# SeanNaren/deepspeech.pytorch

Measured on AMD Instinct MI355X. Metric: audio-seconds/sec (train step), higher is better.
Workload: dtype bf16

## Files before the change

### deepspeech/pytorch_amd/_lib.py

```python
import ctypes as C
import os

HERE = os.path.dirname(os.path.abspath(__file__))
LIB_PATH = os.path.join(HERE, "libds2hip.so")

F32, BF16 = 0, 1
CELL_GRU, CELL_LSTM, CELL_RNN_TANH = 0, 1, 2

_vp, _i, _l, _f, _ll = C.c_void_p, C.c_int, C.c_long, C.c_float, C.c_longlong

SIGNATURES = {
    "ds2_version": (_i, []),
    "ds2_error_string": (C.c_char_p, [_i]),
    "ds2_gemm_nt": (_i, [_i, _vp, _vp, _vp, _vp, _i, _i, _i, _l, _l, _l, _i, _i, _l, _l, _l, _l, _i, _vp]),
    "ds2_gemm_nt_coresident": (_i, [_i, _vp, _vp, _vp, _vp, _i, _i, _i, _l, _l, _l, _i, _i, _l, _l, _l, _l, _i, _vp]),
    "ds2_gemm_nt_rows2": (_i, [_i, _vp, _vp, _i, _vp, _vp, _i, _i, _i, _l, _l, _l, _i, _i, _i, _vp]),
    "ds2_gemm8_nt": (_i, [_vp, _vp, _vp, _vp, _i, _i, _i, _l, _l, _l, _i, _vp]),
    "ds2_gemm8_tn_grouped": (_i, [_i, _vp, _vp, _vp, _vp, _vp, _vp, _vp, _vp, _vp, _vp, _vp, _i, _vp]),
    "ds2_gemm8_nt_rows": (_i, [_vp, _vp, _vp, _vp, _i, _i, _i, _l, _l, _l, _i, _vp, _i, _vp]),
    "ds2_gemm8_tn_grouped_rows": (_i, [_i, _vp, _vp, _vp, _vp, _vp, _vp, _vp, _vp, _vp, _vp, _vp, _i, _vp, _i, _vp]),
    "ds2_gemm8_wgrad_dx_rows": (_i, [_i, _vp, _vp, _vp, _vp, _vp, _vp, _vp, _vp, _vp, _vp, _vp, _i, _vp, _vp, _vp, _i, _i, _i, _l, _l, _l, _vp, _i, _vp]),
    "ds2_zero_pad_rows": (_i, [_i, _vp, _l, _i, _vp, _i, _i, _vp]),
    "ds2_gemm8_wgrad_dx": (_i, [_i, _vp, _vp, _vp, _vp, _vp, _vp, _vp, _vp, _vp, _vp, _vp, _i, _vp, _vp, _vp, _i, _i, _i, _l, _l, _l, _vp]),
    "ds2_norm_partials": (_i, [_l]),
    "ds2_bn_fwd": (_i, [_i, _i, _i, _vp, _vp, _l, _i, _l, _l, _i, _i, _i, _vp, _vp, _vp, _vp, _vp, _vp, _f, _f, _vp, _vp,
                        _vp, _vp, _vp, _vp]),
    "ds2_bn_bwd": (_i, [_i, _i, _vp, _vp, _vp, _l, _i, _l, _l, _l, _i, _i, _i, _vp, _vp, _vp, _vp, _vp, _vp, _vp, _vp, _vp]),
    "ds2_colsum": (_i, [_i, _vp, _l, _i, _l, _vp, _f, _vp, _vp]),
    "ds2_conv_rows": (_i, [_i, _vp, _vp]),
    "ds2_conv1_fwd": (_i, [_i, _vp, _vp, _vp, _vp, _vp, _i, _i, _i, _i, _vp]),
    "ds2_conv1_wgrad_ws_floats": (_l, [_i, _i, _i]),
    "ds2_conv1_wgrad": (_i, [_i, _vp, _vp, _vp, _i, _i, _i, _i, _vp, _vp]),
    "ds2_conv2_fwd_ws_bytes": (_l, [_i, _i, _i, _i]),
    "ds2_conv2_fwd": (_i, [_i, _vp, _vp, _vp, _vp, _vp, _i, _i, _i, _vp, _vp]),
    "ds2_conv2_dgrad": (_i, [_i, _vp, _vp, _vp, _vp, _i, _i, _i, _vp]),
    "ds2_conv2_wgrad_ws_floats": (_l, [_i, _i]),
    "ds2_conv2_wgrad": (_i, [_i, _vp, _vp, _vp, _i, _i, _i, _vp, _vp]),
    "ds2_rnn_gates": (_i, [_i]),
    "ds2_rnn_saved_planes": (_i, [_i]),
    "ds2_rnn_state_bytes": (_l, [_i, _i, _i]),
    "ds2_rnn_fwd": (_i, [_i, _i, _i, _i, _i, _i, _vp, _vp, _vp, _vp, _vp, _vp, _vp, _l, _vp, _vp, _vp, _vp, _vp]),
    "ds2_rnn_bwd": (_i, [_i, _i, _i, _i, _i, _i, _vp, _vp, _vp, _vp, _l, _vp, _vp, _vp, _vp, _vp, _vp, _vp, _vp, _vp]),
    "ds2_rnn_persist_plan": (_i, [_i, _i, _i, _i, _i, _i, C.c_uint, C.POINTER(_l)]),
    "ds2_rnn_persist_supported": (_i, [_i, _i, _i, _i, _i, C.c_uint]),
    "ds2_rnn_persist_shape_covered": (_i, [_i, _i, _i, _i, _i]),
    "ds2_rnn_persist_kind": (_i, [_i, _i, _i, _i, _i, C.c_uint]),
    "ds2_rnn_persist_ws_bytes": (_l, [_i, _i, _i, _i, _i, C.c_uint]),
    "ds2_rnn_persist_fwd": (_i, [_i, _i, _i, _i, _i, _i, _vp, _vp, _vp, _vp, _vp, _vp, _vp, _l, _vp, _vp, _vp, _vp, _vp, _vp, _vp]),
    "ds2_rnn_persist_bwd": (_i, [_i, _i, _i, _i, _i, _i, _vp, _vp, _vp, _vp, _l, _vp, _vp, _vp, _vp, _i, _vp, _vp, _vp, _vp]),
    "ds2_add2": (_i, [_i, _vp, _vp, _vp, _l, _vp]),
    "ds2_sum_slices": (_i, [_vp, _vp, _l, _i, _vp]),
    "ds2_transpose": (_i, [_i, _vp, _vp, _l, _i, _l, _l, _vp]),
    "ds2_split3_bf16": (_i, [_vp, _l, _l, _i, _i, _i, _vp, _l, _vp]),
    "ds2_cast_transpose_bf16": (_i, [_vp, _l, _i, _i, _i, _i, _i, _vp, _l, _vp, _l, _vp]),
    "ds2_small_weight_layouts": (_i, [_i, _vp, _vp, _vp, _i, _i, _vp, _vp, _vp, _vp, _vp, _vp, _vp]),
    "ds2_scale_by": (_i, [_vp, _vp, _l, _vp]),
    "ds2_copy_words": (_i, [_vp, _vp, _l, _vp]),
    "ds2_lookahead_fwd": (_i, [_i, _vp, _vp, _vp, _vp, _i, _i, _i, _i, _vp]),
    "ds2_lookahead_ws_floats": (_l, [_i, _i, _i, _i]),
    "ds2_lookahead_bwd": (_i, [_i, _vp, _vp, _vp, _vp, _vp, _vp, _i, _i, _i, _i, _vp, _vp]),
    "ds2_rnn_bias_grads": (_i, [_i, _i, _i, _i, _vp, _vp, _vp, _vp]),
    "ds2_softmax_rows": (_i, [_vp, _vp, _l, _i, _l, _l, _vp]),
    "ds2_opt_max_tensors": (_i, []),
    "ds2_clip_ws_floats": (_l, [_i, _vp]),
    "ds2_clip_coef": (_i, [_i, _vp, _vp, _f, _vp, _vp, _vp]),
    "ds2_opt_multi": (_i, [_i, _i, _vp, _vp, _vp, _vp, _vp, _vp, _i, _vp, _vp]),
    "ds2_opt_matrix": (_i, [_i, _vp, _vp, _vp, _vp, _i, _i, _i, _i, _i, _vp, _l, _vp, _l, _vp, _i, _vp, _vp]),
    "ds2_opt_matrices": (_i, [_i, _i] + [_vp] * 13 + [_vp, _i, _vp, _vp]),
    "ds2_spect_frames": (_i, [_i]),
    "ds2_spect_ws_bytes": (_l, [_i, _i]),
    "ds2_spectrogram": (_i, [_vp, _l, _vp, _i, _i, _vp, _i, _i, _vp, _vp, _vp]),
    "ds2_spectrogram_aug": (_i, [_vp, _l, _vp, _i, _i, _vp, _i, _i, _vp, _vp, _vp, _i, _vp, _i, _vp, _i, _vp, _vp]),
    "ds2_spec_augment_coef": (_i, [_vp, _i, _i, _i, _vp, _vp, _i, _vp, _vp]),
    "ds2_spec_augment": (_i, [_vp, _vp, _i, _i, _i, _vp, _vp, _vp, _i, _vp, _i, _vp]),
    "ds2_greedy_decode": (_i, [_vp, _l, _l, _i, _i, _i, _vp, _i, _vp, _vp, _vp, _vp]),
    "ds2_beam_ws_bytes": (_l, [_i, _i, _i]),
    "ds2_beam_decode": (_i, [_vp, _l, _l, _i, _i, _i, _vp, _i, _i, _i, _f, _vp, _vp, _vp, _vp, _vp, _vp]),
    "ds2_beam_decode_lm": (_i, [_vp, _l, _l, _i, _i, _i, _vp, _i, _i, _i, _f, _i, _vp, _l, _vp, _l, _i, _i, _f, _f, _i,
                                _vp, _vp, _vp, _vp, _vp, _vp, _vp]),
    "ds2_beam_grid_ws_bytes": (_l, [_i, _i, _i, _i]),
    "ds2_beam_decode_lm_grid": (_i, [_vp, _l, _l, _i, _i, _i, _vp, _i, _i, _i, _f, _i, _vp, _l, _vp, _l, _i, _i, _i, _i, _vp, _vp,
                                     _vp, _vp, _vp, _vp, _vp, _vp, _vp]),
    "ds2_error_counts": (_i, [_vp, _l, _vp, _i, _vp, _vp, _i, _i, _vp, _vp, _vp, _vp, _vp]),
    "ds2_ctc_ws_floats": (_l, [_i, _i, _i, _i]),
    "ds2_ctc_loss_grad": (_i, [_vp, _l, _vp, _vp, _vp, _vp, _i, _i, _i, _i, _i, _f, _vp, _vp, _vp, _l, _vp, _i, _vp]),
}



class PersistOpts(C.Structure):
    _fields_ = [("variant", C.c_uint), ("spin_limit", C.c_uint), ("startup_ms", C.c_uint)]


_lib = None


class Ds2HipError(RuntimeError):
    pass


def load():
    global _lib
    if _lib is not None:
        return _lib
    if not os.path.exists(LIB_PATH):
        raise Ds2HipError(
            "libds2hip.so not found at %s -- build it with `python -m deepspeech.pytorch_amd.build` "
            "(hipcc --offload-arch=gfx950).  There is no fallback path." % LIB_PATH)
    lib = C.CDLL(LIB_PATH)
    for name, (res, args) in SIGNATURES.items():
        fn = getattr(lib, name)
        fn.restype = res
        fn.argtypes = args
    _lib = lib
    return lib


def error_string(code):
    return load().ds2_error_string(int(code)).decode()


def call(name, *args):
    rc = getattr(load(), name)(*args)
    if rc != 0:
        raise Ds2HipError("%s failed with code %d: %s" % (name, rc, error_string(rc)))


def query(name, *args):
    return getattr(load(), name)(*args)
```

### deepspeech/pytorch_amd/csrc/ds2_norm.hip

```cpp
#include "ds2_common.h"

namespace {

constexpr int NORM_RY = 8;
constexpr int NORM_CX = 32;

struct RowMap {
  int F, Tp;
  __device__ __forceinline__ void nt(long row, int& n, int& t) const {
    t = (int)(row % Tp);
    n = (int)(row / ((long)F * Tp));
  }
};

__device__ __forceinline__ float bn_affine(float x, float sc, float sh) { return __builtin_fmaf(x, sc, sh); }
__device__ __forceinline__ bool hardtanh_open(float y) { return y > 0.f && y < 20.f; }
__device__ __forceinline__ float bn_dx(float g, float xh, float sc, float k1, float k2) { return sc * __builtin_fmaf(-xh, k2, g - k1); }

struct RedMap {
  int cpb, rpx, chunk, rsub;
  bool ok;
  __device__ __forceinline__ RedMap(int chunks) {
    cpb = chunks < NORM_CX ? chunks : NORM_CX;
    rpx = NORM_CX / cpb;
    const int tx = threadIdx.x;
    rsub = tx / cpb;
    chunk = blockIdx.x * cpb + tx % cpb;
    ok = rsub < rpx && chunk < chunks;
  }
  __device__ __forceinline__ long first_row() const { return ((long)blockIdx.y * NORM_RY + threadIdx.y) * rpx + rsub; }
  __device__ __forceinline__ long row_step() const { return (long)gridDim.y * NORM_RY * rpx; }
};
template <int V>
__device__ __forceinline__ void red_block(float (*red)[NORM_CX * V + 1], const RedMap& m, const float (&v)[V], float (&out)[V]) {
  __syncthreads();
#pragma unroll
  for (int i = 0; i < V; ++i) red[threadIdx.y][threadIdx.x * V + i] = v[i];
  __syncthreads();
  if (threadIdx.y == 0 && m.rsub == 0) {
#pragma unroll
    for (int i = 0; i < V; ++i) {
      float a = 0.f;
      for (int k = 0; k < m.rpx; ++k)
#pragma unroll
        for (int y = 0; y < NORM_RY; ++y) a += red[y][(threadIdx.x + k * m.cpb) * V + i];
      out[i] = a;
    }
  }
}

template <typename T, bool SQ>
__global__ void __launch_bounds__(NORM_RY* NORM_CX) k_colstats(const T* __restrict__ X, long R, int C, long ld,
                                                                float* __restrict__ psum, float* __restrict__ psq) {
  constexpr int V = Vec16<T>::N;
  __shared__ float red[NORM_RY][NORM_CX * V + 1];
  const RedMap m(C / V);
  float s[V], q[V];
#pragma unroll
  for (int i = 0; i < V; ++i) s[i] = q[i] = 0.f;
  if (m.ok) {
    for (long r = m.first_row(); r < R; r += m.row_step()) {
      float v[V];
      Vec16<T>::load(X + r * ld + (long)m.chunk * V, v);
#pragma unroll
      for (int i = 0; i < V; ++i) {
        s[i] += v[i];
        if (SQ) q[i] += v[i] * v[i];
      }
    }
  }
  float o[V];
  red_block<V>(red, m, s, o);
  if (threadIdx.y == 0 && m.rsub == 0 && m.ok) {
#pragma unroll
    for (int i = 0; i < V; ++i) psum[(long)blockIdx.y * C + (long)m.chunk * V + i] = o[i];
  }
  if (SQ) {
    red_block<V>(red, m, q, o);
    if (threadIdx.y == 0 && m.rsub == 0 && m.ok) {
#pragma unroll
      for (int i = 0; i < V; ++i) psq[(long)blockIdx.y * C + (long)m.chunk * V + i] = o[i];
    }
  }
}

constexpr int FIN_COLS = 32, FIN_SLICES = 8;
template <int NA>
__device__ __forceinline__ void finalize_sums(const float* const (&arr)[NA], int P, int C, int c, int py, double (&tot)[NA]) {
  __shared__ double sh[NA][FIN_SLICES][FIN_COLS];
  double acc[NA];
#pragma unroll
  for (int a = 0; a < NA; ++a) acc[a] = 0.0;
  if (c < C) {
#pragma unroll 8
    for (int p = py; p < P; p += FIN_SLICES) {
#pragma unroll
      for (int a = 0; a < NA; ++a) acc[a] += (double)arr[a][(long)p * C + c];
    }
  }
#pragma unroll
  for (int a = 0; a < NA; ++a) sh[a][py][threadIdx.x & (FIN_COLS - 1)] = acc[a];
  __syncthreads();
#pragma unroll
  for (int a = 0; a < NA; ++a) {
    double t = 0.0;
    if (py == 0) {
#pragma unroll
      for (int q = 0; q < FIN_SLICES; ++q) t += sh[a][q][threadIdx.x & (FIN_COLS - 1)];
    }
    tot[a] = t;
  }
}

__global__ void __launch_bounds__(256) k_colsum_finalize(const float* __restrict__ psum, int P, int C, float* __restrict__ out,
                                                          float scale) {
  const int c = blockIdx.x * FIN_COLS + (threadIdx.x & (FIN_COLS - 1)), py = threadIdx.x / FIN_COLS;
  const float* const arr[1] = {psum};
  double tot[1];
  finalize_sums<1>(arr, P, C, c, py, tot);
  if (py == 0 && c < C) out[c] = (float)(tot[0] * (double)scale);
}

__global__ void k_bn_finalize(const float* __restrict__ psum, const float* __restrict__ psq, int P, int C, double count,
                              const float* __restrict__ gamma, const float* __restrict__ beta, float eps,
                              float momentum, float* __restrict__ running_mean, float* __restrict__ running_var,
                              long long* __restrict__ num_batches_tracked, float* __restrict__ mean_out,
                              float* __restrict__ rstd_out, float* __restrict__ scale_out, float* __restrict__ shift_out) {
  const int c = blockIdx.x * FIN_COLS + (threadIdx.x & (FIN_COLS - 1)), py = threadIdx.x / FIN_COLS;
  if (blockIdx.x == 0 && threadIdx.x == 0 && num_batches_tracked) *num_batches_tracked += 1;
  const float* const arr[2] = {psum, psq};
  double tot[2];
  finalize_sums<2>(arr, P, C, c, py, tot);
  if (py != 0 || c >= C) return;
  const double s = tot[0], q = tot[1];
  double mean = s / count;
  double var = q / count - mean * mean;
  if (var < 0.0) var = 0.0;
  double rstd = 1.0 / sqrt(var + (double)eps);
  mean_out[c] = (float)mean;
  rstd_out[c] = (float)rstd;
  float sc = (float)((double)gamma[c] * rstd);
  scale_out[c] = sc;
  shift_out[c] = (float)((double)beta[c] - mean * (double)gamma[c] * rstd);
  if (running_mean) {
    double unb = count > 1.0 ? var * (count / (count - 1.0)) : var;
    running_mean[c] = (float)((1.0 - (double)momentum) * (double)running_mean[c] + (double)momentum * mean);
    running_var[c] = (float)((1.0 - (double)momentum) * (double)running_var[c] + (double)momentum * unb);
  }
}

__global__ void k_bn_eval_coeffs(int C, const float* __restrict__ gamma, const float* __restrict__ beta,
                                 const float* __restrict__ running_mean, const float* __restrict__ running_var, float eps,
                                 float* __restrict__ scale_out, float* __restrict__ shift_out) {
  int c = blockIdx.x * blockDim.x + threadIdx.x;
  if (c >= C) return;
  double rstd = 1.0 / sqrt((double)running_var[c] + (double)eps);
  scale_out[c] = (float)((double)gamma[c] * rstd);
  shift_out[c] = (float)((double)beta[c] - (double)running_mean[c] * (double)gamma[c] * rstd);
}

template <typename T, bool CONV, bool SEQ_OUT, bool CENTRED = false>
__global__ void __launch_bounds__(256) k_bn_apply(const T* __restrict__ X, T* __restrict__ Y, long R, int C, long ldx,
                                                   long ldy, const float* __restrict__ scale,
                                                   const float* __restrict__ shift, const float* __restrict__ mean,
                                                   const float* __restrict__ beta, RowMap rm,
                                                   const int* __restrict__ lens, int N) {
  constexpr int V = Vec16<T>::N;
  const int chunks = C / V;
  const long total = R * chunks;
  for (long e = (long)blockIdx.x * blockDim.x + threadIdx.x; e < total; e += (long)gridDim.x * blockDim.x) {
    long r = e / chunks;
    int c0 = (int)(e % chunks) * V;
    float v[V];
    bool live = true;
    int n = 0, t = 0;
    if (CONV) {
      rm.nt(r, n, t);
      live = t < lens[n];
    }
    if (live) {
      Vec16<T>::load(X + r * ldx + c0, v);
#pragma unroll
      for (int i = 0; i < V; ++i) {
        float y = CENTRED ? __builtin_fmaf(v[i] - mean[c0 + i], scale[c0 + i], beta[c0 + i]) : bn_affine(v[i], scale[c0 + i], shift[c0 + i]);
        if (CONV) y = fminf(fmaxf(y, 0.f), 20.f);
        v[i] = y;
      }
    } else {
#pragma unroll
      for (int i = 0; i < V; ++i) v[i] = 0.f;
    }
    if (SEQ_OUT) {
      int f = (int)((r / rm.Tp) % rm.F);
      Vec16<T>::store(Y + ((long)t * N + n) * ldy + (long)f * C + c0, v);
    } else {
      Vec16<T>::store(Y + r * ldy + c0, v);
    }
  }
}

template <typename T, bool CONV, bool SEQ_IN>
__device__ __forceinline__ bool load_gated(const T* __restrict__ G, const T* __restrict__ X, long r, int c0, int C,
                                           long ldg, long ldx, const float* __restrict__ scale,
                                           const float* __restrict__ shift, const float* __restrict__ mean,
                                           const float* __restrict__ rstd, const RowMap& rm, const int* __restrict__ lens,
                                           int N, float (&g)[Vec16<T>::N], float (&xh)[Vec16<T>::N]) {
  constexpr int V = Vec16<T>::N;
  int n = 0, t = 0, f = 0;
  if (CONV) {
    const unsigned ur = (unsigned)r, q = ur / (unsigned)rm.Tp;
    t = (int)(ur - q * (unsigned)rm.Tp);
    n = (int)(q / (unsigned)rm.F);
    f = (int)(q - (unsigned)n * (unsigned)rm.F);
  }
  const int len = CONV ? lens[n] : 0;
  float x[V];
  Vec16<T>::load(X + r * ldx + c0, x);
  if (SEQ_IN) {
    Vec16<T>::load(G + ((long)t * N + n) * ldg + (long)f * C + c0, g);
  } else {
    Vec16<T>::load(G + r * ldg + c0, g);
  }
  if (CONV && t >= len) return false;
#pragma unroll
  for (int i = 0; i < V; ++i) {
    if (CONV) {
      if (!hardtanh_open(bn_affine(x[i], scale[c0 + i], shift[c0 + i]))) g[i] = 0.f;
    }
    xh[i] = (x[i] - mean[c0 + i]) * rstd[c0 + i];
  }
  return true;
}

template <typename T, bool CONV, bool SEQ_IN>
__global__ void __launch_bounds__(NORM_RY* NORM_CX)
    k_bn_bwd_reduce(const T* __restrict__ G, const T* __restrict__ X, long R, int C, long ldg, long ldx,
                    const float* __restrict__ scale, const float* __restrict__ shift, const float* __restrict__ mean,
                    const float* __restrict__ rstd, RowMap rm, const int* __restrict__ lens, int N,
                    float* __restrict__ psum_g, float* __restrict__ psum_gx) {
  constexpr int V = Vec16<T>::N;
  __shared__ float red[NORM_RY][NORM_CX * V + 1];
  const RedMap m(C / V);
  float s[V], q[V];
#pragma unroll
  for (int i = 0; i < V; ++i) s[i] = q[i] = 0.f;
  if (m.ok) {
    for (long r = m.first_row(); r < R; r += m.row_step()) {
      float g[V], xh[V];
      if (load_gated<T, CONV, SEQ_IN>(G, X, r, m.chunk * V, C, ldg, ldx, scale, shift, mean, rstd, rm, lens, N, g, xh)) {
#pragma unroll
        for (int i = 0; i < V; ++i) {
          s[i] += g[i];
          q[i] += g[i] * xh[i];
        }
      }
    }
  }
  float o[V];
  red_block<V>(red, m, s, o);
  if (threadIdx.y == 0 && m.rsub == 0 && m.ok) {
#pragma unroll
    for (int i = 0; i < V; ++i) psum_g[(long)blockIdx.y * C + (long)m.chunk * V + i] = o[i];
  }
  red_block<V>(red, m, q, o);
  if (threadIdx.y == 0 && m.rsub == 0 && m.ok) {
#pragma unroll
    for (int i = 0; i < V; ++i) psum_gx[(long)blockIdx.y * C + (long)m.chunk * V + i] = o[i];
  }
}

__global__ void k_bn_bwd_finalize(const float* __restrict__ psum_g, const float* __restrict__ psum_gx, int P, int C,
                                  double count, float* __restrict__ dgamma, float* __restrict__ dbeta,
                                  float* __restrict__ c1, float* __restrict__ c2) {
  const int c = blockIdx.x * FIN_COLS + (threadIdx.x & (FIN_COLS - 1)), py = threadIdx.x / FIN_COLS;
  const float* const arr[2] = {psum_g, psum_gx};
  double tot[2];
  finalize_sums<2>(arr, P, C, c, py, tot);
  if (py != 0 || c >= C) return;
  const double s = tot[0], q = tot[1];
  dbeta[c] = (float)s;
  dgamma[c] = (float)q;
  c1[c] = (float)(s / count);
  c2[c] = (float)(q / count);
}

template <typename T, bool CONV, bool SEQ_IN>
__global__ void __launch_bounds__(256)
    k_bn_bwd_apply(const T* __restrict__ G, const T* __restrict__ X, T* __restrict__ DX, long R, int C, long ldg, long ldx,
                   long lddx, const float* __restrict__ scale, const float* __restrict__ shift,
                   const float* __restrict__ mean, const float* __restrict__ rstd, const float* __restrict__ c1,
                   const float* __restrict__ c2, RowMap rm, const int* __restrict__ lens, int N) {
  constexpr int V = Vec16<T>::N;
  const int chunks = C / V;
  const long total = R * chunks;
  for (long e = (long)blockIdx.x * blockDim.x + threadIdx.x; e < total; e += (long)gridDim.x * blockDim.x) {
    long r = e / chunks;
    int c0 = (int)(e % chunks) * V;
    float g[V], xh[V], o[V];
    if (load_gated<T, CONV, SEQ_IN>(G, X, r, c0, C, ldg, ldx, scale, shift, mean, rstd, rm, lens, N, g, xh)) {
#pragma unroll
      for (int i = 0; i < V; ++i) o[i] = bn_dx(g[i], xh[i], scale[c0 + i], c1[c0 + i], c2[c0 + i]);
    } else {
#pragma unroll
      for (int i = 0; i < V; ++i) o[i] = 0.f;
    }
    Vec16<T>::store(DX + r * lddx + c0, o);
  }
}

template <typename T, bool CONV, bool SEQ_IN>
__global__ void __launch_bounds__(NORM_RY* NORM_CX)
    k_bn_bwd_apply_cols(const T* __restrict__ G, const T* __restrict__ X, T* __restrict__ DX, long R, int C, long ldg, long ldx,
                        long lddx, const float* __restrict__ scale, const float* __restrict__ shift,
                        const float* __restrict__ mean, const float* __restrict__ rstd, const float* __restrict__ c1,
                        const float* __restrict__ c2, RowMap rm, const int* __restrict__ lens, int N) {
  constexpr int V = Vec16<T>::N;
  const RedMap m(C / V);
  if (!m.ok) return;
  const int c0 = m.chunk * V;
  float sc[V], sh[V], mu[V], rs[V], k1[V], k2[V];
#pragma unroll
  for (int i = 0; i < V; ++i) {
    sc[i] = scale[c0 + i];
    sh[i] = CONV ? shift[c0 + i] : 0.f;
    mu[i] = mean[c0 + i];
    rs[i] = rstd[c0 + i];
    k1[i] = c1[c0 + i];
    k2[i] = c2[c0 + i];
  }
  const long step = m.row_step();
  auto addr = [&](long r, int& t, int& len, const T*& gp) {
    int n = 0, f = 0;
    t = 0;
    if (CONV) {
      const unsigned ur = (unsigned)r, q = ur / (unsigned)rm.Tp;
      t = (int)(ur - q * (unsigned)rm.Tp);
      n = (int)(q / (unsigned)rm.F);
      f = (int)(q - (unsigned)n * (unsigned)rm.F);
    }
    len = CONV ? lens[n] : 0;
    gp = SEQ_IN ? G + ((long)t * N + n) * ldg + (long)f * C + c0 : G + r * ldg + c0;
  };
  auto finish = [&](long r, int t, int len, float (&x)[V], float (&g)[V]) {
    float o[V];
    if (CONV && t >= len) {
#pragma unroll
      for (int i = 0; i < V; ++i) o[i] = 0.f;
    } else {
#pragma unroll
      for (int i = 0; i < V; ++i) {
        float gi = g[i];
        if (CONV) {
          if (!hardtanh_open(bn_affine(x[i], sc[i], sh[i]))) gi = 0.f;
        }
        const float xh = (x[i] - mu[i]) * rs[i];
        o[i] = bn_dx(gi, xh, sc[i], k1[i], k2[i]);
      }
    }
    Vec16<T>::store(DX + r * lddx + c0, o);
  };
  long r = m.first_row();
  for (; r + step < R; r += 2 * step) {
    int t0, t1, l0, l1;
    const T *g0p, *g1p;
    addr(r, t0, l0, g0p);
    addr(r + step, t1, l1, g1p);
    float x0[V], x1[V], g0[V], g1[V];
    Vec16<T>::load(X + r * ldx + c0, x0);
    Vec16<T>::load(X + (r + step) * ldx + c0, x1);
    Vec16<T>::load(g0p, g0);
    Vec16<T>::load(g1p, g1);
    finish(r, t0, l0, x0, g0);
    finish(r + step, t1, l1, x1, g1);
  }
  if (r < R) {
    int t0, l0;
    const T* g0p;
    addr(r, t0, l0, g0p);
    float x0[V], g0[V];
    Vec16<T>::load(X + r * ldx + c0, x0);
    Vec16<T>::load(g0p, g0);
    finish(r, t0, l0, x0, g0);
  }
}

inline int norm_grid_y(long R, int col_blocks = 1) {
  long gy = (R + NORM_RY - 1) / NORM_RY;
  long cap = 1024 / (col_blocks < 1 ? 1 : col_blocks);
  if (cap < 256) cap = 256;
  if (gy > cap) gy = cap;
  if (gy < 1) gy = 1;
  return (int)gy;
}

template <typename T>
int colstats_impl(const void* X, long R, int C, long ld, float* psum, float* psq, int* P_out, hipStream_t st) {
  constexpr int V = Vec16<T>::N;
  DS2_REQUIRE(C % V == 0 && ld % V == 0, DS2_ERR_ALIGN);
  dim3 blk(NORM_CX, NORM_RY);
  dim3 grd(ds2_cdiv(C / V, NORM_CX), norm_grid_y(R, ds2_cdiv(C / V, NORM_CX)));
  if (psq)
    hipLaunchKernelGGL((k_colstats<T, true>), grd, blk, 0, st, (const T*)X, R, C, ld, psum, psq);
  else
    hipLaunchKernelGGL((k_colstats<T, false>), grd, blk, 0, st, (const T*)X, R, C, ld, psum, psq);
  *P_out = grd.y;
  DS2_CHECK_LAUNCH();
  return 0;
}

inline int apply_grid(long total) {
  long g = (total + 255) / 256;
  if (g > 256 * 8) g = 256 * 8;
  if (g < 1) g = 1;
  return (int)g;
}

}

extern "C" {

int ds2_norm_partials(long R) { return norm_grid_y(R); }

int ds2_colsum(int dtype, const void* X, long R, int C, long ld, float* out, float scale, float* ws, ds2_stream_t st_) {
  hipStream_t st = (hipStream_t)st_;
  int P = 0, rc;
  if (dtype == DS2_F32)
    rc = colstats_impl<float>(X, R, C, ld, ws, nullptr, &P, st);
  else
    rc = colstats_impl<bf16_t>(X, R, C, ld, ws, nullptr, &P, st);
  if (rc) return rc;
  hipLaunchKernelGGL(k_colsum_finalize, dim3(ds2_cdiv(C, FIN_COLS)), dim3(256), 0, st, ws, P, C, out, scale);
  DS2_CHECK_LAUNCH();
  return 0;
}

int ds2_bn_fwd(int dtype, int mode, int training, const void* X, void* Y, long R, int C, long ldx, long ldy, int F, int Tp,
               int N, const int* lens, const float* gamma, const float* beta, float* running_mean, float* running_var,
               long long* num_batches_tracked, float eps, float momentum, float* save_mean, float* save_rstd,
               float* save_scale, float* save_shift, float* ws, ds2_stream_t st_) {
  hipStream_t st = (hipStream_t)st_;
  DS2_REQUIRE(dtype == DS2_F32 || dtype == DS2_BF16, DS2_ERR_DTYPE);
  DS2_REQUIRE(mode >= 0 && mode <= 2, DS2_ERR_ARG);
  DS2_REQUIRE(mode == 0 || R < (1L << 31), DS2_ERR_ARG);
  int rc, P = 0;
  if (training) {
    float* psum = ws;
    float* psq = ws + (long)norm_grid_y(R) * C;
    rc = dtype == DS2_F32 ? colstats_impl<float>(X, R, C, ldx, psum, psq, &P, st)
                          : colstats_impl<bf16_t>(X, R, C, ldx, psum, psq, &P, st);
    if (rc) return rc;
    hipLaunchKernelGGL(k_bn_finalize, dim3(ds2_cdiv(C, FIN_COLS)), dim3(256), 0, st, psum, psq, P, C, (double)R, gamma, beta,
                       eps, momentum, running_mean, running_var, num_batches_tracked, save_mean, save_rstd, save_scale,
                       save_shift);
  } else {
    hipLaunchKernelGGL(k_bn_eval_coeffs, dim3(ds2_cdiv(C, 128)), dim3(128), 0, st, C, gamma, beta, running_mean,
                       running_var, eps, save_scale, save_shift);
  }
  DS2_CHECK_LAUNCH();
  RowMap rm{F, Tp};
  const int V = dtype == DS2_F32 ? 4 : 8;
  DS2_REQUIRE(C % V == 0 && ldx % V == 0 && ldy % V == 0, DS2_ERR_ALIGN);
  dim3 g(apply_grid(R * (C / V))), b(256);
#define LAUNCH_APPLY(TT)                                                                                              \
  if (mode == 0 && training && R == 1)                                                                                \
    hipLaunchKernelGGL((k_bn_apply<TT, false, false, true>), g, b, 0, st, (const TT*)X, (TT*)Y, R, C, ldx, ldy,        \
                       save_scale, save_shift, save_mean, beta, rm, lens, N);                                         \
  else if (mode == 0)                                                                                                 \
    hipLaunchKernelGGL((k_bn_apply<TT, false, false>), g, b, 0, st, (const TT*)X, (TT*)Y, R, C, ldx, ldy, save_scale,  \
                       save_shift, save_mean, beta, rm, lens, N);                                                     \
  else if (mode == 1)                                                                                                 \
    hipLaunchKernelGGL((k_bn_apply<TT, true, false>), g, b, 0, st, (const TT*)X, (TT*)Y, R, C, ldx, ldy, save_scale,   \
                       save_shift, save_mean, beta, rm, lens, N);                                                     \
  else                                                                                                                \
    hipLaunchKernelGGL((k_bn_apply<TT, true, true>), g, b, 0, st, (const TT*)X, (TT*)Y, R, C, ldx, ldy, save_scale,    \
                       save_shift, save_mean, beta, rm, lens, N);
  if (dtype == DS2_F32) {
    LAUNCH_APPLY(float)
  } else {
    LAUNCH_APPLY(bf16_t)
  }
#undef LAUNCH_APPLY
  DS2_CHECK_LAUNCH();
  return 0;
}

int ds2_bn_bwd(int dtype, int mode, const void* G, const void* X, void* DX, long R, int C, long ldg, long ldx, long lddx,
               int F, int Tp, int N, const int* lens, const float* save_mean, const float* save_rstd,
               const float* save_scale, const float* save_shift, float* dgamma, float* dbeta, float* ws, ds2_stream_t st_) {
  hipStream_t st = (hipStream_t)st_;
  DS2_REQUIRE(dtype == DS2_F32 || dtype == DS2_BF16, DS2_ERR_DTYPE);
  DS2_REQUIRE(mode >= 0 && mode <= 2, DS2_ERR_ARG);
  DS2_REQUIRE(mode == 0 || R < (1L << 31), DS2_ERR_ARG);
  const int V = dtype == DS2_F32 ? 4 : 8;
  DS2_REQUIRE(C % V == 0 && ldx % V == 0 && ldg % V == 0 && lddx % V == 0, DS2_ERR_ALIGN);
  RowMap rm{F, Tp};
  const int P = norm_grid_y(R, ds2_cdiv(C / V, NORM_CX));
  float* ps = ws;
  float* pq = ws + (long)P * C;
  float* c1 = pq + (long)P * C;
  float* c2 = c1 + C;
  dim3 blk(NORM_CX, NORM_RY), grd(ds2_cdiv(C / V, NORM_CX), P);
#define LAUNCH_RED(TT, CV, SI)                                                                                          \
  hipLaunchKernelGGL((k_bn_bwd_reduce<TT, CV, SI>), grd, blk, 0, st, (const TT*)G, (const TT*)X, R, C, ldg, ldx,          \
                     save_scale, save_shift, save_mean, save_rstd, rm, lens, N, ps, pq)
  const int acb = ds2_cdiv(C / V, NORM_CX), arpx = NORM_CX / (C / V < NORM_CX ? C / V : NORM_CX);
  long agy = ds2_cdiv(R, (long)NORM_RY * arpx * 2);
  if (agy > 2048 / acb) agy = 2048 / acb;
  if (agy < 1) agy = 1;
  const dim3 agrd(acb, (unsigned)agy);
#ifdef DS2_BN_APPLY_GRIDSTRIDE
#define LAUNCH_APP(TT, CV, SI)                                                                                          \
  hipLaunchKernelGGL((k_bn_bwd_apply<TT, CV, SI>), dim3(apply_grid(R*(C / V))), dim3(256), 0, st, (const TT*)G,           \
                     (const TT*)X, (TT*)DX, R, C, ldg, ldx, lddx, save_scale, save_shift, save_mean, save_rstd, c1, c2, \
                     rm, lens, N)
#else
#define LAUNCH_APP(TT, CV, SI)                                                                                          \
  hipLaunchKernelGGL((k_bn_bwd_apply_cols<TT, CV, SI>), agrd, blk, 0, st, (const TT*)G, (const TT*)X, (TT*)DX, R, C, ldg, \
                     ldx, lddx, save_scale, save_shift, save_mean, save_rstd, c1, c2, rm, lens, N)
#endif
#define BOTH(WHICH)                                        \
  if (dtype == DS2_F32) {                                  \
    if (mode == 0) WHICH(float, false, false);             \
    else if (mode == 1) WHICH(float, true, false);         \
    else WHICH(float, true, true);                         \
  } else {                                                 \
    if (mode == 0) WHICH(bf16_t, false, false);            \
    else if (mode == 1) WHICH(bf16_t, true, false);        \
    else WHICH(bf16_t, true, true);                        \
  }
  BOTH(LAUNCH_RED)
  DS2_CHECK_LAUNCH();
  hipLaunchKernelGGL(k_bn_bwd_finalize, dim3(ds2_cdiv(C, FIN_COLS)), dim3(256), 0, st, ps, pq, P, C, (double)R, dgamma, dbeta,
                     c1, c2);
  DS2_CHECK_LAUNCH();
  BOTH(LAUNCH_APP)
  DS2_CHECK_LAUNCH();
#undef BOTH
#undef LAUNCH_RED
#undef LAUNCH_APP
  return 0;
}

}
```

### deepspeech/pytorch_amd/model.py

```python
import math
from typing import List

import numpy as np
import torch
import torch.nn as nn

from . import ops
from ._lib import Ds2HipError

try:
    import pytorch_lightning as pl
    _Base = pl.LightningModule
except Exception:
    pl = None

    class _Base(nn.Module):

        def save_hyperparameters(self, *a, **k):
            import inspect
            frame = inspect.currentframe().f_back
            try:
                names = [n for n in inspect.signature(type(self).__init__).parameters if n != "self"]
                self._hparams = {n: frame.f_locals[n] for n in names if n in frame.f_locals}
            finally:
                del frame

        @property
        def hparams(self):
            return getattr(self, "_hparams", {})

        def log(self, *a, **k):
            pass

        @property
        def device(self):
            return next(self.parameters()).device

        @classmethod
        def load_from_checkpoint(cls, checkpoint_path, map_location=None, strict=True, **overrides):
            ckpt = torch.load(checkpoint_path, map_location=map_location or "cpu", weights_only=False)
            hp = dict(ckpt.get("hyper_parameters", {}))
            hp.update(overrides)
            model = cls(**hp)
            model.load_state_dict(ckpt["state_dict"], strict=strict)
            return model

try:
    from omegaconf import OmegaConf

    def _cfg_type_name(cfg):
        t = OmegaConf.get_type(cfg)
        return getattr(t, "__name__", str(t))
except Exception:
    def _cfg_type_name(cfg):
        return type(cfg).__name__

from .configs import AdamConfig, BiDirectionalConfig, SGDConfig, SpectConfig, UniDirectionalConfig, rnn_kind

import os

WGRAD_WITH_DX = os.environ.get("DS2_WGRAD_WITH_DX", "1") not in ("", "0")

COMPOSITE_NODE = {"": None, "0": False}.get(os.environ.get("DS2_COMPOSITE_NODE", ""), True)
PER_LAYER_NODES_FOR_DDP = [False]


PAD_HIDDEN = os.environ.get("DS2_PAD_HIDDEN", "1") != "0"


def _padded_hidden(H, kind, precision, bidirectional=None):
    base = (int(H) + 15) // 16 * 16
    if not PAD_HIDDEN or base < 200 or kind not in ("gru", "lstm", "rnn"):
        return base
    try:
        from ._lib import query
        dt_ = ops.dt(torch.bfloat16 if str(precision) in ("16", "bf16", "16-mixed", "bf16-mixed") else torch.float32)
        cell = ops.CELLS[kind]
        dirs = (2, 1) if bidirectional is None else ((2,) if bidirectional else (1,))
        for w in range(base, int(base * 1.5) + 1, 16):
            if any(query("ds2_rnn_persist_shape_covered", dt_, cell, D_, 1, w) for D_ in dirs):
                return w
    except Exception:
        pass
    return base


def _data_parallel_active():
    if PER_LAYER_NODES_FOR_DDP[0]:
        return True
    try:
        import torch.distributed as _dist
        return _dist.is_available() and _dist.is_initialized() and _dist.get_world_size() > 1
    except Exception:
        return False


FP32_WGRAD_TN = os.environ.get("DS2_FP32_WGRAD_TN", "1") != "0"

ROW_LISTS = os.environ.get("DS2_ROW_LISTS", "1") != "0"
ROW_LIST_MIN_PADDING = 0.97

N_FREQ_CONV2 = 41
RNN_INPUT = 32 * N_FREQ_CONV2
RNN_INPUT_LD = 1344


def _round64(n):
    return (n + 63) // 64 * 64


class SequenceWise(nn.Module):
    def __init__(self, module):
        super().__init__()
        self.module = module


class MaskConv(nn.Module):
    def __init__(self, seq_module):
        super().__init__()
        self.seq_module = seq_module


class _RNNParams(nn.Module):

    def __init__(self, kind, input_size, hidden_size, bidirectional):
        super().__init__()
        g = ops.GATES[kind]
        for suf in [""] + (["_reverse"] if bidirectional else []):
            self.register_parameter("weight_ih_l0" + suf, nn.Parameter(torch.empty(g * hidden_size, input_size)))
            self.register_parameter("weight_hh_l0" + suf, nn.Parameter(torch.empty(g * hidden_size, hidden_size)))
            self.register_parameter("bias_ih_l0" + suf, nn.Parameter(torch.empty(g * hidden_size)))
            self.register_parameter("bias_hh_l0" + suf, nn.Parameter(torch.empty(g * hidden_size)))
        stdv = 1.0 / math.sqrt(hidden_size) if hidden_size > 0 else 0
        for w in self.parameters():
            nn.init.uniform_(w, -stdv, stdv)


class BatchRNN(nn.Module):
    def __init__(self, input_size, hidden_size, kind, bidirectional=False, batch_norm=True):
        super().__init__()
        self.input_size, self.hidden_size, self.bidirectional, self.kind = input_size, hidden_size, bidirectional, kind
        self.batch_norm = SequenceWise(nn.BatchNorm1d(input_size)) if batch_norm else None
        self.rnn = _RNNParams(kind, input_size, hidden_size, bidirectional)
        self.num_directions = 2 if bidirectional else 1


class Lookahead(nn.Module):
    def __init__(self, n_features, context):
        super().__init__()
        assert context > 0
        self.context, self.n_features = context, n_features
        self.conv = nn.Conv1d(n_features, n_features, kernel_size=context, stride=1, groups=n_features, padding=0, bias=False)


class _WeightCache:

    def __init__(self):
        self._store = {}
        self.epoch = 0

    def get(self, key, params, builder):
        ver = (self.epoch,) + tuple((p._version, p.data_ptr()) for p in params)
        hit = self._store.get(key)
        if hit is not None and hit[0] == ver:
            return hit[1]
        with torch.no_grad():
            val = builder()
        self._store[key] = (ver, val)
        return val

    def _ver(self, params):
        return (self.epoch,) + tuple((p._version, p.data_ptr()) for p in params)

    def valid(self, key, params):
        hit = self._store.get(key)
        return hit is not None and hit[0] == self._ver(params)

    def put(self, key, params, val, epoch=None):
        ver = self._ver(params)
        if epoch is not None:
            ver = (epoch,) + ver[1:]
        self._store[key] = (ver, val)

    def clear(self):
        self._store.clear()


def _wgrad_splitk(M, N, K):
    tiles = ((M + 127) // 128) * ((N + 127) // 128)
    if tiles >= 128:
        return 1
    return max(1, min(8, 768 // max(tiles, 1), K // (64 * 32)))


def _pad_gate_rows(w, G, H, Hp):
    if Hp == H:
        return w
    out = w.new_zeros((G, Hp) + tuple(w.shape[1:]))
    out[:, :H] = w.reshape((G, H) + tuple(w.shape[1:]))
    return out.reshape((G * Hp,) + tuple(w.shape[1:]))


def _pad_cols(w, Cp):
    if w.shape[-1] == Cp:
        return w
    out = w.new_zeros(tuple(w.shape[:-1]) + (Cp,))
    out[..., :w.shape[-1]] = w
    return out


def _unpad_gate_rows(g, G, H, Hp):
    if Hp == H:
        return g
    return g.reshape((G, Hp) + tuple(g.shape[1:]))[:, :H].reshape((G * H,) + tuple(g.shape[1:])).contiguous()


def _bn_seq_fwd(bn, w, b, X, Xh, R, Ct, Cp, training):
    if Ct == Cp:
        return ops.bn_fwd(X, 0, training, w.detach(), b.detach(), bn.running_mean, bn.running_var, bn.num_batches_tracked, R, Ct,
                          X.stride(0), Xh, Xh.stride(0), eps=bn.eps, momentum=bn.momentum)
    g, be = w.new_ones(Cp), w.new_zeros(Cp)
    rm, rv = w.new_zeros(Cp), w.new_ones(Cp)
    g[:Ct], be[:Ct], rm[:Ct], rv[:Ct] = w.detach(), b.detach(), bn.running_mean, bn.running_var
    sv = ops.bn_fwd(X, 0, training, g, be, rm, rv, bn.num_batches_tracked, R, Cp, X.stride(0), Xh, Xh.stride(0), eps=bn.eps,
                    momentum=bn.momentum)
    if training:
        bn.running_mean.copy_(rm[:Ct])
        bn.running_var.copy_(rv[:Ct])
    return sv


def _bn_seq_bwd(G, X, DX, sv, R, Ct, Cp):
    dg, db = ops.bn_bwd(G, X, DX, 0, sv, R, Cp, G.stride(0), X.stride(0), DX.stride(0))
    return (dg, db) if Ct == Cp else (dg[:Ct].contiguous(), db[:Ct].contiguous())


def _perm_cols_to_internal(w):
    g, rin = w.shape
    out = w.new_zeros((g, _round64(rin)))
    out[:, :rin] = w.reshape(g, 32, rin // 32).permute(0, 2, 1).reshape(g, rin)
    return out


def _perm_cols_to_reference(w, rin=RNN_INPUT):
    g = w.shape[0]
    return w[:, :rin].reshape(g, rin // 32, 32).permute(0, 2, 1).reshape(g, rin)


class _ConvStackFn(torch.autograd.Function):

    @staticmethod
    def forward(ctx, x, w1, b1, g1, be1, w2, b2, g2, be2, mod, lens_dev, Tp, dtype, training):
        N, T = x.shape[0], x.shape[3]
        c = mod._cache
        bn1, bn2 = mod.conv.seq_module[1], mod.conv.seq_module[4]
        w1k = c.get("w1k", [w1], lambda: w1.detach().reshape(32, 451).t().contiguous())
        w2t = c.get(("w2t", dtype), [w2], lambda: w2.detach().permute(2, 3, 0, 1).contiguous().to(dtype))
        x = x.contiguous().float()
        F0, F1, F2, rin, rld = mod._F0, mod._F1, mod._F2, mod._rnn_in, mod._rnn_ld
        if x.shape[2] != F0:
            raise ValueError("this model was built for %d frequency bins (SpectConfig: sample_rate * window_size / 2 + 1), got input "
                             "with %d" % (F0, x.shape[2]))
        y1 = ops.conv1_fwd(x, w1k, b1.detach(), lens_dev, Tp, dtype)
        R1 = N * F1 * Tp
        a1 = torch.empty_like(y1)
        sv1 = ops.bn_fwd(y1, 1, training, g1.detach(), be1.detach(), bn1.running_mean, bn1.running_var,
                         bn1.num_batches_tracked, R1, 32, 32, a1, 32, F=F1, Tp=Tp, N=N, lens=lens_dev, eps=bn1.eps,
                         momentum=bn1.momentum)
        y2 = ops.conv2_fwd(a1, w2t, b2.detach(), lens_dev, F0)
        R2 = N * F2 * Tp
        x0 = torch.empty((Tp * N, rld), dtype=dtype, device=x.device)
        if rld > rin:
            x0[:, rin:].zero_()
        sv2 = ops.bn_fwd(y2, 2, training, g2.detach(), be2.detach(), bn2.running_mean, bn2.running_var,
                         bn2.num_batches_tracked, R2, 32, 32, x0, rld, F=F2, Tp=Tp, N=N, lens=lens_dev, eps=bn2.eps,
                         momentum=bn2.momentum)
        ctx.mod, ctx.dims, ctx.sv = mod, (N, T, Tp, dtype), (sv1, sv2)
        ctx.save_for_backward(x, y1, a1, y2, lens_dev, w2)
        return x0

    @staticmethod
    def backward(ctx, dx0):
        x, y1, a1, y2, lens_dev, w2 = ctx.saved_tensors
        N, T, Tp, dtype = ctx.dims
        sv1, sv2 = ctx.sv
        c = ctx.mod._cache
        dx0 = dx0.contiguous().to(dtype)
        F0, F1, F2, rld = ctx.mod._F0, ctx.mod._F1, ctx.mod._F2, ctx.mod._rnn_ld
        R1, R2 = N * F1 * Tp, N * F2 * Tp
        dy2 = torch.empty_like(y2)
        dg2, dbe2 = ops.bn_bwd(dx0, y2, dy2, 2, sv2, R2, 32, rld, 32, 32, F=F2, Tp=Tp, N=N, lens=lens_dev)
        w2d = c.get(("w2d", dtype), [w2], lambda: [
            w2.detach()[:, :, q::2, :].flip(2, 3).permute(2, 3, 1, 0).contiguous().to(dtype) for q in (0, 1)])
        da1 = ops.conv2_dgrad(dy2, w2d[0], w2d[1], F0)
        dy1 = torch.empty_like(y1)
        dg1, dbe1 = ops.bn_bwd(da1, y1, dy1, 1, sv1, R1, 32, 32, 32, 32, F=F1, Tp=Tp, N=N, lens=lens_dev)
        db1 = ops.colsum(dy1.view(R1, 32))
        dw1k = ops.conv1_wgrad(x, dy1, Tp)
        dw1 = dw1k.t().reshape(32, 1, 41, 11).contiguous()
        db2 = ops.colsum(dy2.view(R2, 32))
        dw2 = ops.conv2_wgrad(dy2, a1, F0).view(21, 11, 32, 32).permute(2, 3, 0, 1).contiguous()
        return (None, dw1, db1, dg1, dbe1, dw2, db2, dg2, dbe2, None, None, None, None, None)


def _layer_param_count(layer):
    return (2 if layer.batch_norm is not None else 0) + 4 * layer.num_directions


_ROWS_STAGING, _CTC_STAGING = ops.PinnedRing(), ops.PinnedRing()


def _frame_rows(output_lengths, Tp, N, dev):
    ol = output_lengths.numpy().astype(np.int32)
    n_valid = int(np.minimum(ol, Tp).sum())
    if not ROW_LISTS or n_valid >= ROW_LIST_MIN_PADDING * Tp * N or n_valid == 0:
        return output_lengths.to(dev, torch.int32, non_blocking=True), None
    rows = np.flatnonzero(np.arange(Tp, dtype=np.int32)[:, None] < ol[None, :]).astype(np.int32)
    both = _ROWS_STAGING.stage(dev, [ol, rows])
    return both[:N], both[N:]


def _rnn_layer_forward(mod, li, X, lens_dev, N, Tp, dtype, training, h0, c0, lparams, rows=None):
    c = mod._cache
    R = Tp * N
    layer = mod.rnns[li]
    kind, Ht, D = layer.kind, layer.hidden_size, layer.num_directions
    H = mod._Hp
    G = ops.GATES[kind]
    first = li == 0
    I = mod._rnn_ld if first else H
    has_bn = layer.batch_norm is not None
    bn_w, bn_b = (lparams[0], lparams[1]) if has_bn else (None, None)
    wts = lparams[2 if has_bn else 0:]
    wih = [wts[4 * d + 0] for d in range(D)]
    whh = [wts[4 * d + 1] for d in range(D)]
    bih = [wts[4 * d + 2] for d in range(D)]
    bhh = [wts[4 * d + 3] for d in range(D)]

    def build_ih():
        w = torch.cat([_pad_gate_rows(p.detach(), G, Ht, H) for p in wih], 0)
        w = _perm_cols_to_internal(w) if first else _pad_cols(w, H)
        out = ops.empty_padded(w.shape[0], w.shape[1], dtype, w.device)
        out.copy_(w)
        return out
    Wih = c.get(("wih", li, dtype), wih, build_ih)
    Whh = c.get(("whh", li, dtype), whh, lambda: torch.stack(
        [_pad_gate_rows(_pad_cols(p.detach(), H), G, Ht, H) for p in whh], 0).to(dtype).contiguous())
    if H == Ht:
        Bih, Bhh = mod._bias_views(li)
    else:
        Bih = c.get(("bih", li), bih, lambda: torch.cat([_pad_gate_rows(p.detach(), G, Ht, H) for p in bih], 0))
        Bhh = c.get(("bhh", li), bhh, lambda: torch.stack([_pad_gate_rows(p.detach(), G, Ht, H) for p in bhh], 0))
    sv, Xh = None, X
    if has_bn:
        bn = layer.batch_norm.module
        Xh = ops.empty_padded(R, I, X.dtype, X.device)
        sv = _bn_seq_fwd(bn, bn_w, bn_b, X, Xh, R, layer.input_size, I, training)
    if ops.split3_ok(dtype, R, D * G * H, I):
        Wih3 = c.get(("wih3", li), wih, lambda: ops.split3(Wih, 1))
        GI = ops.gemm_nt(ops.split3(Xh, 0), Wih3, bias=Bih, out_dtype=torch.float32, rows=rows)
    else:
        GI = ops.gemm_nt(Xh, Wih, bias=Bih, rows=rows)
    if H != Ht:
        h0 = _pad_cols(h0, H) if h0 is not None else None
        c0 = _pad_cols(c0, H) if c0 is not None else None
    hext, Sv, hn, cn = ops.rnn_fwd(kind, GI, Whh, Bhh, lens_dev, D, N, H, Tp, h0=h0, c0=c0)
    if H != Ht:
        hn = hn[..., :Ht].contiguous()
        cn = cn[..., :Ht].contiguous() if cn is not None else None
    del GI
    if D == 2:
        out = ops.add2(hext[0, 1:Tp + 1].reshape(R, H), hext[1, 1:Tp + 1].reshape(R, H))
    else:
        out = hext[0, 1:Tp + 1].reshape(R, H)
    return out, hn, cn, [X, Xh if has_bn else None, hext, Sv], (kind, H, D, G, I, has_bn, sv, Ht, layer.input_size)


def _rnn_layer_backward(mod, li, meta, saved, lparams, dout, lens_dev, N, Tp, dtype, main, side, rows=None, state=None):
    kind, H, D, G, I, has_bn, sv, Ht, It = meta
    if state is not None:
        h0, c0, want = state
        h0p = _pad_cols(h0, H) if (h0 is not None and H != Ht) else h0
        c0p = _pad_cols(c0, H) if (c0 is not None and H != Ht) else c0
        state = (h0p, c0p, bool(want))
    dX, grads, rg = _rnn_layer_backward_impl(mod, li, meta, saved, lparams, dout, lens_dev, N, Tp, dtype, main, side, rows, state)
    if state is None:
        return dX, grads, None
    main.wait_stream(side)
    GH, po = G * H, (2 if has_bn else 0)
    if h0p is not None:
        n4 = (N + 3) // 4 * 4
        ar = torch.arange(N, device=lens_dev.device)
        for d in range(D):
            t_first = torch.zeros_like(ar) if d == 0 else (lens_dev.long().clamp(1, Tp) - 1)
            src = rg.dGH[d].reshape(Tp * N, GH) if (kind == "gru" and rg.dGH is not None) else rg.dGI[:, d * GH:(d + 1) * GH]
            g_first = src.index_select(0, t_first * N + ar).float()
            A = torch.zeros((GH, n4), dtype=torch.float32, device=g_first.device)
            A[:, :N] = g_first.t()
            B = torch.zeros((H, n4), dtype=torch.float32, device=g_first.device)
            B[:, :N] = h0p[d].t()
            corr = ops.gemm_nt(A, B, out_dtype=torch.float32)
            grads[po + 4 * d + 1] = grads[po + 4 * d + 1] + _unpad_gate_rows(corr, G, Ht, H)[:, :Ht]
    dstate = None
    if want:
        dstate = (rg.dh0[..., :Ht].contiguous(), rg.dc0[..., :Ht].contiguous() if rg.dc0 is not None else None)
    return dX, grads, dstate


def _rnn_transposed_weights(mod, li, meta, lparams, dtype):
    kind, H, D, G, I, has_bn, sv, Ht, It = meta
    po = 2 if has_bn else 0
    wih = [lparams[po + 4 * d + 0] for d in range(D)]
    whh = [lparams[po + 4 * d + 1] for d in range(D)]
    WhhT = mod._cache.get(("whhT", li, dtype), whh, lambda: torch.stack(
        [_pad_gate_rows(_pad_cols(p.detach(), H), G, Ht, H).t() for p in whh], 0).to(dtype).contiguous())

    def build_ihT():
        w = torch.cat([_pad_gate_rows(p.detach(), G, Ht, H) for p in wih], 0)
        w = _perm_cols_to_internal(w) if li == 0 else _pad_cols(w, H)
        return w.t().to(dtype).contiguous()
    return WhhT, mod._cache.get(("wihT", li, dtype), wih, build_ihT)


def _wgrad_path(dtype, kind, R, D, GH, H, Xh, rg=None):
    if ops.wgrad_tn_ok(dtype, R, D * GH, Xh.shape[1], lda=D * GH, ldb=Xh.stride(0)) and \
            ops.wgrad_tn_ok(dtype, R, GH, H, lda=D * GH, ldb=H):
        return "tn"
    if rg is None:
        return None
    if ops.split3_ok(dtype, GH, H, R, leaf=True) and FP32_WGRAD_TN and Xh.shape[1] % 8 == 0 and \
            ops.wgrad_tn_ok(torch.bfloat16, 3 * R, D * GH, Xh.shape[1]) and ops.wgrad_tn_ok(torch.bfloat16, 3 * R, GH, H) and \
            (kind != "gru" or rg.dQ is not None or rg.dGH is not None):
        return "tn_split"
    return "nt"


def _rnn_layer_backward_impl(mod, li, meta, saved, lparams, dout, lens_dev, N, Tp, dtype, main, side, rows=None, state=None):
    kind, H, D, G, I, has_bn, sv, Ht, It = meta
    X, Xh, hext, Sv = saved
    if Xh is None:
        Xh = X
    R, GH = Tp * N, G * H
    grads = [None] * len(lparams)
    WhhT, WihT = _rnn_transposed_weights(mod, li, meta, lparams, dtype)
    path = _wgrad_path(dtype, kind, R, D, GH, H, Xh)
    n_probs = 1 + D * (2 if (kind == "gru" and (2 * H) % 256 != 0) else 1)
    fuse_dx = path == "tn" and WGRAD_WITH_DX and n_probs < 6 and WihT.dim() == 2 and WihT.data_ptr() % 16 == 0 and \
        ops.gemm8_nt_shape_ok(dtype, R, WihT.shape[0], D * GH, D * GH, WihT.stride(0))
    if state is None:
        rg = ops.rnn_bwd(kind, dout, WhhT, hext, Sv, lens_dev, D, N, H, Tp, pad_rows_unread=bool(fuse_dx and rows is not None))
    else:
        rg = ops.rnn_bwd(kind, dout, WhhT, hext, Sv, lens_dev, D, N, H, Tp, h0=state[0], c0=state[1], want_dstate=state[2])
    dGI = rg.dGI
    layer = (mod, li, meta, lparams, grads, Xh, hext, rg, N, Tp)
    if fuse_dx:
        dXh = _wgrad_tn(*layer, rows=rows, dx=(dGI, WihT), zero_pad=(lens_dev, Tp, N))
    else:
        if path == "tn":
            _wgrad_tn(*layer, rows=rows)
        if ops.split3_ok(dtype, R, H, GH):
            po = 2 if has_bn else 0
            WihT3 = mod._cache.get(("wihT3", li), [lparams[po + 4 * d] for d in range(D)], lambda: ops.split3(WihT, 1))
            dXh = ops.gemm_nt(ops.split3(dGI, 0), WihT3, out_dtype=torch.float32, rows=rows, zero_pad=(lens_dev, Tp, N))
        else:
            dXh = ops.gemm_nt(dGI, WihT, rows=rows, zero_pad=(lens_dev, Tp, N))
    if has_bn:
        dX = torch.empty_like(dXh)
        grads[0], grads[1] = _bn_seq_bwd(dXh, X, dX, sv, R, It, I)
    else:
        dX = dXh
    if path == "tn":
        return dX, grads, rg
    ready = torch.cuda.Event()
    ready.record(main)
    with torch.cuda.stream(side):
        side.wait_event(ready)
        for t in rg.tensors() + [Xh, hext]:
            t.record_stream(side)
        if _wgrad_path(dtype, kind, R, D, GH, H, Xh, rg) == "tn_split":
            _wgrad_tn(*layer, split=True)
        else:
            _wgrad_nt(*layer)
    return dX, grads, rg


def _h_prev(hext, d, Tp, R, H):
    return (hext[d, 0:Tp] if d == 0 else hext[d, 2:Tp + 2]).reshape(R, H)


def _wgrad_problems(kind, rg, Xh, hext, Tp, operand, two_block, dWih, dWhh):
    D, GH, H = dWhh.shape
    R = rg.dGI.shape[0]
    A, B = operand(rg.dGI, 0), operand(Xh, 1)
    lda = A.stride(0)
    probs = [dict(At=A, Bt=B, M=D * GH, N=Xh.shape[1], lda=lda, ldb=B.stride(0), out=dWih)]
    for d in range(D):
        Hp = operand(_h_prev(hext, d, Tp, R, H), 1)
        hh = dict(Bt=Hp, N=H, ldb=Hp.stride(0))
        if kind == "gru" and rg.dQ is not None:
            Q = operand(rg.dQ[d].reshape(R, H), 0)
            if two_block:
                probs.append(dict(hh, At=A[:, d * GH:], At2=Q, lda2=Q.stride(0), m_split=2 * H, M=GH, lda=lda, out=dWhh[d]))
            else:
                probs.append(dict(hh, At=A[:, d * GH:], M=2 * H, lda=lda, out=dWhh[d, :2 * H]))
                probs.append(dict(hh, At=Q, M=H, lda=Q.stride(0), out=dWhh[d, 2 * H:]))
        elif kind == "gru":
            Gd = operand(rg.dGH[d].reshape(R, GH), 0)
            probs.append(dict(hh, At=Gd, M=GH, lda=Gd.stride(0), out=dWhh[d]))
        else:
            probs.append(dict(hh, At=A[:, d * GH:], M=GH, lda=lda, out=dWhh[d]))
    return probs


def _rnn_bias_grads(kind, rg, D, N, H):
    R, GH = rg.dGI.shape[0], rg.dGI.shape[1] // D
    if rg.bacc is not None:
        dBih, dBhh_all = ops.rnn_bias_grads(kind, rg.bacc, D, N, H)
        return dBih, dBhh_all, [dBhh_all[d] for d in range(D)]
    dBih = ops.colsum(rg.dGI)
    if kind == "gru":
        return dBih, None, [ops.colsum(rg.dGH[d].reshape(R, GH)) for d in range(D)]
    return dBih, None, [dBih[d * GH:(d + 1) * GH] for d in range(D)]


def _deliver_layer_grads(mod, li, meta, lparams, grads, per_dir, own):
    kind, H, D, G, I, has_bn, sv, Ht, It = meta
    po = 2 if has_bn else 0
    for d in range(D):
        grads[po + 4 * d:po + 4 * d + 4] = per_dir[d]
    sync = getattr(mod, "_grad_sync", None)
    if sync is not None and H == Ht:
        sync.layer_ready(own, lparams[po:po + 4 * D])
    _unpad_layer_grads(grads, po, D, G, Ht, H, It, li == 0)


def _wgrad_tn(mod, li, meta, lparams, grads, Xh, hext, rg, N, Tp, split=False, rows=None, dx=None, zero_pad=None):
    kind, H, D, G = meta[:4]
    GH, dev = G * H, rg.dGI.device
    K = (3 if split else 1) * Tp * N
    dWih = torch.empty((D * GH, Xh.shape[1]), dtype=torch.float32, device=dev)
    dWhh = torch.empty((D, GH, H), dtype=torch.float32, device=dev)
    probs = _wgrad_problems(kind, rg, Xh, hext, Tp, ops.split3_rows if split else (lambda t, mode: t),
                            not split and (2 * H) % 256 == 0, dWih, dWhh)
    dXh = None
    if dx is not None:
        assert ops.gemm8_nt_ok(dx[0], dx[1], K, dx[1].shape[0], D * GH, D * GH, dx[1].stride(0))
        _, dXh = ops.gemm8_tn_grouped(probs, K, dx=dx, rows=rows, zero_pad=zero_pad)
    else:
        ops.gemm8_tn_grouped(probs, K, rows=rows)
    if li == 0:
        dWih = torch.cat([_perm_cols_to_reference(dWih[d * GH:(d + 1) * GH], mod._rnn_in) for d in range(D)], 0)
    dBih, dBhh_all, dBhh_l = _rnn_bias_grads(kind, rg, D, N, H)
    per_dir = [(dWih[d * GH:(d + 1) * GH], dWhh[d], dBih[d * GH:(d + 1) * GH], dBhh_l[d]) for d in range(D)]
    own = [dWih, dWhh, dBih] + ([dBhh_all] if dBhh_all is not None else dBhh_l if kind == "gru" else [])
    _deliver_layer_grads(mod, li, meta, lparams, grads, per_dir, own)
    return dXh


def _wgrad_nt(mod, li, meta, lparams, grads, Xh, hext, rg, N, Tp):
    kind, H, D, G = meta[:4]
    R, GH, dGI, cores = Tp * N, G * H, rg.dGI, li > 0
    s3 = ops.split3_ok(dGI.dtype, GH, H, R, leaf=True)
    dGI_T = ops.transpose(dGI)
    Xh_T = ops.transpose(Xh)
    ldT = dGI_T.shape[1]
    dGI_T3 = ops.split3(dGI_T, 0) if s3 else None
    if s3:
        dWih = ops.gemm_nt(dGI_T3, ops.split3(Xh_T, 1), out_dtype=torch.float32, coresident=cores)
    else:
        dWih = ops.gemm_nt(dGI_T, Xh_T, out_dtype=torch.float32, splitk=_wgrad_splitk(dGI_T.shape[0], Xh_T.shape[0], ldT),
                           coresident=cores)
    del Xh_T
    if li == 0:
        dWih = torch.cat([_perm_cols_to_reference(dWih[d * GH:(d + 1) * GH], mod._rnn_in) for d in range(D)], 0)
    bsum = None
    if rg.bacc is not None:
        bsum = [ops.colsum(rg.bacc[d]) for d in range(D)]
        dBih = torch.cat([b[:GH] for b in bsum], 0)
    else:
        dBih = ops.colsum(dGI)
    per_dir = []
    for d in range(D):
        Hp_T = ops.transpose(_h_prev(hext, d, Tp, R, H))
        if kind == "gru" and rg.dQ is not None:
            dQ_T = ops.transpose(rg.dQ[d].reshape(R, H))
            if s3:
                A3 = torch.empty((GH, 3 * ldT), dtype=torch.bfloat16, device=dGI.device)
                A3[:2 * H].copy_(dGI_T3[d * GH:d * GH + 2 * H])
                ops.split3(dQ_T, 0, out=A3[2 * H:])
                dWhh = ops.gemm_nt(A3, ops.split3(Hp_T, 1), out_dtype=torch.float32, coresident=cores)
            else:
                dWhh = ops.gemm_nt_rows2(dGI_T[d * GH:d * GH + 2 * H], dQ_T, 2 * H, Hp_T, GH, H, ldT, ldT, ldT,
                                         splitk=_wgrad_splitk(GH, H, ldT), coresident=cores)
            dBhh = torch.cat([bsum[d][:2 * H], bsum[d][3 * H:4 * H]], 0) if bsum is not None else \
                torch.cat([dBih[d * GH:d * GH + 2 * H], ops.colsum(rg.dQ[d].reshape(R, H))], 0)
        else:
            if kind == "gru":
                dGH_T = ops.transpose(rg.dGH[d].reshape(R, GH))
                dBhh = ops.colsum(rg.dGH[d].reshape(R, GH))
            else:
                dGH_T = dGI_T[d * GH:(d + 1) * GH]
                dBhh = dBih[d * GH:(d + 1) * GH]
            if s3:
                A3 = ops.split3(dGH_T, 0) if kind == "gru" else dGI_T3[d * GH:(d + 1) * GH]
                dWhh = ops.gemm_nt(A3, ops.split3(Hp_T, 1), out_dtype=torch.float32, coresident=cores)
            else:
                dWhh = ops.gemm_nt(dGH_T, Hp_T, out_dtype=torch.float32, M=GH, N=H, K=ldT, lda=ldT, ldb=ldT,
                                   splitk=_wgrad_splitk(GH, H, ldT), coresident=cores)
        per_dir.append((dWih[d * GH:(d + 1) * GH].contiguous(), dWhh, dBih[d * GH:(d + 1) * GH].contiguous(), dBhh.contiguous()))
    own = [dWih, dBih] + [p[1] for p in per_dir] + ([p[3] for p in per_dir] if kind == "gru" else [])
    _deliver_layer_grads(mod, li, meta, lparams, grads, per_dir, own)


class _RnnLayerFn(torch.autograd.Function):

    @staticmethod
    def forward(ctx, X, mod, lens_dev, N, Tp, dtype, training, li, h0, c0, *lparams):
        ctx.rows = mod._frame_rows
        out, hn, cn, saved, meta = _rnn_layer_forward(mod, li, X, lens_dev, N, Tp, dtype, training, h0, c0, lparams, rows=ctx.rows)
        ctx.mod, ctx.dims, ctx.meta, ctx.li = mod, (N, Tp, dtype), meta, li
        ctx.had_state = h0 is not None or c0 is not None
        ctx.h0, ctx.c0 = h0, c0
        ctx.none_mask = [t is None for t in saved]
        ctx.save_for_backward(lens_dev, *[t for t in saved if t is not None], *lparams)
        ctx.n_saved = sum(1 for t in saved if t is not None)
        outs = (out, hn) + ((cn,) if cn is not None else ())
        ctx.mark_non_differentiable(*outs[1:])
        ctx.set_materialize_grads(False)
        return outs

    @staticmethod
    def backward(ctx, dout, *unused):
        N, Tp, dtype = ctx.dims
        mod = ctx.mod
        st = ctx.saved_tensors
        it = iter(st[1:1 + ctx.n_saved])
        saved = [None if is_none else next(it) for is_none in ctx.none_mask]
        lparams = st[1 + ctx.n_saved:]
        main = torch.cuda.current_stream()
        side = mod._wgrad_stream(dout.device)
        state = None
        if ctx.had_state:
            want = bool(ctx.needs_input_grad[8] or (len(ctx.needs_input_grad) > 9 and ctx.needs_input_grad[9]))
            state = (ctx.h0, ctx.c0, want)
        dX, grads, dstate = _rnn_layer_backward(mod, ctx.li, ctx.meta, saved, lparams, dout.contiguous().to(dtype), st[0], N, Tp, dtype,
                                                main, side, rows=ctx.rows, state=state)
        main.wait_stream(side)
        for g in grads:
            if g is not None:
                g.record_stream(main)
        sync = getattr(mod, "_grad_sync", None)
        if sync is not None:
            grads = sync.defer_early(lparams, grads)
        dh0 = dstate[0] if (dstate is not None and ctx.needs_input_grad[8]) else None
        dc0 = dstate[1] if (dstate is not None and ctx.c0 is not None and ctx.needs_input_grad[9]) else None
        return (dX, None, None, None, None, None, None, None, dh0, dc0, *grads)


class _RnnStackFn(torch.autograd.Function):

    @staticmethod
    def forward(ctx, X, mod, lens_dev, N, Tp, dtype, training, n_layers, *rest):
        L = n_layers
        hs0, cs0, params = rest[:L], rest[L:2 * L], rest[2 * L:]
        ctx.rows = mod._frame_rows
        saved, meta, outs_h, outs_c, pos = [], [], [], [], 0
        for li in range(L):
            n = _layer_param_count(mod.rnns[li])
            out, hn, cn, sv4, mt = _rnn_layer_forward(mod, li, X, lens_dev, N, Tp, dtype, training, hs0[li], cs0[li], params[pos:pos + n],
                                                      rows=ctx.rows)
            pos += n
            saved += sv4
            meta.append(mt)
            outs_h.append(hn)
            if cn is not None:
                outs_c.append(cn)
            X = out
        ctx.mod, ctx.dims, ctx.meta = mod, (N, Tp, dtype, L), meta
        ctx.had_state = any(h is not None for h in hs0)
        ctx.n_params = len(params)
        ctx.save_for_backward(lens_dev, *saved, *params)
        ctx.mark_non_differentiable(*outs_h, *outs_c)
        return (X, *outs_h, *outs_c)

    @staticmethod
    def backward(ctx, dout, *unused):
        N, Tp, dtype, L = ctx.dims
        if ctx.had_state:
            raise Ds2HipError("backward through a forward that was given initial hidden states (hs) is not supported")
        mod = ctx.mod
        st = ctx.saved_tensors
        lens_dev, saved, params = st[0], st[1:1 + 4 * L], st[1 + 4 * L:]
        main = torch.cuda.current_stream()
        side = mod._wgrad_stream(dout.device)
        offs, pos = [], 0
        for li in range(L):
            offs.append(pos)
            pos += _layer_param_count(mod.rnns[li])
        grads = [None] * len(params)
        dout = dout.contiguous().to(dtype)
        for li in reversed(range(L)):
            n = _layer_param_count(mod.rnns[li])
            dout, lg, _ = _rnn_layer_backward(mod, li, ctx.meta[li], list(saved[4 * li:4 * li + 4]), params[offs[li]:offs[li] + n],
                                              dout, lens_dev, N, Tp, dtype, main, side, rows=ctx.rows)
            grads[offs[li]:offs[li] + n] = lg
        if getattr(ctx, "defer_join", False):
            ctx.pending = (main, side, grads, mod)
        else:
            _join_side(main, side, grads, mod)
        return (dout, None, None, None, None, None, None, None, *([None] * (2 * L)), *grads)


def _unpad_layer_grads(grads, po, D, G, Ht, H, It, first):
    if H == Ht:
        return
    for d in range(D):
        dWih, dWhh, dBih, dBhh = grads[po + 4 * d:po + 4 * d + 4]
        dWih = _unpad_gate_rows(dWih, G, Ht, H)
        grads[po + 4 * d] = dWih if first else dWih[:, :It].contiguous()
        grads[po + 4 * d + 1] = _unpad_gate_rows(dWhh, G, Ht, H)[:, :Ht].contiguous()
        grads[po + 4 * d + 2] = _unpad_gate_rows(dBih, G, Ht, H)
        grads[po + 4 * d + 3] = _unpad_gate_rows(dBhh, G, Ht, H)


def _join_side(main, side, grads, mod=None):
    main.wait_stream(side)
    sync = getattr(mod, "_grad_sync", None)
    if sync is not None:
        sync.wait_early()
    for g in grads:
        if g is not None:
            g.record_stream(main)


class _SubCtx:

    def save_for_backward(self, *t):
        self.saved_tensors = t

    def mark_non_differentiable(self, *a):
        pass


class _FrontFn(torch.autograd.Function):

    @staticmethod
    def forward(ctx, x, mod, lens_dev, N, Tp, dtype, training, n_layers, *rest):
        conv_params, rnn_rest = rest[:8], rest[8:]
        c1, c2 = _SubCtx(), _SubCtx()
        X0 = _ConvStackFn.forward(c1, x, *conv_params, mod, lens_dev, Tp, dtype, training)
        if mod._prep_done is not None:
            torch.cuda.current_stream().wait_event(mod._prep_done)
            mod._prep_done = None
        outs = _RnnStackFn.forward(c2, X0, mod, lens_dev, N, Tp, dtype, training, n_layers, *rnn_rest)
        ctx.c1, ctx.c2, ctx.L = c1, c2, n_layers
        ctx.mark_non_differentiable(*outs[1:])
        ctx.set_materialize_grads(False)
        return outs

    @staticmethod
    def backward(ctx, dout, *unused):
        c1, c2, L = ctx.c1, ctx.c2, ctx.L
        if c1 is None:
            raise RuntimeError("DeepSpeech (gfx950): trying to backward through the conv + RNN stack a second time -- its saved "
                               "activations were freed by the first backward; run the forward again (retain_graph is not supported)")
        c2.defer_join = True
        r = _RnnStackFn.backward(c2, dout)
        rnn_grads = r[8 + 2 * L:]
        cg = _ConvStackFn.backward(c1, r[0])
        _join_side(*c2.pending)
        ctx.c1 = ctx.c2 = None
        return (None,) * 8 + tuple(cg[1:9]) + (None,) * (2 * L) + tuple(rnn_grads)


class _LookaheadFn(torch.autograd.Function):

    @staticmethod
    def forward(ctx, X, w, N, Tp):
        Ht, ctxlen = w.shape[0], w.shape[2]
        H = X.shape[1]
        wf = w.detach().reshape(Ht, ctxlen)
        if H != Ht:
            wf = torch.cat([wf, wf.new_zeros((H - Ht, ctxlen))], 0)
        wf = wf.contiguous()
        y, pre = ops.lookahead_fwd(X, wf, Tp, N, H)
        ctx.dims = (N, Tp, H, ctxlen, Ht)
        ctx.save_for_backward(X, wf, pre)
        return y

    @staticmethod
    def backward(ctx, dy):
        X, wf, pre = ctx.saved_tensors
        N, Tp, H, ctxlen, Ht = ctx.dims
        dx, dw = ops.lookahead_bwd(X, wf, pre, dy.contiguous().to(X.dtype), Tp, N, H)
        return dx, dw[:Ht].reshape(Ht, 1, ctxlen).contiguous(), None, None


class _HeadFn(torch.autograd.Function):

    @staticmethod
    def forward(ctx, X, bn_w, bn_b, wfc, mod, N, Tp, dtype, training):
        bn = mod.fc[0].module[0]
        Ht, Cc = wfc.shape[1], wfc.shape[0]
        H, Cp = mod._Hp, mod._Cp
        R = Tp * N
        c = mod._cache
        Xh = torch.empty_like(X)
        sv = _bn_seq_fwd(bn, bn_w, bn_b, X, Xh, R, Ht, H, training)
        Wp = c.get(("wfc", dtype), [wfc], lambda: _pad_cols(torch.cat(
            [wfc.detach(), torch.zeros(Cp - Cc, Ht, device=wfc.device)], 0), H).to(dtype).contiguous())
        logits = ops.gemm_nt(Xh, Wp, out_dtype=torch.float32)
        ctx.mod, ctx.dims, ctx.sv = mod, (N, Tp, dtype, H, Cc, Ht, Cp), sv
        ctx.save_for_backward(X, Xh, wfc)
        return logits

    @staticmethod
    def backward(ctx, dlogits):
        X, Xh, wfc = ctx.saved_tensors
        N, Tp, dtype, H, Cc, Ht, Cp = ctx.dims
        R = Tp * N
        c = ctx.mod._cache
        dl = dlogits.contiguous().to(dtype)
        WpT = c.get(("wfcT", dtype), [wfc], lambda: _pad_cols(torch.cat(
            [wfc.detach(), torch.zeros(Cp - Cc, Ht, device=wfc.device)], 0), H).t().to(dtype).contiguous())
        dXh = ops.gemm_nt(dl, WpT)
        dl_T, Xh_T = ops.transpose(dl), ops.transpose(Xh)
        dW = ops.gemm_nt_kslices(dl_T, Xh_T, max(1, min(32, R // 2048)))
        dX = torch.empty_like(dXh)
        dg, db = _bn_seq_bwd(dXh, X, dX, ctx.sv, R, Ht, H)
        return dX, dg, db, dW[:Cc, :Ht].contiguous(), None, None, None, None, None


class _CtcFn(torch.autograd.Function):

    @staticmethod
    def forward(ctx, logits, targets, out_lens_dev, target_sizes, N, Tp, Cc, blank):
        dev = logits.device
        tsz = target_sizes.to(torch.int64).cpu()
        offs = torch.zeros(N, dtype=torch.int64)
        if N > 1:
            offs[1:] = torch.cumsum(tsz, 0)[:-1]
        max_tl = int(tsz.max().item()) if N > 0 else 0
        tg = targets.cpu() if targets.is_cuda else targets
        parts = [offs.to(torch.int32).numpy(), tsz.to(torch.int32).numpy(), tg.reshape(-1).to(torch.int32).numpy()]
        meta = _CTC_STAGING.stage(dev, parts)
        loss, nll, dl = ops.ctc_loss_grad(logits, meta[2 * N:], meta[:N], out_lens_dev, meta[N:2 * N], Tp, N, Cc, blank, max_tl)
        ctx.save_for_backward(dl)
        ctx.consumed = False
        return loss.reshape(())

    @staticmethod
    def backward(ctx, g):
        (dl,) = ctx.saved_tensors
        if ctx.consumed:
            raise RuntimeError("DeepSpeech (gfx950): backward through the CTC loss a second time -- its gradient buffer was scaled in "
                               "place by the first backward; run the forward again (retain_graph is not supported)")
        ctx.consumed = True
        return ops.scale_by_(dl, g.detach().float()), None, None, None, None, None, None, None


class InferenceBatchSoftmax(nn.Module):
    def forward(self, input_):
        if self.training:
            return input_
        if not input_.is_cuda:
            raise Ds2HipError("InferenceBatchSoftmax (gfx950) needs a HIP tensor; there is no CPU fallback")
        x = input_.float().contiguous()
        return ops.softmax_rows(x.view(-1, x.shape[-1]), x.shape[-1]).view(x.shape)


class CTCLossHip(nn.Module):

    def __init__(self, blank=0):
        super().__init__()
        self.blank, self.reduction, self.zero_infinity = blank, "sum", True

    def forward(self, log_probs, targets, input_lengths, target_lengths):
        Tp, N, Cc = log_probs.shape
        if not log_probs.is_cuda:
            raise Ds2HipError("CTCLossHip needs a HIP tensor; there is no CPU fallback")
        x = torch.zeros((Tp * N, (Cc + 31) // 32 * 32), dtype=torch.float32, device=log_probs.device)
        x[:, :Cc] = log_probs.reshape(Tp * N, Cc).float()
        loss = _CtcFn.apply(x, targets, input_lengths.to(log_probs.device, torch.int32), target_lengths, N, Tp, Cc, self.blank)
        return loss


def _reference_metrics(decoder):
    try:
        from deepspeech_pytorch.validation import CharErrorRate, WordErrorRate
    except Exception:
        from .decoder import CharErrorRate, WordErrorRate
    return (WordErrorRate(decoder=decoder, target_decoder=decoder), CharErrorRate(decoder=decoder, target_decoder=decoder))


class DeepSpeech(_Base):
    def __init__(self, labels: List, model_cfg, precision, optim_cfg, spect_cfg):
        super().__init__()
        self.save_hyperparameters()
        self.model_cfg = model_cfg
        self.precision = precision
        self.optim_cfg = optim_cfg
        self.spect_cfg = spect_cfg
        self.bidirectional = _cfg_type_name(model_cfg) == "BiDirectionalConfig"
        self.labels = labels
        num_classes = len(self.labels)
        kind = rnn_kind(model_cfg.rnn_type)
        H, L = int(model_cfg.hidden_size), int(model_cfg.hidden_layers)
        if num_classes > 8192:
            raise ValueError("the CTC gradient kernel holds one row of per-class sums per wave in LDS: at most 8192 classes, got %d" % num_classes)
        self._Hp = _padded_hidden(H, kind, precision, self.bidirectional)
        self._Cp = (num_classes + 31) // 32 * 32

        self.conv = MaskConv(nn.Sequential(
            nn.Conv2d(1, 32, kernel_size=(41, 11), stride=(2, 2), padding=(20, 5)),
            nn.BatchNorm2d(32),
            nn.Hardtanh(0, 20, inplace=True),
            nn.Conv2d(32, 32, kernel_size=(21, 11), stride=(2, 1), padding=(10, 5)),
            nn.BatchNorm2d(32),
            nn.Hardtanh(0, 20, inplace=True)
        ))
        rnn_input_size = int(math.floor((self.spect_cfg.sample_rate * self.spect_cfg.window_size) / 2) + 1)
        rnn_input_size = int(math.floor(rnn_input_size + 2 * 20 - 41) / 2 + 1)
        rnn_input_size = int(math.floor(rnn_input_size + 2 * 10 - 21) / 2 + 1)
        rnn_input_size *= 32
        self._F0 = int(math.floor((self.spect_cfg.sample_rate * self.spect_cfg.window_size) / 2) + 1)
        self._F1, self._F2 = ops.conv_rows(self._F0)
        self._rnn_in, self._rnn_ld = 32 * self._F2, _round64(32 * self._F2)
        if rnn_input_size != self._rnn_in or self._F2 < 1:
            raise ValueError("unsupported spectrogram geometry: %d frequency bins" % self._F0)
        self.rnns = nn.Sequential(
            BatchRNN(rnn_input_size, H, kind, bidirectional=self.bidirectional, batch_norm=False),
            *(BatchRNN(H, H, kind, bidirectional=self.bidirectional) for _ in range(L - 1))
        )
        self.lookahead = nn.Sequential(
            Lookahead(H, context=model_cfg.lookahead_context),
            nn.Hardtanh(0, 20, inplace=True)
        ) if not self.bidirectional else None
        fully_connected = nn.Sequential(nn.BatchNorm1d(H), nn.Linear(H, num_classes, bias=False))
        self.fc = nn.Sequential(SequenceWise(fully_connected))
        self.blank_index = self.labels.index('_')
        from .decoder import GreedyDecoder
        self.inference_softmax = InferenceBatchSoftmax()
        self.criterion = CTCLossHip(blank=self.blank_index)
        self.evaluation_decoder = GreedyDecoder(self.labels, blank_index=self.blank_index)
        self.wer, self.cer = _reference_metrics(self.evaluation_decoder)
        self._cache = _WeightCache()
        self._flat_bias = {}
        self._side_streams = {}
        self._prep_done = None
        self._frame_rows = None
        self._weights_dirty = False
        self._kind = kind

    def _prep_rnn_weights(self, dtype, need_backward):
        c = self._cache
        if self._Hp != self.rnns[0].hidden_size:
            return
        for li, layer in enumerate(self.rnns):
            p, D, first = layer.rnn, layer.num_directions, li == 0
            sufs = [""] + (["_reverse"] if D == 2 else [])
            wih = [getattr(p, "weight_ih_l0" + s_) for s_ in sufs]
            whh = [getattr(p, "weight_hh_l0" + s_) for s_ in sufs]
            bih = [getattr(p, "bias_ih_l0" + s_) for s_ in sufs]
            bhh = [getattr(p, "bias_hh_l0" + s_) for s_ in sufs]

            if dtype == torch.bfloat16:
                keys = [("wih", li, dtype), ("whh", li, dtype)]
                if need_backward:
                    keys += [("wihT", li, dtype), ("whhT", li, dtype)]
                if not all(c.valid(k, wih if k[0].startswith("wih") else whh) for k in keys):
                    GH, H = whh[0].shape
                    I = wih[0].shape[1]
                    Io = self._rnn_ld if first else I
                    perm = (32, self._F2) if first else None
                    dev = wih[0].device
                    Wih = ops.empty_padded(D * GH, Io, dtype, dev)
                    Whh = torch.empty((D, GH, H), dtype=dtype, device=dev)
                    WihT = torch.empty((Io, D * GH), dtype=dtype, device=dev) if need_backward else None
                    WhhT = torch.empty((D, H, GH), dtype=dtype, device=dev) if need_backward else None
                    with torch.no_grad():
                        for d in range(D):
                            ops.cast_transpose_bf16(wih[d].detach(), Wih[d * GH:], Wih.stride(0),
                                                    WihT[:, d * GH:] if need_backward else None, D * GH, perm=perm, cout=Io)
                            ops.cast_transpose_bf16(whh[d].detach(), Whh[d], H, WhhT[d] if need_backward else None, GH)
                    c.put(("wih", li, dtype), wih, Wih)
                    c.put(("whh", li, dtype), whh, Whh)
                    if need_backward:
                        c.put(("wihT", li, dtype), wih, WihT)
                        c.put(("whhT", li, dtype), whh, WhhT)

            def cat_ih(wih=wih, first=first):
                w = torch.cat([q.detach() for q in wih], 0)
                return _perm_cols_to_internal(w) if first else w
            def padded_ih():
                w = cat_ih()
                out = ops.empty_padded(w.shape[0], w.shape[1], dtype, w.device)
                out.copy_(w)
                return out
            c.get(("wih", li, dtype), wih, padded_ih)
            c.get(("whh", li, dtype), whh, lambda whh=whh: torch.stack([q.detach() for q in whh], 0).to(dtype).contiguous())
            self._bias_views(li)
            if need_backward:
                c.get(("whhT", li, dtype), list(whh),
                      lambda whh=whh: torch.stack([q.detach().t() for q in whh], 0).to(dtype).contiguous())
                c.get(("wihT", li, dtype), list(wih), lambda: cat_ih().t().to(dtype).contiguous())

    def _bias_views(self, li):
        layer = self.rnns[li]
        p, D = layer.rnn, layer.num_directions
        sufs = [""] + (["_reverse"] if D == 2 else [])
        out = []
        for name in ("bias_ih_l0", "bias_hh_l0"):
            ps = [getattr(p, name + s_) for s_ in sufs]
            n = ps[0].numel()
            key = (li, name)
            flat = self._flat_bias.get(key)
            ok = flat is not None and all(q.data_ptr() == flat.data_ptr() + 4 * n * i and q.is_contiguous() for i, q in enumerate(ps))
            if not ok:
                with torch.no_grad():
                    flat = torch.cat([q.detach().reshape(-1) for q in ps]).contiguous()
                    for i, q in enumerate(ps):
                        q.data = flat[i * n:(i + 1) * n]
                self._flat_bias[key] = flat
            out.append(flat)
        return out[0], out[1].view(D, -1)

    def _prep_small_weights(self, dtype):
        c = self._cache
        sm, fcw = self.conv.seq_module, self.fc[0].module[1].weight
        w1, w2 = sm[0].weight, sm[3].weight
        keys = (("w1k", [w1]), (("w2t", dtype), [w2]), (("w2d", dtype), [w2]), (("wfc", dtype), [fcw]), (("wfcT", dtype), [fcw]))
        if all(c.valid(k, ps) for k, ps in keys[:3]) and (c.valid(*keys[3]) or fcw.shape[0] > 32 or self._Hp != fcw.shape[1]):
            return
        plain_head = fcw.shape[0] <= 32 and self._Hp == fcw.shape[1]
        with torch.no_grad():
            vals = ops.small_weight_layouts(w1.detach().contiguous(), w2.detach().contiguous(),
                                            fcw.detach().contiguous() if plain_head else fcw.detach()[:min(32, fcw.shape[0])].contiguous(), dtype)
        for (k, ps), v in zip(keys, vals):
            if plain_head or k[0] not in ("wfc", "wfcT"):
                c.put(k, ps, v)

    def _wgrad_stream(self, device):
        key = device.index if device.index is not None else torch.cuda.current_device()
        st = self._side_streams.get(key)
        if st is None:
            st = self._side_streams[key] = torch.cuda.Stream(device=device)
        return st

    def compute_dtype(self):
        if torch.is_autocast_enabled():
            return torch.bfloat16
        if str(self.precision) in ("16", "bf16", "16-mixed", "bf16-mixed"):
            return torch.bfloat16
        return torch.float32

    def _logits(self, x, lengths, hs=None):
        if not x.is_cuda:
            raise Ds2HipError("DeepSpeech (gfx950) needs its input on a HIP device; there is no CPU fallback")
        dtype = self.compute_dtype()
        if self.training:
            self._cache.epoch += 1
            self._weights_dirty = True
        elif self._weights_dirty:
            self._cache.epoch += 1
            self._weights_dirty = False
        lengths = lengths.cpu().int()
        output_lengths = self.get_seq_lens(lengths)
        N, T = x.shape[0], x.shape[3]
        Tp = (T + 2 * 5 - 10 - 1) // 2 + 1
        dev = x.device
        lens_dev, self._frame_rows = _frame_rows(output_lengths, Tp, N, dev)
        training = self.training
        sm = self.conv.seq_module
        with torch.autocast("cuda", enabled=False):
            self._prep_small_weights(dtype)
            if self._Hp == self.rnns[0].hidden_size:
                for li in range(len(self.rnns)):
                    self._bias_views(li)
            main, side = torch.cuda.current_stream(), self._wgrad_stream(dev)
            side.wait_stream(main)
            ready = getattr(self, "_layouts_ready", None)
            if ready is not None:
                side.wait_event(ready)
                self._layouts_ready = None
            with torch.cuda.stream(side):
                self._prep_rnn_weights(dtype, training and torch.is_grad_enabled())
            prep_done = torch.cuda.Event()
            prep_done.record(side)
            self._prep_done = prep_done
            L = len(self.rnns)
            if hs is None:
                hs = [None] * L
            h0s, c0s, params = [], [], []
            for i, layer in enumerate(self.rnns):
                h0 = c0 = None
                if hs[i] is not None:
                    if self._kind == "lstm":
                        h0, c0 = hs[i][0].float().contiguous(), hs[i][1].float().contiguous()
                    else:
                        h0 = hs[i].float().contiguous()
                h0s.append(h0)
                c0s.append(c0)
                if layer.batch_norm is not None:
                    bn = layer.batch_norm.module
                    params += [bn.weight, bn.bias]
                p = layer.rnn
                for suf in [""] + (["_reverse"] if self.bidirectional else []):
                    params += [getattr(p, "weight_ih_l0" + suf), getattr(p, "weight_hh_l0" + suf),
                               getattr(p, "bias_ih_l0" + suf), getattr(p, "bias_hh_l0" + suf)]
            Hh = self._Hp
            GH = ops.GATES[self._kind] * Hh
            Dd = 2 if self.bidirectional else 1
            fast_bwd = (ops.wgrad_tn_ok(dtype, Tp * N, Dd * GH, Hh, lda=Dd * GH, ldb=ops.pad_ld(Hh, dtype)) and
                        ops.wgrad_tn_ok(dtype, Tp * N, GH, Hh, lda=Dd * GH, ldb=Hh))
            composite = COMPOSITE_NODE if COMPOSITE_NODE is not None else (not fast_bwd and not _data_parallel_active())
            if any(h is not None for h in h0s) and torch.is_grad_enabled():
                composite = False
            if composite:
                res = _FrontFn.apply(x, self, lens_dev, N, Tp, dtype, training, L, sm[0].weight, sm[0].bias, sm[1].weight, sm[1].bias,
                                     sm[3].weight, sm[3].bias, sm[4].weight, sm[4].bias, *h0s, *c0s, *params)
                X = res[0]
                hn_l = list(res[1:1 + L])
                cn_l = list(res[1 + L:1 + 2 * L]) if self._kind == "lstm" else []
            else:
                X = _ConvStackFn.apply(x, sm[0].weight, sm[0].bias, sm[1].weight, sm[1].bias, sm[3].weight, sm[3].bias, sm[4].weight,
                                       sm[4].bias, self, lens_dev, Tp, dtype, training)
                if self._prep_done is not None:
                    torch.cuda.current_stream().wait_event(self._prep_done)
                    self._prep_done = None
                hn_l, cn_l, pos = [], [], 0
                for i, layer in enumerate(self.rnns):
                    n = _layer_param_count(layer)
                    outs = _RnnLayerFn.apply(X, self, lens_dev, N, Tp, dtype, training, i, h0s[i], c0s[i], *params[pos:pos + n])
                    pos += n
                    X = outs[0]
                    hn_l.append(outs[1])
                    if len(outs) > 2:
                        cn_l.append(outs[2])
            if self._kind == "lstm":
                new_hs = [(hn_l[i], cn_l[i]) for i in range(L)]
            else:
                new_hs = list(hn_l)
            if not self.bidirectional:
                X = _LookaheadFn.apply(X, self.lookahead[0].conv.weight, N, Tp)
            fcm = self.fc[0].module
            logits = _HeadFn.apply(X, fcm[0].weight, fcm[0].bias, fcm[1].weight, self, N, Tp, dtype, training)
        return logits, output_lengths, new_hs, lens_dev, N, Tp

    def forward(self, x, lengths, hs=None):
        logits, output_lengths, new_hs, _, N, Tp = self._logits(x, lengths, hs)
        Cc = len(self.labels)
        if self.training:
            out = logits.view(Tp, N, self._Cp)[:, :, :Cc].transpose(0, 1)
        else:
            out = ops.softmax_rows(logits, Cc).view(Tp, N, Cc).transpose(0, 1)
        return out, output_lengths, new_hs

    def training_step(self, batch, batch_idx):
        inputs, targets, input_percentages, target_sizes = batch
        if inputs.is_cuda:
            ops.poll_persistent_error(inputs.device)
        input_sizes = input_percentages.mul_(int(inputs.size(3))).int()
        logits, output_sizes, _, lens_dev, N, Tp = self._logits(inputs, input_sizes)
        return _CtcFn.apply(logits, targets, lens_dev, target_sizes, N, Tp, len(self.labels), self.blank_index)

    def validation_step(self, batch, batch_idx):
        inputs, targets, input_percentages, target_sizes = batch
        input_sizes = input_percentages.mul_(int(inputs.size(3))).int()
        inputs = inputs.to(self.device)
        with torch.autocast("cuda", dtype=torch.bfloat16, enabled=str(self.precision) in ("16", "bf16", "16-mixed", "bf16-mixed")):
            out, output_sizes, hs = self(inputs, input_sizes)
        decoded_output, _ = self.evaluation_decoder.decode(out, output_sizes)
        self.wer(preds=out, preds_sizes=output_sizes, targets=targets, target_sizes=target_sizes)
        self.cer(preds=out, preds_sizes=output_sizes, targets=targets, target_sizes=target_sizes)
        self.log('wer', self.wer.compute(), prog_bar=True, on_epoch=True)
        self.log('cer', self.cer.compute(), prog_bar=True, on_epoch=True)

    def attach_evaluation(self, decoder, wer=None, cer=None):
        self.evaluation_decoder = decoder
        if wer is not None:
            self.wer = wer
        if cer is not None:
            self.cer = cer

    def configure_optimizers(self):
        from .optim import FusedAdamW, FusedSGD
        name = _cfg_type_name(self.optim_cfg)
        on_gpu = all(p.is_cuda for p in self.parameters())
        if name == "SGDConfig":
            kw = dict(params=self.parameters(), lr=self.optim_cfg.learning_rate, momentum=self.optim_cfg.momentum, nesterov=True,
                      weight_decay=self.optim_cfg.weight_decay)
            optimizer = FusedSGD(model=self, **kw) if on_gpu else torch.optim.SGD(**kw)
        elif name == "AdamConfig":
            kw = dict(params=self.parameters(), lr=self.optim_cfg.learning_rate, betas=tuple(self.optim_cfg.betas),
                      eps=self.optim_cfg.eps, weight_decay=self.optim_cfg.weight_decay)
            optimizer = FusedAdamW(model=self, **kw) if on_gpu else torch.optim.AdamW(**kw)
        else:
            raise ValueError("Optimizer has not been specified correctly.")
        scheduler = torch.optim.lr_scheduler.ExponentialLR(optimizer=optimizer, gamma=self.optim_cfg.learning_anneal)
        return [optimizer], [scheduler]

    def get_seq_lens(self, input_length):
        seq_len = input_length
        for m in self.conv.modules():
            if type(m) == nn.modules.conv.Conv2d:
                seq_len = ((seq_len + 2 * m.padding[1] - m.dilation[1] * (m.kernel_size[1] - 1) - 1) // m.stride[1] + 1)
        return seq_len.int()
```

### deepspeech/pytorch_amd/ops.py

```python
import ctypes as C

import numpy as np
import torch

from . import _lib
from ._lib import F32, BF16, call, query

CELLS = {"gru": _lib.CELL_GRU, "lstm": _lib.CELL_LSTM, "rnn": _lib.CELL_RNN_TANH}
GATES = {"gru": 3, "lstm": 4, "rnn": 1}
SAVED_PLANES = {"gru": 4, "lstm": 5, "rnn": 0}


def dt(t):
    d = t if isinstance(t, torch.dtype) else t.dtype
    if d == torch.float32:
        return F32
    if d == torch.bfloat16:
        return BF16
    raise TypeError("ds2hip supports float32 and bfloat16 activations, got %s" % d)


def vecw(dtype):
    return 4 if dtype == torch.float32 else 8


def P(t):
    if t is None:
        return C.c_void_p(0)
    if not t.is_cuda:
        raise _lib.Ds2HipError("ds2hip ops need CUDA(HIP) tensors; got a %s tensor -- there is no CPU fallback" % t.device)
    return C.c_void_p(t.data_ptr())


def PF(t):
    if t is not None and t.dtype != torch.float32:
        raise _lib.Ds2HipError("ds2hip kernels keep parameters, BatchNorm statistics and carried states in float32 (bf16 is an "
                               "activation/operand type selected by `precision`/autocast); got %s" % t.dtype)
    return P(t)


def S():
    return C.c_void_p(torch.cuda.current_stream().cuda_stream)


def rup(x, m):
    return (x + m - 1) // m * m


SWEEP_EVENTS = None


class _sweep_timer:
    def __init__(self, tag, launches):
        self.tag, self.launches = tag, launches

    def __enter__(self):
        if SWEEP_EVENTS is not None:
            self.e0 = torch.cuda.Event(enable_timing=True)
            self.e1 = torch.cuda.Event(enable_timing=True)
            self.e0.record()
        return self

    def __exit__(self, *exc):
        if SWEEP_EVENTS is not None:
            self.e1.record()
            SWEEP_EVENTS.append((self.tag, self.launches, self.e0, self.e1))
        return False


def pad_ld(n, dtype=torch.bfloat16):
    esz = 2 if dtype == torch.bfloat16 else 4
    return n + 64 if (n * esz) % 1024 == 0 else n


def empty_padded(rows, cols, dtype, device):
    ld = pad_ld(cols, dtype)
    return torch.empty((rows, ld), dtype=dtype, device=device)[:, :cols] if ld != cols else torch.empty((rows, cols), dtype=dtype, device=device)


GEMM8_ENABLED = True


def gemm8_nt_shape_ok(dtype, M, N, K, lda, ldb):
    return (GEMM8_ENABLED and dtype == torch.bfloat16 and K % 64 == 0 and lda % 8 == 0 and ldb % 8 == 0 and
            M >= 1024 and N >= 256 and rup(M, 256) // 256 * (rup(N, 256) // 256) >= 160 and M * lda < (1 << 31) and N * ldb < (1 << 31))


def gemm8_nt_ok(A, B, M, N, K, lda, ldb):
    return (A.dtype == B.dtype and gemm8_nt_shape_ok(A.dtype, M, N, K, lda, ldb) and
            A.data_ptr() % 16 == 0 and B.data_ptr() % 16 == 0)


def wgrad_tn_ok(dtype, R, M, N, lda=None, ldb=None):
    lda = M if lda is None else lda
    ldb = N if ldb is None else ldb
    return (GEMM8_ENABLED and dtype == torch.bfloat16 and R >= 512 and M % 8 == 0 and N % 8 == 0 and M >= 256 and N >= 256 and
            R * lda < (1 << 31) and R * ldb < (1 << 31))


def zero_pad_rows(X, lens, Tp, N):
    call("ds2_zero_pad_rows", dt(X), P(X), X.stride(0), X.shape[1], P(lens), Tp, N, S())
    return X


def gemm_nt(A, B, bias=None, out_dtype=None, M=None, N=None, K=None, lda=None, ldb=None, out=None, ldc=None, splitk=1,
            batch=1, sA=0, sB=0, sC=0, sBias=0, coresident=False, rows=None, zero_pad=None):
    M = A.shape[-2] if M is None else M
    N = B.shape[-2] if N is None else N
    K = A.shape[-1] if K is None else K
    lda = A.stride(-2) if lda is None else lda
    ldb = B.stride(-2) if ldb is None else ldb
    out_dtype = out_dtype or A.dtype
    if out is None and splitk == 1 and batch == 1 and not coresident and gemm8_nt_ok(A, B, M, N, K, lda, ldb):
        res = gemm8_nt(A, B, bias=bias, out_dtype=out_dtype, M=M, N=N, K=K, lda=lda, ldb=ldb, rows=rows)
        if rows is not None and zero_pad is not None:
            zero_pad_rows(res, *zero_pad)
        return res
    ks = fp32_ksplit(A.dtype, M, N, K) if (out is None and splitk == 1 and batch == 1 and not coresident and bias is None and
                                            out_dtype == torch.float32 and A.dtype == torch.float32) else 1
    if ks > 1:
        Ks = K // ks
        ws = torch.empty((ks, M, N), dtype=torch.float32, device=A.device)
        call("ds2_gemm_nt", dt(A), P(A), P(B), P(ws), None, M, N, Ks, lda, ldb, N, 1, ks, Ks, Ks, M * N, 0, 1, S())
        out = torch.empty((M, N), dtype=torch.float32, device=A.device)
        call("ds2_sum_slices", P(ws), P(out), M * N, ks, S())
        if rows is not None and zero_pad is not None:
            zero_pad_rows(out, *zero_pad)
        return out
    if out is None:
        shape = (batch, M, N) if batch > 1 else (M, N)
        out = torch.empty(shape, dtype=out_dtype, device=A.device)
        ldc = N
        sC = M * N
    out_f32 = 1 if out.dtype == torch.float32 else 0
    call("ds2_gemm_nt_coresident" if coresident else "ds2_gemm_nt", dt(A), P(A), P(B), P(out), PF(bias), M, N, K, lda, ldb, ldc,
         out_f32, batch, sA, sB, sC, sBias, splitk, S())
    if rows is not None and zero_pad is not None and batch == 1:
        zero_pad_rows(out, *zero_pad)
    return out


def gemm_nt_kslices(A, B, slices):
    M, K = A.shape[-2], A.shape[-1]
    N = B.shape[-2]
    lda, ldb = A.stride(-2), B.stride(-2)
    nkt = K // 64
    for s_ in range(slices, max(1, slices // 2), -1):
        if nkt % s_ == 0 and K % 64 == 0:
            slices = s_
            break
    Ks = (K // max(slices, 1)) // 64 * 64
    if slices <= 1 or Ks == 0 or (M * N) % 4 != 0:
        return gemm_nt(A, B, out_dtype=torch.float32)
    rest = K - slices * Ks
    ws = torch.empty((slices + (1 if rest else 0), M, N), dtype=torch.float32, device=A.device)
    call("ds2_gemm_nt", dt(A), P(A), P(B), P(ws), None, M, N, Ks, lda, ldb, N, 1, slices, Ks, Ks, M * N, 0, 1, S())
    if rest:
        call("ds2_gemm_nt", dt(A), P(A[:, slices * Ks:]), P(B[:, slices * Ks:]), P(ws[slices]), None, M, N, rest, lda, ldb, N, 1, 1,
             0, 0, 0, 0, 1, S())
    out = torch.empty((M, N), dtype=torch.float32, device=A.device)
    call("ds2_sum_slices", P(ws), P(out), M * N, ws.shape[0], S())
    return out


FP32_KSPLIT = __import__("os").environ.get("DS2_FP32_KSPLIT", "1") != "0"


def fp32_ksplit(dtype, M, N, K):
    if not FP32_KSPLIT or dtype != torch.float32 or K % 32 != 0 or (M * N) % 4 != 0:
        return 1
    tiles = ((M + 127) // 128) * ((N + 127) // 128)
    nkt = K // 32
    if tiles >= 128 or nkt < 32:
        return 1
    want = min(8, max(1, 256 // tiles))
    for s_ in range(want, 1, -1):
        if nkt % s_ == 0 and nkt // s_ >= 8:
            return s_
    return 1


def gemm_nt_rows2(A, A2, m_split, B, M, N, K, lda, ldb, splitk=1, coresident=False):
    out = torch.empty((M, N), dtype=torch.float32, device=A.device)
    call("ds2_gemm_nt_rows2", dt(A), P(A), P(A2), m_split, P(B), P(out), M, N, K, lda, ldb, N, 1, splitk, 1 if coresident else 0, S())
    return out


def gemm8_nt(A, B, bias=None, out_dtype=None, M=None, N=None, K=None, lda=None, ldb=None, rows=None):
    M = A.shape[-2] if M is None else M
    N = B.shape[-2] if N is None else N
    K = A.shape[-1] if K is None else K
    lda = A.stride(-2) if lda is None else lda
    ldb = B.stride(-2) if ldb is None else ldb
    out = torch.empty((M, N), dtype=out_dtype or A.dtype, device=A.device)
    if rows is not None:
        call("ds2_gemm8_nt_rows", P(A), P(B), P(out), PF(bias), M, N, K, lda, ldb, N, 1 if out.dtype == torch.float32 else 0, P(rows),
             rows.numel(), S())
        return out
    call("ds2_gemm8_nt", P(A), P(B), P(out), PF(bias), M, N, K, lda, ldb, N, 1 if out.dtype == torch.float32 else 0, S())
    return out


def gemm8_tn_grouped(problems, K, dx=None, rows=None, zero_pad=None):
    rp, nr = (P(rows), rows.numel()) if rows is not None else (None, 0)
    n = len(problems)
    outs = []
    for pr in problems:
        o = pr.get("out")
        if o is None:
            o = torch.empty((pr["M"], pr["N"]), dtype=torch.float32, device=pr["At"].device)
        outs.append(o)
    vp = C.c_void_p * n
    ia, la = C.c_int * n, C.c_long * n
    At = vp(*[pr["At"].data_ptr() for pr in problems])
    At2 = vp(*[(pr["At2"].data_ptr() if pr.get("At2") is not None else 0) for pr in problems])
    ms = ia(*[int(pr.get("m_split", 0)) for pr in problems])
    Bt = vp(*[pr["Bt"].data_ptr() for pr in problems])
    Cs = vp(*[o.data_ptr() for o in outs])
    Ms, Ns = ia(*[pr["M"] for pr in problems]), ia(*[pr["N"] for pr in problems])
    lda, ldb = la(*[pr["lda"] for pr in problems]), la(*[pr["ldb"] for pr in problems])
    lda2 = la(*[int(pr.get("lda2", 0)) for pr in problems])
    ldc = la(*[o.stride(0) for o in outs])
    for pr in problems:
        P(pr["At"]), P(pr["Bt"])
    if dx is not None:
        A, B = dx
        Mx, Nx, Kx = A.shape[0], B.shape[0], A.shape[1]
        out_x = torch.empty((Mx, Nx), dtype=A.dtype, device=A.device)
        call("ds2_gemm8_wgrad_dx_rows", n, At, At2, ms, Bt, Cs, Ms, Ns, lda, lda2, ldb, ldc, K, P(A), P(B), P(out_x), Mx, Nx, Kx, A.stride(0),
             B.stride(0), Nx, rp, nr, S())
        if rows is not None and zero_pad is not None:
            zero_pad_rows(out_x, *zero_pad)
        return outs, out_x
    call("ds2_gemm8_tn_grouped_rows", n, At, At2, ms, Bt, Cs, Ms, Ns, lda, lda2, ldb, ldc, K, rp, nr, S())
    return outs


def colsum(X, R=None, Cc=None, ld=None, scale=1.0):
    R = X.shape[0] if R is None else R
    Cc = X.shape[1] if Cc is None else Cc
    ld = X.stride(0) if ld is None else ld
    out = torch.empty(Cc, dtype=torch.float32, device=X.device)
    ws = torch.empty(query("ds2_norm_partials", R) * Cc, dtype=torch.float32, device=X.device)
    call("ds2_colsum", dt(X), P(X), R, Cc, ld, P(out), float(scale), P(ws), S())
    return out


import os as _os
FP32_GEMM_MODE = _os.environ.get("DS2_FP32_GEMM", "wgrad")
FP32_SPLIT3 = FP32_GEMM_MODE != "exact"


def split3_ok(dtype, M, N, K, leaf=False):
    if dtype != torch.float32 or FP32_GEMM_MODE == "exact" or not (M >= 256 and N >= 256 and K >= 256):
        return False
    return leaf or FP32_GEMM_MODE == "split3"


def split3(X, mode, out=None):
    rows, K = X.shape
    Kp = rup(K, 64)
    if out is None:
        out = torch.empty((rows, 3 * Kp), dtype=torch.bfloat16, device=X.device)
    assert out.shape[0] == rows and out.shape[1] == 3 * Kp and X.dtype == torch.float32 and X.stride(1) == 1
    call("ds2_split3_bf16", P(X), X.stride(0), rows, K, Kp, mode, P(out), out.stride(0), S())
    return out


def split3_rows(X, mode):
    rows, K = X.shape
    K8 = rup(K, 8)
    out = torch.empty((3 * rows, K8), dtype=torch.bfloat16, device=X.device)
    assert X.dtype == torch.float32 and X.stride(1) == 1
    call("ds2_split3_bf16", P(X), X.stride(0), rows, K, K8, 2 + mode, P(out), K8, S())
    return out


def transpose(X, R=None, Cc=None, lds=None):
    R = X.shape[0] if R is None else R
    Cc = X.shape[1] if Cc is None else Cc
    lds = X.stride(0) if lds is None else lds
    ldd = rup(R, 64)
    out = torch.empty((Cc, ldd), dtype=X.dtype, device=X.device)
    call("ds2_transpose", dt(X), P(X), P(out), R, Cc, lds, ldd, S())
    return out


def cast_transpose_bf16(src, dst=None, ldd=0, dstT=None, lddT=0, perm=None, cout=None):
    R, Cc = src.shape
    pc, pf = perm if perm is not None else (0, 0)
    call("ds2_cast_transpose_bf16", PF(src), src.stride(0), R, Cc, pc, pf, Cc if cout is None else cout,
         P(dst) if dst is not None else None, ldd, P(dstT) if dstT is not None else None, lddT, S())


def small_weight_layouts(w1, w2, wfc, dtype):
    dev, Cc, H = w1.device, wfc.shape[0], wfc.shape[1]
    w1k = torch.empty((451, 32), dtype=torch.float32, device=dev)
    w2t = torch.empty((21, 11, 32, 32), dtype=dtype, device=dev)
    w2d0 = torch.empty((11, 11, 32, 32), dtype=dtype, device=dev)
    w2d1 = torch.empty((10, 11, 32, 32), dtype=dtype, device=dev)
    wp = torch.empty((32, H), dtype=dtype, device=dev)
    wpT = torch.empty((H, 32), dtype=dtype, device=dev)
    call("ds2_small_weight_layouts", dt(dtype), PF(w1), PF(w2), PF(wfc), Cc, H, P(w1k), P(w2t), P(w2d0), P(w2d1), P(wp), P(wpT), S())
    return w1k, w2t, [w2d0, w2d1], wp, wpT


def scale_by_(x, s):
    call("ds2_scale_by", P(x), PF(s.reshape(1)), x.numel(), S())
    return x


def add2(a, b):
    out = torch.empty_like(a)
    call("ds2_add2", dt(a), P(a), P(b), P(out), a.numel(), S())
    return out


class BnSaved:
    __slots__ = ("mean", "rstd", "scale", "shift")

    def __init__(self, Cc, device):
        buf = torch.empty((4, Cc), dtype=torch.float32, device=device)
        self.mean, self.rstd, self.scale, self.shift = buf[0], buf[1], buf[2], buf[3]


def bn_fwd(X, mode, training, gamma, beta, rmean, rvar, nbt, R, Cc, ldx, Y, ldy, F=0, Tp=0, N=0, lens=None, eps=1e-5,
           momentum=0.1):
    sv = BnSaved(Cc, X.device)
    ws = torch.empty(2 * query("ds2_norm_partials", R) * Cc, dtype=torch.float32, device=X.device)
    call("ds2_bn_fwd", dt(X), mode, 1 if training else 0, P(X), P(Y), R, Cc, ldx, ldy, F, Tp, N, P(lens), PF(gamma), PF(beta),
         PF(rmean), PF(rvar), P(nbt) if training else C.c_void_p(0), float(eps), float(momentum), P(sv.mean), P(sv.rstd),
         P(sv.scale), P(sv.shift), P(ws), S())
    return sv


def bn_bwd(G, X, DX, mode, sv, R, Cc, ldg, ldx, lddx, F=0, Tp=0, N=0, lens=None):
    dgamma = torch.empty(Cc, dtype=torch.float32, device=X.device)
    dbeta = torch.empty(Cc, dtype=torch.float32, device=X.device)
    ws = torch.empty((2 * query("ds2_norm_partials", R) + 2) * Cc, dtype=torch.float32, device=X.device)
    call("ds2_bn_bwd", dt(X), mode, P(G), P(X), P(DX), R, Cc, ldg, ldx, lddx, F, Tp, N, P(lens), P(sv.mean), P(sv.rstd),
         P(sv.scale), P(sv.shift), P(dgamma), P(dbeta), P(ws), S())
    return dgamma, dbeta


def conv_rows(F0):
    F1 = (F0 + 2 * 20 - 41) // 2 + 1
    return F1, (F1 + 2 * 10 - 21) // 2 + 1


def conv1_fwd(x, w1k, b1, lens, Tp, dtype):
    N, _, F0, T = x.shape
    y1 = torch.empty((N, conv_rows(F0)[0], Tp, 32), dtype=dtype, device=x.device)
    call("ds2_conv1_fwd", dt(dtype), PF(x), PF(w1k), PF(b1), P(lens), P(y1), N, F0, T, Tp, S())
    return y1


def conv1_wgrad(x, dy1, Tp):
    N, _, F0, T = x.shape
    dw = torch.empty((451, 32), dtype=torch.float32, device=x.device)
    ws = torch.empty(query("ds2_conv1_wgrad_ws_floats", N, F0, Tp), dtype=torch.float32, device=x.device)
    call("ds2_conv1_wgrad", dt(dy1), P(x), P(dy1), P(dw), N, F0, T, Tp, P(ws), S())
    return dw


def conv2_fwd(a1, w2t, b2, lens, F0=161):
    N, F1, Tp, _ = a1.shape
    assert F1 == conv_rows(F0)[0]
    y2 = torch.empty((N, conv_rows(F0)[1], Tp, 32), dtype=a1.dtype, device=a1.device)
    nws = query("ds2_conv2_fwd_ws_bytes", dt(a1), N, F0, Tp)
    ws = torch.empty(nws, dtype=torch.uint8, device=a1.device) if nws else None
    call("ds2_conv2_fwd", dt(a1), P(a1), P(w2t), PF(b2), P(lens), P(y2), N, F0, Tp, P(ws), S())
    return y2


def conv2_dgrad(dy2, w2d_even, w2d_odd, F0=161):
    N, F2, Tp, _ = dy2.shape
    assert F2 == conv_rows(F0)[1]
    da1 = torch.empty((N, conv_rows(F0)[0], Tp, 32), dtype=dy2.dtype, device=dy2.device)
    call("ds2_conv2_dgrad", dt(dy2), P(dy2), P(w2d_even), P(w2d_odd), P(da1), N, F0, Tp, S())
    return da1


def conv2_wgrad(dy2, a1, F0=161):
    N, _, Tp, _ = dy2.shape
    dw = torch.empty((231, 32, 32), dtype=torch.float32, device=dy2.device)
    ws = torch.empty(query("ds2_conv2_wgrad_ws_floats", N, Tp), dtype=torch.float32, device=dy2.device)
    call("ds2_conv2_wgrad", dt(dy2), P(dy2), P(a1), P(dw), N, F0, Tp, P(ws), S())
    return dw


_PERSIST_ERR = {}
LAST_PERSIST_WS = None

STARTUP_MS_SINGLE = 300
STARTUP_MS_DP_MIN, STARTUP_MS_DP_MAX = 30_000, 3_600_000
_OPTS = {"variant": 0, "spin_limit": 0, "startup_ms": None}
FORCE_DATA_PARALLEL_BUDGET = [False]


class persist_options:

    def __init__(self, **kw):
        assert set(kw) <= set(_OPTS), kw
        self.kw = kw

    def __enter__(self):
        self.old = dict(_OPTS)
        _OPTS.update(self.kw)
        return self

    def __exit__(self, *exc):
        _OPTS.clear()
        _OPTS.update(self.old)
        return False


def data_parallel_ranks():
    try:
        import torch.distributed as _dist
        if _dist.is_available() and _dist.is_initialized():
            return int(_dist.get_world_size())
    except Exception:
        pass
    return 1


def persist_startup_ms():
    if _OPTS["startup_ms"] is not None:
        return int(_OPTS["startup_ms"])
    env = _os.environ.get("DS2_PERSIST_STARTUP_MS", "")
    if env:
        return max(1, int(env))
    if data_parallel_ranks() > 1 or FORCE_DATA_PARALLEL_BUDGET[0]:
        ms = 600_000
        try:
            import torch.distributed as _dist
            from torch.distributed.distributed_c10d import _get_default_group
            if _dist.is_initialized():
                to = getattr(_get_default_group(), "_timeout", None) or getattr(_dist, "default_pg_timeout", None)
                if to is not None:
                    ms = int(to.total_seconds() * 1000)
        except Exception:
            pass
        return min(max(ms, STARTUP_MS_DP_MIN), STARTUP_MS_DP_MAX)
    return STARTUP_MS_SINGLE


def _persist_opts():
    o = _lib.PersistOpts(int(_OPTS["variant"]), int(_OPTS["spin_limit"]), persist_startup_ms())
    return o


def persist_kind(dtype, kind, D, N, H):
    return query("ds2_rnn_persist_kind", dt(dtype), CELLS[kind], D, N, H, int(_OPTS["variant"]))


def _persist_err(dev):
    key = dev.index if dev.index is not None else torch.cuda.current_device()
    t = _PERSIST_ERR.get(key)
    if t is None:
        t = _PERSIST_ERR[key] = torch.zeros(16, dtype=torch.int32, device=dev)
    return t


def _persist_error_message(code, key):
    if code == 2:
        return ("a persistent recurrent sweep on device %d could not start: its workgroups never became co-resident within its start-up "
                "budget (%.1f s now; 0.3 s single-process, the process group's time-out under data parallelism, DS2_PERSIST_STARTUP_MS "
                "overrides) -- another kernel holds compute units (a second process on this GPU, e.g. a validation job or two ranks with "
                "the same LOCAL_RANK; or a long-running kernel on another stream).  The sweep gave up, its outputs were NaN-poisoned"
                % (key, persist_startup_ms() / 1000.0))
    return ("a persistent recurrent kernel timed out on device %d waiting for its peer workgroups in the middle of a sweep "
            "(are other kernels occupying CUs?); its outputs were NaN-poisoned" % key)


def check_persistent_kernels():
    for key, t in _PERSIST_ERR.items():
        code = int(t[0].item())
        if code != 0:
            raise _lib.Ds2HipError(_persist_error_message(code, key))


_ERR_MIRROR = {}


def poll_persistent_error(dev):
    key = dev.index if dev.index is not None else torch.cuda.current_device()
    t = _PERSIST_ERR.get(key)
    if t is None:
        return
    m = _ERR_MIRROR.get(key)
    if m is None:
        m = _ERR_MIRROR[key] = [torch.zeros(1, dtype=torch.int32).pin_memory(), None]
    if m[1] is not None:
        if not m[1].query():
            return
        m[1] = None
        if int(m[0][0]) != 0:
            raise _lib.Ds2HipError(_persist_error_message(int(m[0][0]), key))
    call("ds2_copy_words", P(t), C.c_void_p(m[0].data_ptr()), 1, S())
    ev = torch.cuda.Event()
    ev.record()
    m[1] = ev


class PinnedRing:

    def __init__(self, depth=32):
        self.depth = depth
        self._per_device = {}
        self._lock = __import__("threading").Lock()

    class _RingState:
        def __init__(self):
            self.cap, self.buf, self.events, self.i = 0, None, None, 0

    def stage(self, dev, parts):
        n = int(sum(p.size for p in parts))
        dev = torch.device(dev)
        if dev.type != "cuda":
            return torch.from_numpy(np.concatenate([np.asarray(p, dtype=np.int32).reshape(-1) for p in parts]) if parts else np.zeros(0, np.int32))
        key = dev.index if dev.index is not None else torch.cuda.current_device()
        with self._lock, torch.cuda.device(key):
            st = self._per_device.setdefault(key, PinnedRing._RingState())
            if st.buf is None or n > st.cap:
                if st.events is not None:
                    for e in st.events:
                        if e is not None:
                            e.synchronize()
                st.cap = max(1024, 1 << (max(n, 1) - 1).bit_length())
                st.buf = torch.empty(self.depth * st.cap, dtype=torch.int32, pin_memory=True)
                st.events = [None] * self.depth
                st.i = 0
            k = st.i
            st.i = (k + 1) % self.depth
            if st.events[k] is not None and not st.events[k].query():
                st.events[k].synchronize()
            slot = st.buf[k * st.cap:k * st.cap + n]
            hv = slot.numpy()
            o = 0
            for p in parts:
                hv[o:o + p.size] = np.asarray(p).reshape(-1)
                o += p.size
            out = torch.empty(n, dtype=torch.int32, device=torch.device("cuda", key))
            if n:
                dptr = _pinned_device_ptr(slot)
                if dptr is not None:
                    call("ds2_copy_words", C.c_void_p(dptr), P(out), n, S())
                else:
                    out.copy_(slot, non_blocking=True)
            if st.events[k] is None:
                st.events[k] = torch.cuda.Event()
            st.events[k].record()
            return out


_HIPRT = []


def _pinned_device_ptr(t):
    if not _HIPRT:
        try:
            lib = C.CDLL("libamdhip64.so")
            lib.hipHostGetDevicePointer.restype = C.c_int
            lib.hipHostGetDevicePointer.argtypes = [C.POINTER(C.c_void_p), C.c_void_p, C.c_uint]
            _HIPRT.append(lib)
        except OSError:
            _HIPRT.append(None)
    lib = _HIPRT[0]
    if lib is None:
        return t.data_ptr()
    dp = C.c_void_p(0)
    rc = lib.hipHostGetDevicePointer(C.byref(dp), C.c_void_p(t.data_ptr()), 0)
    return dp.value if rc == 0 and dp.value else None


POISON_UNWRITTEN = False
PERSIST_ENABLED = True


_WARNED_CUS = set()
_WARNED_SHAPES = set()
PERSIST_CLIFF_MIN_H = 256


def use_persistent(kind, dtype, D, N, H):
    if not PERSIST_ENABLED:
        return False
    ok = bool(query("ds2_rnn_persist_supported", dt(dtype), CELLS[kind], D, N, H, int(_OPTS["variant"])))
    if ok:
        return True
    import os
    import warnings
    covered = bool(query("ds2_rnn_persist_shape_covered", dt(dtype), CELLS[kind], D, N, H))
    if covered:
        dev = torch.cuda.current_device()
        cus = torch.cuda.get_device_properties(dev).multi_processor_count
        if os.environ.get("DS2_ALLOW_LAUNCH_PER_STEP", "0") in ("", "0"):
            raise _lib.Ds2HipError("ds2hip: device %d exposes %d compute units (< 256): the persistent recurrent kernels need one "
                                   "workgroup per CU, all co-resident.  Set DS2_ALLOW_LAUNCH_PER_STEP=1 to run the launch-per-time-step "
                                   "kernels instead (several times slower)." % (dev, cus))
        if dev not in _WARNED_CUS:
            _WARNED_CUS.add(dev)
            warnings.warn("ds2hip: device %d exposes %d compute units (< 256): the persistent recurrent kernels are disabled, the "
                          "recurrent sweeps use one launch per time step" % (dev, cus))
    elif H >= PERSIST_CLIFF_MIN_H:
        key = (kind, str(dtype), D, N, H)
        if key not in _WARNED_SHAPES:
            _WARNED_SHAPES.add(key)
            widths = [w for w in range(16, 2049, 16) if query("ds2_rnn_persist_shape_covered", dt(dtype), CELLS[kind], D, N, w)]
            warnings.warn("ds2hip: no persistent recurrent kernel is instantiated for %s %s hidden=%d, %d direction(s), batch %d: the "
                          "sweeps run one launch per time step (5-8x slower per step).  For this cell, type, direction count and batch "
                          "persistent kernels exist with hidden in {%s}; the model class zero-pads other hidden sizes up to the nearest "
                          "instantiated width when that is at most 1.5x as wide (DS2_PAD_HIDDEN)."
                          % (str(dtype).replace("torch.", ""), kind, H, D, N, ", ".join(map(str, widths))))
    return False


def rnn_fwd(kind, GI, Whh, bhh, lens, D, N, H, Tp, h0=None, c0=None, save=True):
    dev, dtype = GI.device, GI.dtype
    hext = torch.empty((D, Tp + 2, N, H), dtype=dtype, device=dev)
    persistent = use_persistent(kind, dtype, D, N, H)
    if not persistent:
        hext[:, 0].zero_()
        hext[:, Tp + 1].zero_()
    ns = SAVED_PLANES[kind]
    Sv = torch.empty((D, Tp, N, max(ns, 1) * H) if ns else (1,), dtype=dtype, device=dev)
    hn = torch.empty((D, N, H), dtype=torch.float32, device=dev)
    cn = torch.empty((D, N, H), dtype=torch.float32, device=dev) if kind == "lstm" else None
    if persistent:
        ws = torch.empty(query("ds2_rnn_persist_ws_bytes", dt(dtype), CELLS[kind], D, N, H, int(_OPTS["variant"])), dtype=torch.uint8, device=dev)
        global LAST_PERSIST_WS
        LAST_PERSIST_WS = ws
        po = _persist_opts()
        with _sweep_timer("rnn_fwd_persistent", Tp):
            call("ds2_rnn_persist_fwd", dt(dtype), CELLS[kind], D, N, H, Tp, P(lens), P(GI), P(Whh), PF(bhh), PF(h0), PF(c0),
                 P(hext[:, 1]), (Tp + 2) * N * H, P(Sv), P(hn), P(cn), P(ws), P(_persist_err(dev)), C.byref(po), S())
        return hext, Sv, hn, cn
    state = torch.empty(query("ds2_rnn_state_bytes", D, N, H), dtype=torch.uint8, device=dev)
    with _sweep_timer("rnn_fwd", Tp):
        call("ds2_rnn_fwd", dt(dtype), CELLS[kind], D, N, H, Tp, P(lens), P(GI), P(Whh), PF(bhh), PF(h0), PF(c0),
             P(hext[:, 1]), (Tp + 2) * N * H, P(Sv), P(hn), P(cn), P(state), S())
    return hext, Sv, hn, cn


class RnnGrads:
    __slots__ = ("dGI", "dGH", "dQ", "bacc", "dh0", "dc0")

    def __init__(self, dGI, dGH=None, dQ=None, bacc=None):
        self.dGI, self.dGH, self.dQ, self.bacc = dGI, dGH, dQ, bacc
        self.dh0 = self.dc0 = None

    def tensors(self):
        return [t for t in (self.dGI, self.dGH, self.dQ, self.bacc) if t is not None]


def rnn_bwd(kind, dOut, WhhT, hext, Sv, lens, D, N, H, Tp, pad_rows_unread=False, h0=None, c0=None, want_dstate=False):
    dev, dtype = dOut.device, dOut.dtype
    G = GATES[kind]
    dGI = torch.empty((Tp * N, D * G * H), dtype=dtype, device=dev)
    with_state = h0 is not None or c0 is not None or want_dstate
    if not with_state and use_persistent(kind, dtype, D, N, H):
        dQ = torch.empty((D, Tp, N, H), dtype=dtype, device=dev) if kind == "gru" else None
        if POISON_UNWRITTEN:
            dGI.fill_(float("nan"))
            if dQ is not None:
                dQ.fill_(float("nan"))
        bacc = torch.empty((D, N, (4 if kind == "gru" else G) * H), dtype=torch.float32, device=dev)
        ws = torch.empty(query("ds2_rnn_persist_ws_bytes", dt(dtype), CELLS[kind], D, N, H, int(_OPTS["variant"])), dtype=torch.uint8, device=dev)
        global LAST_PERSIST_WS
        LAST_PERSIST_WS = ws
        po = _persist_opts()
        with _sweep_timer("rnn_bwd_persistent", Tp):
            call("ds2_rnn_persist_bwd", dt(dtype), CELLS[kind], D, N, H, Tp, P(lens), P(dOut), P(WhhT), P(hext[:, 1]), (Tp + 2) * N * H,
                 P(Sv), P(dGI), P(dQ), P(bacc), 1 if pad_rows_unread else 0, P(ws), P(_persist_err(dev)), C.byref(po), S())
        return RnnGrads(dGI, dQ=dQ, bacc=bacc)
    dGH = torch.empty((D, Tp, N, G * H), dtype=dtype, device=dev) if kind == "gru" else None
    state = torch.empty(query("ds2_rnn_state_bytes", D, N, H), dtype=torch.uint8, device=dev)
    dh0 = torch.empty((D, N, H), dtype=torch.float32, device=dev) if want_dstate else None
    dc0 = torch.empty((D, N, H), dtype=torch.float32, device=dev) if (want_dstate and kind == "lstm") else None
    with _sweep_timer("rnn_bwd", Tp):
        call("ds2_rnn_bwd", dt(dtype), CELLS[kind], D, N, H, Tp, P(lens), P(dOut), P(WhhT), P(hext[:, 1]), (Tp + 2) * N * H,
             P(Sv), P(dGI), P(dGH), PF(h0), PF(c0), P(dh0), P(dc0), P(state), S())
    rg = RnnGrads(dGI, dGH=dGH)
    rg.dh0, rg.dc0 = dh0, dc0
    return rg


def rnn_bias_grads(kind, bacc, D, N, H):
    G = GATES[kind]
    dbih = torch.empty(D * G * H, dtype=torch.float32, device=bacc.device)
    dbhh = torch.empty((D, G * H), dtype=torch.float32, device=bacc.device)
    call("ds2_rnn_bias_grads", CELLS[kind], D, N, H, PF(bacc), P(dbih), P(dbhh), S())
    return dbih, dbhh


def lookahead_fwd(x, w, Tp, N, H, save=True):
    y = torch.empty_like(x)
    pre = torch.empty_like(x) if save else None
    call("ds2_lookahead_fwd", dt(x), P(x), PF(w), P(y), P(pre), Tp, N, H, w.shape[1], S())
    return y, pre


def lookahead_bwd(x, w, pre, dy, Tp, N, H):
    ctx = w.shape[1]
    dx = torch.empty_like(x)
    dw = torch.empty((H, ctx), dtype=torch.float32, device=x.device)
    ws = torch.empty(query("ds2_lookahead_ws_floats", Tp, N, H, ctx), dtype=torch.float32, device=x.device)
    call("ds2_lookahead_bwd", dt(x), P(x), P(w), P(pre), P(dy), P(dx), P(dw), Tp, N, H, ctx, P(ws), S())
    return dx, dw


def softmax_rows(logits, Cc):
    rows = logits.shape[0]
    out = torch.empty((rows, Cc), dtype=torch.float32, device=logits.device)
    call("ds2_softmax_rows", P(logits), P(out), rows, Cc, logits.stride(0), Cc, S())
    return out


def greedy_decode(scores, sizes, blank):
    if scores.dtype != torch.float32:
        scores = scores.float()
    if scores.stride(2) != 1:
        scores = scores.contiguous()
    N, T, Cc = scores.shape
    dev = scores.device
    sz = sizes.to(dev, torch.int32) if sizes is not None else None
    buf = torch.empty((2, N, T), dtype=torch.int32, device=dev)
    counts = torch.empty(N, dtype=torch.int32, device=dev)
    call("ds2_greedy_decode", P(scores), scores.stride(0), scores.stride(1), N, T, Cc, P(sz), blank, P(buf[0]), P(buf[1]), P(counts),
         S())
    cnt = counts.cpu()
    width = int(cnt.max().item()) if N > 0 else 0
    host = buf[:, :, :max(width, 1)].cpu()
    toks = [host[0, i, :int(cnt[i])].tolist() for i in range(N)]
    offs = [host[1, i, :int(cnt[i])] for i in range(N)]
    return toks, offs


BEAM_MAX_WIDTH, BEAM_MAX_TOP_N, BEAM_MAX_CLASSES = 256, 64, 8192


def beam_decode(probs, sizes, blank, beam_width, cutoff_top_n, cutoff_prob):
    N, T, Cc = probs.shape
    B, top_n = int(beam_width), int(cutoff_top_n)
    if not 1 <= B <= BEAM_MAX_WIDTH:
        raise ValueError("beam_width must be in [1, %d], got %d" % (BEAM_MAX_WIDTH, B))
    if top_n < 1 or min(top_n, Cc) > BEAM_MAX_TOP_N:
        raise ValueError("min(cutoff_top_n, number of classes) must be in [1, %d], got cutoff_top_n=%d with %d classes"
                         % (BEAM_MAX_TOP_N, top_n, Cc))
    if not 1 <= Cc <= BEAM_MAX_CLASSES:
        raise ValueError("the beam decoder supports up to %d classes, got %d" % (BEAM_MAX_CLASSES, Cc))
    if not 0 <= blank < Cc:
        raise ValueError("blank index %d out of range for %d classes" % (blank, Cc))
    if N == 0 or T == 0:
        scores = torch.full((N, B), float("inf"))
        scores[:, 0] = 0.0
        return [[[] for _ in range(B)] for _ in range(N)], \
            [[torch.zeros(0, dtype=torch.int32) for _ in range(B)] for _ in range(N)], scores
    if probs.dtype != torch.float32:
        probs = probs.float()
    if probs.stride(2) != 1:
        probs = probs.contiguous()
    dev = probs.device
    sz = sizes.to(dev, torch.int32) if sizes is not None else None
    buf = torch.empty((2, N, B, T), dtype=torch.int32, device=dev)
    lens = torch.empty((N, B), dtype=torch.int32, device=dev)
    scores = torch.empty((N, B), dtype=torch.float32, device=dev)
    ws = torch.empty(query("ds2_beam_ws_bytes", N, T, B), dtype=torch.uint8, device=dev)
    call("ds2_beam_decode", P(probs), probs.stride(0), probs.stride(1), N, T, Cc, P(sz), int(blank), B, top_n, float(cutoff_prob),
         P(buf[0]), P(buf[1]), P(lens), P(scores), P(ws), S())
    ln = lens.cpu().numpy()
    width = max(int(ln.max()), 1)
    host = buf[:, :, :, :width].cpu().numpy()
    toks = [[host[0, n, b, :ln[n, b]].tolist() for b in range(B)] for n in range(N)]
    offs = [[torch.from_numpy(host[1, n, b, :ln[n, b]]) for b in range(B)] for n in range(N)]
    return toks, offs, scores.cpu()


BEAM_LM_MAX_ORDER = 5


def beam_decode_lm(probs, sizes, blank, beam_width, cutoff_top_n, cutoff_prob, space, word_table, ngram_table, order, bos,
                   alpha, beta, lexicon=True):
    B, top_n = _beam_lm_checks(probs, beam_width, cutoff_top_n, blank, space, word_table, ngram_table, order, bos)
    N, T, Cc = probs.shape
    if N == 0 or T == 0:
        scores = torch.full((N, B), float("inf"))
        scores[:, 0] = 0.0
        return [[[] for _ in range(B)] for _ in range(N)], \
            [[torch.zeros(0, dtype=torch.int32) for _ in range(B)] for _ in range(N)], scores, scores.clone()
    if probs.dtype != torch.float32:
        probs = probs.float()
    if probs.stride(2) != 1:
        probs = probs.contiguous()
    dev = probs.device
    sz = sizes.to(dev, torch.int32) if sizes is not None else None
    buf = torch.empty((2, N, B, T), dtype=torch.int32, device=dev)
    lens = torch.empty((N, B), dtype=torch.int32, device=dev)
    scores = torch.empty((2, N, B), dtype=torch.float32, device=dev)
    ws = torch.empty(query("ds2_beam_ws_bytes", N, T, B), dtype=torch.uint8, device=dev)
    call("ds2_beam_decode_lm", P(probs), probs.stride(0), probs.stride(1), N, T, Cc, P(sz), int(blank), B, top_n, float(cutoff_prob),
         int(space), P(word_table), word_table.shape[0], P(ngram_table), ngram_table.shape[0], int(order), int(bos), float(alpha),
         float(beta), int(bool(lexicon)), P(buf[0]), P(buf[1]), P(lens), P(scores[0]), P(scores[1]), P(ws), S())
    ln = lens.cpu().numpy()
    width = max(int(ln.max()), 1)
    host = buf[:, :, :, :width].cpu().numpy()
    toks = [[host[0, n, b, :ln[n, b]].tolist() for b in range(B)] for n in range(N)]
    offs = [[torch.from_numpy(host[1, n, b, :ln[n, b]]) for b in range(B)] for n in range(N)]
    sc = scores.cpu()
    return toks, offs, sc[0], sc[1]


def _beam_lm_checks(probs, beam_width, cutoff_top_n, blank, space, word_table, ngram_table, order, bos):
    N, T, Cc = probs.shape
    B, top_n = int(beam_width), int(cutoff_top_n)
    if not 1 <= B <= BEAM_MAX_WIDTH:
        raise ValueError("beam_width must be in [1, %d], got %d" % (BEAM_MAX_WIDTH, B))
    if top_n < 1 or min(top_n, Cc) > BEAM_MAX_TOP_N:
        raise ValueError("min(cutoff_top_n, number of classes) must be in [1, %d], got cutoff_top_n=%d with %d classes"
                         % (BEAM_MAX_TOP_N, top_n, Cc))
    if not 1 <= Cc <= BEAM_MAX_CLASSES:
        raise ValueError("the beam decoder supports up to %d classes, got %d" % (BEAM_MAX_CLASSES, Cc))
    if not 0 <= blank < Cc:
        raise ValueError("blank index %d out of range for %d classes" % (blank, Cc))
    if not 0 <= space < Cc or space == blank:
        raise ValueError("space label %d must be one of the %d classes and differ from the blank (%d)" % (space, Cc, blank))
    if not 1 <= int(order) <= BEAM_LM_MAX_ORDER:
        raise ValueError("language-model order must be in [1, %d], got %d" % (BEAM_LM_MAX_ORDER, order))
    if bos < 0:
        raise ValueError("the id of <s> must not be negative, got %d" % bos)
    for name, t in (("word_table", word_table), ("ngram_table", ngram_table)):
        if not (torch.is_tensor(t) and t.dtype == torch.int64 and t.dim() == 2 and t.shape[1] == 2 and t.is_contiguous()):
            raise ValueError("%s must be a contiguous int64 tensor of shape (slots, 2)" % name)
        if t.shape[0] < 2 or t.shape[0] & (t.shape[0] - 1):
            raise ValueError("%s: the number of slots must be a power of two >= 2, got %d" % (name, t.shape[0]))
        if t.device != probs.device or not t.is_cuda:
            raise ValueError("%s must live on the device of the probabilities (%s), not %s" % (name, probs.device, t.device))
    return B, top_n


BEAM_GRID_MAX_POINTS = 65535


def plan_grid_chunks(G, bytes_one, bytes_per_point, max_ws_bytes, max_points=BEAM_GRID_MAX_POINTS):
    G, bytes_one, bytes_per_point, max_ws_bytes = int(G), int(bytes_one), int(bytes_per_point), int(max_ws_bytes)
    if G < 1:
        raise ValueError("the grid needs at least one point, got %d" % G)
    if bytes_one > max_ws_bytes:
        raise ValueError("max_ws_bytes=%d is below the workspace of a single point (%d bytes)" % (max_ws_bytes, bytes_one))
    per = max_points if bytes_per_point <= 0 else min(max_points, 1 + (max_ws_bytes - bytes_one) // bytes_per_point)
    return [(g, min(per, G - g)) for g in range(0, G, per)]


def _weights(name, w, dev):
    t = torch.as_tensor(w, dtype=torch.float32)
    if t.dim() != 1:
        raise ValueError("%s must be a one-dimensional sequence of floats, got shape %s" % (name, tuple(t.shape)))
    return t.to(dev).contiguous()


def beam_decode_lm_grid(probs, sizes, blank, beam_width, cutoff_top_n, cutoff_prob, space, word_table, ngram_table, order, bos,
                        alphas, betas, lexicon=True, max_ws_bytes=1 << 30):
    B, top_n = _beam_lm_checks(probs, beam_width, cutoff_top_n, blank, space, word_table, ngram_table, order, bos)
    if not probs.is_cuda:
        raise ValueError("probs must be a HIP device tensor")
    N, T, Cc = probs.shape
    dev = probs.device
    al, be = _weights("alphas", alphas, dev), _weights("betas", betas, dev)
    G = al.shape[0]
    if G < 1 or be.shape[0] != G:
        raise ValueError("alphas and betas must have the same length >= 1, got %d and %d" % (G, be.shape[0]))
    buf = torch.zeros((2, G, N, T), dtype=torch.int32, device=dev)
    lens = torch.zeros((G, N), dtype=torch.int32, device=dev)
    scores = torch.zeros((2, G, N), dtype=torch.float32, device=dev)
    if N == 0 or T == 0:
        return buf[0], buf[1], lens, scores[0], scores[1]
    one = query("ds2_beam_grid_ws_bytes", 1, N, T, B)
    chunks = plan_grid_chunks(G, one, query("ds2_beam_grid_ws_bytes", 2, N, T, B) - one, max_ws_bytes)
    if probs.dtype != torch.float32:
        probs = probs.float()
    if probs.stride(2) != 1:
        probs = probs.contiguous()
    sz = sizes.to(dev, torch.int32) if sizes is not None else None
    ws = torch.empty(query("ds2_beam_grid_ws_bytes", max(c for _, c in chunks), N, T, B), dtype=torch.uint8, device=dev)
    for g0, cnt in chunks:
        g1 = g0 + cnt
        call("ds2_beam_decode_lm_grid", P(probs), probs.stride(0), probs.stride(1), N, T, Cc, P(sz), int(blank), B, top_n,
             float(cutoff_prob), int(space), P(word_table), word_table.shape[0], P(ngram_table), ngram_table.shape[0], int(order),
             int(bos), int(bool(lexicon)), cnt, P(al[g0:g1]), P(be[g0:g1]), P(buf[0, g0:g1]), P(buf[1, g0:g1]), P(lens[g0:g1]),
             P(scores[0, g0:g1]), P(scores[1, g0:g1]), P(ws), S())
    return buf[0], buf[1], lens, scores[0], scores[1]


ERROR_COUNTS_MAX_LEN = 4096


def error_counts(hyp, hyp_lens, targets, target_sizes, space):
    if not (torch.is_tensor(hyp) and hyp.is_cuda and hyp.dim() >= 1):
        raise ValueError("hyp must be a HIP device tensor of label rows")
    dev = hyp.device
    L = hyp.shape[-1]
    hyp = hyp.to(torch.int32).reshape(-1, L).contiguous()
    P_ = hyp.shape[0]
    hl = torch.as_tensor(hyp_lens).to(dev, torch.int32).reshape(-1).contiguous()
    if hl.shape[0] != P_:
        raise ValueError("hyp_lens has %d entries for %d hypotheses" % (hl.shape[0], P_))
    ts = torch.as_tensor(target_sizes).reshape(-1)
    R = ts.shape[0]
    if R < 1 or P_ < R or P_ % R:
        raise ValueError("the number of hypotheses (%d) must be a positive multiple of the number of references (%d)" % (P_, R))
    longest_ref = int(ts.max()) if R else 0
    if longest_ref > ERROR_COUNTS_MAX_LEN or int(ts.min()) < 0:
        raise ValueError("a reference has %d labels; error_counts takes 0 to %d" % (longest_ref, ERROR_COUNTS_MAX_LEN))
    if L > ERROR_COUNTS_MAX_LEN:
        longest = int(hl.max())
        if longest > ERROR_COUNTS_MAX_LEN:
            raise ValueError("a hypothesis has %d labels; error_counts takes up to %d" % (longest, ERROR_COUNTS_MAX_LEN))
    tg = torch.as_tensor(targets).to(dev, torch.int32).reshape(-1).contiguous()
    offs = torch.zeros(R + 1, dtype=torch.int32, device=dev)
    offs[1:] = torch.cumsum(ts.to(dev, torch.int64), 0)
    if int(ts.sum()) > tg.shape[0]:
        raise ValueError("target_sizes add up to %d labels, targets has %d" % (int(ts.sum()), tg.shape[0]))
    out = torch.empty(2 * P_ + 2 * R, dtype=torch.int32, device=dev)
    ce, we, rc, rw = out[:P_], out[P_:2 * P_], out[2 * P_:2 * P_ + R], out[2 * P_ + R:]
    call("ds2_error_counts", P(hyp), L, P(hl), P_, P(tg), P(offs), R, int(space), P(ce), P(we), P(rc), P(rw), S())
    return ce, we, rc, rw


SPEC_AUGMENT_MAX_MASKS = 4


def _aug_batch(x, frames):
    if not (torch.is_tensor(x) and x.is_cuda and x.dim() == 4 and x.shape[1] == 1 and x.dtype == torch.float32):
        raise ValueError("spec_augment takes a float32 HIP device batch of shape (N, 1, F, Tmax)")
    fr = torch.as_tensor(frames).to(x.device, torch.int32).reshape(-1).contiguous()
    if fr.shape[0] != x.shape[0]:
        raise ValueError("frames has %d entries for %d clips" % (fr.shape[0], x.shape[0]))
    return x.contiguous(), fr


def aug_masks(m, N, dev, what):
    if m is None:
        return None, 0
    m = torch.as_tensor(m)
    if m.dim() != 3 or m.shape[0] != N or m.shape[2] != 2:
        raise ValueError("%s must have shape (N, masks, 2) = [start, width] per mask; got %s" % (what, tuple(m.shape)))
    if m.shape[1] > SPEC_AUGMENT_MAX_MASKS:
        raise ValueError("%s holds %d masks per clip; the kernels take up to %d" % (what, m.shape[1], SPEC_AUGMENT_MAX_MASKS))
    if m.shape[1] == 0:
        return None, 0
    return m.to(dev, torch.int32).contiguous(), m.shape[1]


def spec_augment_coef(x, frames, warp_draw, W=5):
    x, fr = _aug_batch(x, frames)
    N, _, F, Tmax = x.shape
    wd = torch.as_tensor(warp_draw).to(x.device, torch.float32).contiguous()
    if tuple(wd.shape) != (N, 12):
        raise ValueError("warp_draw must have shape (N, 12); got %s" % (tuple(wd.shape),))
    coef = torch.empty((N, 3), dtype=torch.float32, device=x.device)
    call("ds2_spec_augment_coef", P(x), N, F, Tmax, P(fr), P(wd), int(W), P(coef), S())
    return coef


def spec_augment(x, frames, coef, fmask, tmask):
    x, fr = _aug_batch(x, frames)
    N, _, F, Tmax = x.shape
    coef = torch.as_tensor(coef).to(x.device, torch.float32).contiguous()
    if tuple(coef.shape) != (N, 3):
        raise ValueError("coef must have shape (N, 3); got %s" % (tuple(coef.shape),))
    fm, MF = aug_masks(fmask, N, x.device, "fmask")
    tm, MT = aug_masks(tmask, N, x.device, "tmask")
    out = torch.empty_like(x)
    call("ds2_spec_augment", P(x), P(out), N, F, Tmax, P(fr), P(coef), P(fm), MF, P(tm), MT, S())
    return out


CTC_RECURSION = 0


def ctc_loss_grad(logits, targets_i32, target_offsets, input_lengths, target_lengths, Tp, N, Cc, blank, max_target_len,
                  ldg=None, recursion=None):
    dev = logits.device
    ldg = logits.shape[1] if ldg is None else ldg
    nll = torch.empty(N, dtype=torch.float32, device=dev)
    loss = torch.empty(1, dtype=torch.float32, device=dev)
    dlogits = torch.empty((Tp * N, ldg), dtype=torch.float32, device=dev)
    ws = torch.empty(query("ds2_ctc_ws_floats", Tp, N, Cc, max_target_len), dtype=torch.float32, device=dev)
    call("ds2_ctc_loss_grad", P(logits), logits.stride(0), P(targets_i32), P(target_offsets), P(input_lengths),
         P(target_lengths), Tp, N, Cc, blank, max_target_len, 1.0, P(nll), P(loss), P(dlogits), ldg, P(ws),
         int(CTC_RECURSION if recursion is None else recursion), S())
    return loss, nll, dlogits
```

### include/ds2hip.h

```cpp
#ifndef DS2HIP_H
#define DS2HIP_H

#include <stdint.h>

#ifdef __cplusplus
extern "C" {
#endif

typedef void* ds2_stream_t;

enum { DS2_F32 = 0, DS2_BF16 = 1 };
enum { DS2_CELL_GRU = 0, DS2_CELL_LSTM = 1, DS2_CELL_RNN_TANH = 2 };
enum {
  DS2_OK = 0,
  DS2_ERR_DTYPE = 1001,
  DS2_ERR_ARG = 1002,
  DS2_ERR_ALIGN = 1003
};

int ds2_version(void);
const char* ds2_error_string(int code);

int ds2_gemm_nt(int dtype, const void* A, const void* B, void* C, const float* bias, int M, int N, int K, long lda, long ldb,
                long ldc, int out_f32, int batch, long strideA, long strideB, long strideC, long strideBias, int splitk,
                ds2_stream_t stream);

int ds2_gemm_nt_rows2(int dtype, const void* A, const void* A2, int m_split, const void* B, void* C, int M, int N, int K, long lda,
                      long ldb, long ldc, int out_f32, int splitk, int coresident, ds2_stream_t stream);
int ds2_gemm_nt_coresident(int dtype, const void* A, const void* B, void* C, const float* bias, int M, int N, int K, long lda,
                           long ldb, long ldc, int out_f32, int batch, long strideA, long strideB, long strideC, long strideBias,
                           int splitk, ds2_stream_t stream);

int ds2_gemm8_nt(const void* A, const void* B, void* C, const float* bias, int M, int N, int K, long lda, long ldb, long ldc, int out_f32,
                 ds2_stream_t stream);
int ds2_gemm8_tn_grouped(int n_problems, const void* const* At, const void* const* At2, const int* m_split, const void* const* Bt, void* const* C,
                         const int* M, const int* N, const long* lda, const long* lda2, const long* ldb, const long* ldc, int K, ds2_stream_t stream);

int ds2_gemm8_wgrad_dx(int n_tn, const void* const* At, const void* const* At2, const int* m_split, const void* const* Bt, void* const* C,
                       const int* M, const int* N, const long* lda, const long* lda2, const long* ldb, const long* ldc, int K_tn,
                       const void* A_nt, const void* B_nt, void* C_nt, int M_nt, int N_nt, int K_nt, long lda_nt, long ldb_nt, long ldc_nt,
                       ds2_stream_t stream);

int ds2_gemm8_nt_rows(const void* A, const void* B, void* C, const float* bias, int n_phys, int N, int K, long lda, long ldb, long ldc,
                      int out_f32, const int* rows, int n_rows, ds2_stream_t stream);
int ds2_gemm8_tn_grouped_rows(int n_problems, const void* const* At, const void* const* At2, const int* m_split, const void* const* Bt,
                              void* const* C, const int* M, const int* N, const long* lda, const long* lda2, const long* ldb, const long* ldc,
                              int n_phys, const int* rows, int n_rows, ds2_stream_t stream);
int ds2_gemm8_wgrad_dx_rows(int n_tn, const void* const* At, const void* const* At2, const int* m_split, const void* const* Bt, void* const* C,
                            const int* M, const int* N, const long* lda, const long* lda2, const long* ldb, const long* ldc, int K_tn,
                            const void* A_nt, const void* B_nt, void* C_nt, int M_nt, int N_nt, int K_nt, long lda_nt, long ldb_nt, long ldc_nt,
                            const int* rows, int n_rows, ds2_stream_t stream);
int ds2_zero_pad_rows(int dtype, void* X, long ld, int cols, const int* lens, int Tp, int N, ds2_stream_t stream);

int ds2_norm_partials(long R);
int ds2_bn_fwd(int dtype, int mode, int training, const void* X, void* Y, long R, int C, long ldx, long ldy, int F, int Tp,
               int N, const int* lens, const float* gamma, const float* beta, float* running_mean, float* running_var,
               long long* num_batches_tracked, float eps, float momentum, float* save_mean, float* save_rstd,
               float* save_scale, float* save_shift, float* ws, ds2_stream_t stream);
int ds2_bn_bwd(int dtype, int mode, const void* G, const void* X, void* DX, long R, int C, long ldg, long ldx, long lddx,
               int F, int Tp, int N, const int* lens, const float* save_mean, const float* save_rstd,
               const float* save_scale, const float* save_shift, float* dgamma, float* dbeta, float* ws,
               ds2_stream_t stream);
int ds2_colsum(int dtype, const void* X, long R, int C, long ld, float* out, float scale, float* ws, ds2_stream_t stream);

int ds2_conv_rows(int F0, int* F1, int* F2);
int ds2_conv1_fwd(int dtype, const float* x, const float* w1k, const float* b1, const int* lens, void* y1, int N, int F0, int T,
                  int Tp, ds2_stream_t stream);
long ds2_conv1_wgrad_ws_floats(int N, int F0, int Tp);
int ds2_conv1_wgrad(int dtype, const float* x, const void* dy1, float* dw1k, int N, int F0, int T, int Tp, float* ws,
                    ds2_stream_t stream);
long ds2_conv2_fwd_ws_bytes(int dtype, int N, int F0, int Tp);
int ds2_conv2_fwd(int dtype, const void* a1, const void* w2t, const float* b2, const int* lens, void* y2, int N, int F0, int Tp,
                  void* ws, ds2_stream_t stream);
int ds2_conv2_dgrad(int dtype, const void* dy2, const void* w2d_even, const void* w2d_odd, void* da1, int N, int F0, int Tp,
                    ds2_stream_t stream);
long ds2_conv2_wgrad_ws_floats(int N, int Tp);
int ds2_conv2_wgrad(int dtype, const void* dy2, const void* a1, float* dw2t, int N, int F0, int Tp, float* ws, ds2_stream_t stream);

int ds2_rnn_gates(int cell);
int ds2_rnn_saved_planes(int cell);
long ds2_rnn_state_bytes(int D, int N, int H);
int ds2_rnn_fwd(int dtype, int cell, int D, int N, int H, int Tp, const int* lens, const void* GI, const void* Whh,
                const float* bhh, const float* h0, const float* c0, void* Hseq, long hseq_dstride, void* S, float* hn, float* cn,
                void* state, ds2_stream_t stream);
int ds2_rnn_bwd(int dtype, int cell, int D, int N, int H, int Tp, const int* lens, const void* dOut, const void* WhhT,
                const void* Hseq, long hseq_dstride, const void* S, void* dGI, void* dGH, const float* h0, const float* c0,
                float* dh0, float* dc0, void* state, ds2_stream_t stream);

typedef struct ds2_persist_opts {
  unsigned variant;
  unsigned spin_limit;
  unsigned startup_ms;
} ds2_persist_opts;
int ds2_rnn_persist_plan(int dtype, int cell, int D, int N, int H, int cus, unsigned variant, long* ws_bytes);
int ds2_rnn_persist_supported(int dtype, int cell, int D, int N, int H, unsigned variant);
int ds2_rnn_persist_shape_covered(int dtype, int cell, int D, int N, int H);
int ds2_rnn_persist_kind(int dtype, int cell, int D, int N, int H, unsigned variant);
long ds2_rnn_persist_ws_bytes(int dtype, int cell, int D, int N, int H, unsigned variant);
int ds2_rnn_persist_fwd(int dtype, int cell, int D, int N, int H, int Tp, const int* lens, const void* GI, const void* Whh,
                        const float* bhh, const float* h0, const float* c0, void* Hseq, long hseq_dstride, void* S, float* hn,
                        float* cn, void* ws, int* err, const ds2_persist_opts* opts, ds2_stream_t stream);
int ds2_rnn_persist_bwd(int dtype, int cell, int D, int N, int H, int Tp, const int* lens, const void* dOut, const void* WhhT,
                        const void* Hseq, long hseq_dstride, const void* S, void* dGI, void* dQ, float* dBacc, int flags, void* ws,
                        int* err, const ds2_persist_opts* opts, ds2_stream_t stream);

int ds2_add2(int dtype, const void* a, const void* b, void* out, long n, ds2_stream_t stream);
int ds2_sum_slices(const float* src, float* out, long n, int slices, ds2_stream_t stream);
int ds2_transpose(int dtype, const void* src, void* dst, long R, int C, long lds, long ldd, ds2_stream_t stream);
int ds2_split3_bf16(const float* src, long lds, long rows, int K, int Kp, int mode, void* dst, long ldd, ds2_stream_t stream);
int ds2_cast_transpose_bf16(const float* src, long lds, int R, int C, int perm_c, int perm_f, int Cout, void* dst, long ldd,
                            void* dstT, long lddT, ds2_stream_t stream);
int ds2_small_weight_layouts(int dtype, const float* w1, const float* w2, const float* wfc, int C, int H, float* w1k, void* w2t,
                             void* w2d0, void* w2d1, void* wfcp, void* wfcT, ds2_stream_t stream);
int ds2_scale_by(float* x, const float* s, long n, ds2_stream_t stream);

int ds2_copy_words(const void* src, void* dst, long n_words, ds2_stream_t stream);
int ds2_lookahead_fwd(int dtype, const void* x, const float* w, void* y, void* pre, int Tp, int N, int H, int ctx,
                      ds2_stream_t stream);
long ds2_lookahead_ws_floats(int Tp, int N, int H, int ctx);
int ds2_lookahead_bwd(int dtype, const void* x, const float* w, const void* pre, const void* dy, void* dx, float* dw, int Tp,
                      int N, int H, int ctx, float* ws, ds2_stream_t stream);
int ds2_rnn_bias_grads(int cell, int D, int N, int H, const float* dBacc, float* dbih, float* dbhh, ds2_stream_t stream);

int ds2_softmax_rows(const float* logits, float* probs, long rows, int C, long ld_in, long ld_out, ds2_stream_t stream);

long ds2_ctc_ws_floats(int Tp, int N, int C, int max_target_len);
int ds2_ctc_loss_grad(const float* logits, long ldl, const int* targets, const int* target_offsets, const int* input_lengths,
                      const int* target_lengths, int Tp, int N, int C, int blank, int max_target_len, float grad_scale,
                      float* nll, float* loss_sum, float* dlogits, long ldg, float* ws, int recursion, ds2_stream_t stream);

int ds2_opt_max_tensors(void);
long ds2_clip_ws_floats(int count, const long* n);
int ds2_clip_coef(int count, const float* const* g, const long* n, float max_norm, float* out, float* ws, ds2_stream_t stream);
int ds2_opt_multi(int mode, int count, float* const* p, const float* const* g, float* const* m, float* const* v, const long* n,
                  const float* hp, int first, const float* clip, ds2_stream_t stream);
int ds2_opt_matrix(int mode, float* p, const float* g, float* m, float* v, int R, int C, int perm_c, int perm_f, int Cout,
                   void* dst, long ldd, void* dstT, long lddT, const float* hp, int first, const float* clip, ds2_stream_t stream);
int ds2_opt_matrices(int mode, int count, float* const* p, const float* const* g, float* const* m, float* const* v, const int* R,
                     const int* C, const int* perm_c, const int* perm_f, const int* Cout, void* const* dst, const long* ldd,
                     void* const* dstT, const long* lddT, const float* hp, int first, const float* clip, ds2_stream_t stream);

int ds2_spect_frames(int nsamples);
long ds2_spect_ws_bytes(int N, int Lmax);
int ds2_spectrogram(const float* wav, long ldw, const int* nsamples, int N, int Lmax, const float* basis, int reflect,
                    int normalize, float* out, void* ws, ds2_stream_t stream);

int ds2_spectrogram_aug(const float* wav, long ldw, const int* nsamples, int N, int Lmax, const float* basis, int reflect,
                        int normalize, float* out, void* ws, const float* warp_draw, int W, const int* fmask, int MF,
                        const int* tmask, int MT, float* coef_out, ds2_stream_t stream);
int ds2_spec_augment_coef(const float* x, int N, int F, int Tmax, const int* frames, const float* warp_draw, int W, float* coef,
                          ds2_stream_t stream);
int ds2_spec_augment(const float* in, float* out, int N, int F, int Tmax, const int* frames, const float* coef, const int* fmask,
                     int MF, const int* tmask, int MT, ds2_stream_t stream);

int ds2_greedy_decode(const float* x, long stride_n, long stride_t, int N, int T, int C, const int* sizes, int blank,
                      int* tokens, int* offsets, int* counts, ds2_stream_t stream);

long ds2_beam_ws_bytes(int N, int T, int B);
int ds2_beam_decode(const float* x, long stride_n, long stride_t, int N, int T, int C, const int* sizes, int blank, int B,
                    int cutoff_top_n, float cutoff_prob, int* tokens, int* offsets, int* lens, float* scores, void* ws,
                    ds2_stream_t stream);

int ds2_beam_decode_lm(const float* x, long stride_n, long stride_t, int N, int T, int C, const int* sizes, int blank, int B,
                       int cutoff_top_n, float cutoff_prob, int space, const void* word_table, long word_slots,
                       const void* ngram_table, long ngram_slots, int order, int bos, float alpha, float beta, int lexicon,
                       int* tokens, int* offsets, int* lens, float* scores, float* acoustic, void* ws, ds2_stream_t stream);

long ds2_beam_grid_ws_bytes(int G, int N, int T, int B);
int ds2_beam_decode_lm_grid(const float* x, long stride_n, long stride_t, int N, int T, int C, const int* sizes, int blank, int B,
                            int cutoff_top_n, float cutoff_prob, int space, const void* word_table, long word_slots,
                            const void* ngram_table, long ngram_slots, int order, int bos, int lexicon, int G, const float* alphas,
                            const float* betas, int* tokens, int* offsets, int* lens, float* scores, float* acoustic, void* ws,
                            ds2_stream_t stream);

int ds2_error_counts(const int* hyp, long hyp_stride, const int* hyp_lens, int P, const int* ref, const int* ref_offsets, int R,
                     int space, int* char_err, int* word_err, int* ref_chars, int* ref_words, ds2_stream_t stream);

#ifdef __cplusplus
}
#endif
#endif
```

Baseline: 21270.

## Fuse norm finalize into reduction kernels via last-block counters; fuse add2 with BN stats

```diff
diff --git a/deepspeech/pytorch_amd/_lib.py b/deepspeech/pytorch_amd/_lib.py
--- a/deepspeech/pytorch_amd/_lib.py
+++ b/deepspeech/pytorch_amd/_lib.py
@@ -27,6 +27,13 @@
                         _vp, _vp, _vp, _vp]),
     "ds2_bn_bwd": (_i, [_i, _i, _vp, _vp, _vp, _l, _i, _l, _l, _l, _i, _i, _i, _vp, _vp, _vp, _vp, _vp, _vp, _vp, _vp, _vp]),
     "ds2_colsum": (_i, [_i, _vp, _l, _i, _l, _vp, _f, _vp, _vp]),
+    "ds2_norm_fused_ws_header": (_i, []),
+    "ds2_bn_fwd_fused": (_i, [_i, _i, _i, _vp, _vp, _l, _i, _l, _l, _i, _i, _i, _vp, _vp, _vp, _vp, _vp, _vp, _f, _f, _vp, _vp,
+                              _vp, _vp, _vp, _vp]),
+    "ds2_bn_bwd_fused": (_i, [_i, _i, _vp, _vp, _vp, _l, _i, _l, _l, _l, _i, _i, _i, _vp, _vp, _vp, _vp, _vp, _vp, _vp, _vp, _vp]),
+    "ds2_colsum_fused": (_i, [_i, _vp, _l, _i, _l, _vp, _f, _vp, _vp]),
+    "ds2_add2_colstats": (_i, [_i, _vp, _vp, _vp, _l, _i, _l, _l, _vp, _vp, _vp, _vp, _vp, _f, _f, _vp, _vp, _vp, _vp, _vp, _vp]),
+    "ds2_bn_apply_seq": (_i, [_i, _vp, _vp, _l, _i, _l, _l, _vp, _vp, _vp, _vp, _vp]),
     "ds2_conv_rows": (_i, [_i, _vp, _vp]),
     "ds2_conv1_fwd": (_i, [_i, _vp, _vp, _vp, _vp, _vp, _i, _i, _i, _i, _vp]),
     "ds2_conv1_wgrad_ws_floats": (_l, [_i, _i, _i]),
diff --git a/deepspeech/pytorch_amd/csrc/ds2_norm.hip b/deepspeech/pytorch_amd/csrc/ds2_norm.hip
--- a/deepspeech/pytorch_amd/csrc/ds2_norm.hip
+++ b/deepspeech/pytorch_amd/csrc/ds2_norm.hip
@@ -49,11 +49,220 @@
   }
 }
 
-template <typename T, bool SQ>
-__global__ void __launch_bounds__(NORM_RY* NORM_CX) k_colstats(const T* __restrict__ X, long R, int C, long ld,
-                                                                float* __restrict__ psum, float* __restrict__ psq) {
+constexpr int FIN_COLS = 32, FIN_SLICES = 8;
+template <int NA>
+__device__ __forceinline__ void finalize_sums(const float* const (&arr)[NA], int P, int C, int c, int py, double (&tot)[NA]) {
+  __shared__ double sh[NA][FIN_SLICES][FIN_COLS];
+  double acc[NA];
+#pragma unroll
+  for (int a = 0; a < NA; ++a) acc[a] = 0.0;
+  if (c < C) {
+#pragma unroll 8
+    for (int p = py; p < P; p += FIN_SLICES) {
+#pragma unroll
+      for (int a = 0; a < NA; ++a) acc[a] += (double)arr[a][(long)p * C + c];
+    }
+  }
+#pragma unroll
+  for (int a = 0; a < NA; ++a) sh[a][py][threadIdx.x & (FIN_COLS - 1)] = acc[a];
+  __syncthreads();
+#pragma unroll
+  for (int a = 0; a < NA; ++a) {
+    double t = 0.0;
+    if (py == 0) {
+#pragma unroll
+      for (int q = 0; q < FIN_SLICES; ++q) t += sh[a][q][threadIdx.x & (FIN_COLS - 1)];
+    }
+    tot[a] = t;
+  }
+}
+
+struct FinNone {
+  static constexpr bool on = false;
+  static constexpr int NA = 1;
+  static constexpr bool with_add2 = false;
+  __device__ __forceinline__ void first() const {}
+  __device__ __forceinline__ void col(int, const double (&)[1]) const {}
+};
+struct FinColsum {
+  static constexpr bool on = true;
+  static constexpr int NA = 1;
+  static constexpr bool with_add2 = false;
+  float* out;
+  float scale;
+  __device__ __forceinline__ void first() const {}
+  __device__ __forceinline__ void col(int c, const double (&tot)[1]) const { out[c] = (float)(tot[0] * (double)scale); }
+};
+struct FinBn {
+  static constexpr bool on = true;
+  static constexpr int NA = 2;
+  static constexpr bool with_add2 = true;
+  double count;
+  const float *gamma, *beta;
+  float eps, momentum;
+  float *running_mean, *running_var;
+  long long* num_batches_tracked;
+  float *mean_out, *rstd_out, *scale_out, *shift_out;
+  __device__ __forceinline__ void first() const {
+    if (num_batches_tracked) *num_batches_tracked += 1;
+  }
+  __device__ __forceinline__ void col(int c, const double (&tot)[2]) const {
+    const double s = tot[0], q = tot[1];
+    double mean = s / count;
+    double var = q / count - mean * mean;
+    if (var < 0.0) var = 0.0;
+    double rstd = 1.0 / sqrt(var + (double)eps);
+    mean_out[c] = (float)mean;
+    rstd_out[c] = (float)rstd;
+    float sc = (float)((double)gamma[c] * rstd);
+    scale_out[c] = sc;
+    shift_out[c] = (float)((double)beta[c] - mean * (double)gamma[c] * rstd);
+    if (running_mean) {
+      double unb = count > 1.0 ? var * (count / (count - 1.0)) : var;
+      running_mean[c] = (float)((1.0 - (double)momentum) * (double)running_mean[c] + (double)momentum * mean);
+      running_var[c] = (float)((1.0 - (double)momentum) * (double)running_var[c] + (double)momentum * unb);
+    }
+  }
+};
+struct FinBnBwd {
+  static constexpr bool on = true;
+  static constexpr int NA = 2;
+  static constexpr bool with_add2 = false;
+  double count;
+  float *dgamma, *dbeta, *c1, *c2;
+  __device__ __forceinline__ void first() const {}
+  __device__ __forceinline__ void col(int c, const double (&tot)[2]) const {
+    const double s = tot[0], q = tot[1];
+    dbeta[c] = (float)s;
+    dgamma[c] = (float)q;
+    c1[c] = (float)(s / count);
+    c2[c] = (float)(q / count);
+  }
+};
+
+__global__ void __launch_bounds__(256) k_colsum_finalize(const float* __restrict__ psum, int P, int C, FinColsum fin) {
+  const int c = blockIdx.x * FIN_COLS + (threadIdx.x & (FIN_COLS - 1)), py = threadIdx.x / FIN_COLS;
+  const float* const arr[1] = {psum};
+  double tot[1];
+  finalize_sums<1>(arr, P, C, c, py, tot);
+  if (py == 0 && c < C) fin.col(c, tot);
+}
+
+__global__ void k_bn_finalize(const float* __restrict__ psum, const float* __restrict__ psq, int P, int C, FinBn fin) {
+  const int c = blockIdx.x * FIN_COLS + (threadIdx.x & (FIN_COLS - 1)), py = threadIdx.x / FIN_COLS;
+  if (blockIdx.x == 0 && threadIdx.x == 0) fin.first();
+  const float* const arr[2] = {psum, psq};
+  double tot[2];
+  finalize_sums<2>(arr, P, C, c, py, tot);
+  if (py != 0 || c >= C) return;
+  fin.col(c, tot);
+}
+
+constexpr int NORM_CTR_WORDS = 64;
+static_assert(FIN_COLS == NORM_CX && FIN_SLICES == NORM_RY, "the last workgroup walks the partials as a finalize block does");
+
+template <int NGA, int UNROLL, int NG, int NA>
+__device__ __forceinline__ void walk_partials(const float* const* arr, const int (&cc)[NG], int P, int C, int py, double (&acc)[NG][NA]) {
+  unsigned idx[NGA];
+#pragma unroll
+  for (int g = 0; g < NGA; ++g) idx[g] = (unsigned)py * (unsigned)C + (unsigned)cc[g];
+#pragma unroll UNROLL
+  for (int p = py; p < P; p += FIN_SLICES) {
+#pragma unroll
+    for (int g = 0; g < NGA; ++g) {
+#pragma unroll
+      for (int a = 0; a < NA; ++a) acc[g][a] += (double)arr[a][idx[g]];
+      idx[g] += (unsigned)FIN_SLICES * (unsigned)C;
+    }
+  }
+}
+
+template <int NG, typename FIN>
+__device__ __forceinline__ void last_block_finalize(unsigned* __restrict__ counters, double* lds, const float* const* arr, int C,
+                                                    const FIN& fin) {
+  constexpr int NA = FIN::NA;
+  const int lane = threadIdx.x, py = threadIdx.y, P = gridDim.y;
+  asm volatile("s_waitcnt vmcnt(0)" ::: "memory");
+  __syncthreads();
+  unsigned* flag = reinterpret_cast<unsigned*>(lds);
+  if (lane == 0 && py == 0) {
+    __builtin_amdgcn_fence(__ATOMIC_RELEASE, "agent");
+    asm volatile("s_waitcnt vmcnt(0)" ::: "memory");
+    const unsigned t = __hip_atomic_fetch_add(counters + blockIdx.x, 1u, __ATOMIC_RELAXED, __HIP_MEMORY_SCOPE_AGENT);
+    const bool last = t == (unsigned)(P - 1);
+    if (last) {
+      __builtin_amdgcn_fence(__ATOMIC_ACQUIRE, "agent");
+      asm volatile("s_waitcnt vmcnt(0)" ::: "memory");
+      __hip_atomic_store(counters + blockIdx.x, 0u, __ATOMIC_RELAXED, __HIP_MEMORY_SCOPE_AGENT);
+      if (blockIdx.x == 0) fin.first();
+    }
+    *flag = last ? 1u : 0u;
+  }
+  __syncthreads();
+  const bool last = *flag != 0u;
+  __syncthreads();
+  if (!last) return;
+  const int cbeg = blockIdx.x * (NG * FIN_COLS), cend = min(C, cbeg + NG * FIN_COLS);
+  const int ng = (cend - cbeg + FIN_COLS - 1) / FIN_COLS;
+  int cc[NG];
+#pragma unroll
+  for (int g = 0; g < NG; ++g) cc[g] = min(cbeg + g * FIN_COLS + lane, cend - 1);
+  double acc[NG][NA];
+#pragma unroll
+  for (int g = 0; g < NG; ++g)
+#pragma unroll
+    for (int a = 0; a < NA; ++a) acc[g][a] = 0.0;
+  if (ng == 1)
+    walk_partials<1, 8, NG, NA>(arr, cc, P, C, py, acc);
+  else
+    walk_partials<NG, 2, NG, NA>(arr, cc, P, C, py, acc);
+  double(*sh)[FIN_SLICES][FIN_COLS] = reinterpret_cast<double(*)[FIN_SLICES][FIN_COLS]>(lds);
+  double tot[NA];
+#pragma unroll
+  for (int a = 0; a < NA; ++a) {
+#pragma unroll
+    for (int g = 0; g < NG; ++g) sh[g][py][lane] = acc[g][a];
+    __syncthreads();
+    double t = 0.0;
+    if (py < NG) {
+#pragma unroll
+      for (int q = 0; q < FIN_SLICES; ++q) t += sh[py][q][lane];
+    }
+    tot[a] = t;
+    __syncthreads();
+  }
+  const int c = cbeg + py * FIN_COLS + lane;
+  if (py < NG && c < cend) fin.col(c, tot);
+}
+
+constexpr int FUSED_WAVES = 4;
+
+template <int V, bool FUSED>
+struct RedLds {
+  static constexpr int RED = NORM_RY * (NORM_CX * V + 1) * 4, FIN = FUSED ? V * FIN_SLICES * FIN_COLS * 8 : 0;
+  static constexpr int DOUBLES = ((RED > FIN ? RED : FIN) + 7) / 8;
+};
+
+__device__ __forceinline__ void store_rounded(float* p, float (&v)[4]) { Vec16<float>::store(p, v); }
+__device__ __forceinline__ void store_rounded(bf16_t* p, float (&v)[8]) {
+  uint32_t w[4];
+#pragma unroll
+  for (int i = 0; i < 4; ++i) {
+    w[i] = cvt_pk_bf16(v[2 * i], v[2 * i + 1]);
+    v[2 * i] = __uint_as_float(w[i] << 16);
+    v[2 * i + 1] = __uint_as_float(w[i] & 0xffff0000u);
+  }
+  *reinterpret_cast<uint4*>(p) = make_uint4(w[0], w[1], w[2], w[3]);
+}
+
+template <typename T, bool SQ, typename FIN = FinNone, bool ADD2 = false>
+__global__ void __launch_bounds__(NORM_RY* NORM_CX) __attribute__((amdgpu_waves_per_eu(FIN::on ? FUSED_WAVES : 1, FIN::on ? FUSED_WAVES : 8))) k_colstats(const T* __restrict__ X, long R, int C, long ld,
+                                                                float* __restrict__ psum, float* __restrict__ psq,
+                                                                const T* __restrict__ B, T* __restrict__ O, long ldo,
+                                                                unsigned* __restrict__ counters, FIN fin) {
   constexpr int V = Vec16<T>::N;
-  __shared__ float red[NORM_RY][NORM_CX * V + 1];
+  __shared__ double lds[RedLds<V, FIN::on>::DOUBLES];
+  float(*red)[NORM_CX * V + 1] = reinterpret_cast<float(*)[NORM_CX * V + 1]>(lds);
   const RedMap m(C / V);
   float s[V], q[V];
 #pragma unroll
@@ -62,6 +271,13 @@
     for (long r = m.first_row(); r < R; r += m.row_step()) {
       float v[V];
       Vec16<T>::load(X + r * ld + (long)m.chunk * V, v);
+      if (ADD2) {
+        float y[V];
+        Vec16<T>::load(B + r * ld + (long)m.chunk * V, y);
+#pragma unroll
+        for (int i = 0; i < V; ++i) v[i] += y[i];
+        store_rounded(O + r * ldo + (long)m.chunk * V, v);
+      }
 #pragma unroll
       for (int i = 0; i < V; ++i) {
         s[i] += v[i];
@@ -82,70 +298,10 @@
       for (int i = 0; i < V; ++i) psq[(long)blockIdx.y * C + (long)m.chunk * V + i] = o[i];
     }
   }
-}
-
-constexpr int FIN_COLS = 32, FIN_SLICES = 8;
-template <int NA>
-__device__ __forceinline__ void finalize_sums(const float* const (&arr)[NA], int P, int C, int c, int py, double (&tot)[NA]) {
-  __shared__ double sh[NA][FIN_SLICES][FIN_COLS];
-  double acc[NA];
-#pragma unroll
-  for (int a = 0; a < NA; ++a) acc[a] = 0.0;
-  if (c < C) {
-#pragma unroll 8
-    for (int p = py; p < P; p += FIN_SLICES) {
-#pragma unroll
-      for (int a = 0; a < NA; ++a) acc[a] += (double)arr[a][(long)p * C + c];
-    }
-  }
-#pragma unroll
-  for (int a = 0; a < NA; ++a) sh[a][py][threadIdx.x & (FIN_COLS - 1)] = acc[a];
-  __syncthreads();
-#pragma unroll
-  for (int a = 0; a < NA; ++a) {
-    double t = 0.0;
-    if (py == 0) {
-#pragma unroll
-      for (int q = 0; q < FIN_SLICES; ++q) t += sh[a][q][threadIdx.x & (FIN_COLS - 1)];
-    }
-    tot[a] = t;
-  }
-}
-
-__global__ void __launch_bounds__(256) k_colsum_finalize(const float* __restrict__ psum, int P, int C, float* __restrict__ out,
-                                                          float scale) {
-  const int c = blockIdx.x * FIN_COLS + (threadIdx.x & (FIN_COLS - 1)), py = threadIdx.x / FIN_COLS;
-  const float* const arr[1] = {psum};
-  double tot[1];
-  finalize_sums<1>(arr, P, C, c, py, tot);
-  if (py == 0 && c < C) out[c] = (float)(tot[0] * (double)scale);
-}
-
-__global__ void k_bn_finalize(const float* __restrict__ psum, const float* __restrict__ psq, int P, int C, double count,
-                              const float* __restrict__ gamma, const float* __restrict__ beta, float eps,
-                              float momentum, float* __restrict__ running_mean, float* __restrict__ running_var,
-                              long long* __restrict__ num_batches_tracked, float* __restrict__ mean_out,
-                              float* __restrict__ rstd_out, float* __restrict__ scale_out, float* __restrict__ shift_out) {
-  const int c = blockIdx.x * FIN_COLS + (threadIdx.x & (FIN_COLS - 1)), py = threadIdx.x / FIN_COLS;
-  if (blockIdx.x == 0 && threadIdx.x == 0 && num_batches_tracked) *num_batches_tracked += 1;
-  const float* const arr[2] = {psum, psq};
-  double tot[2];
-  finalize_sums<2>(arr, P, C, c, py, tot);
-  if (py != 0 || c >= C) return;
-  const double s = tot[0], q = tot[1];
-  double mean = s / count;
-  double var = q / count - mean * mean;
-  if (var < 0.0) var = 0.0;
-  double rstd = 1.0 / sqrt(var + (double)eps);
-  mean_out[c] = (float)mean;
-  rstd_out[c] = (float)rstd;
-  float sc = (float)((double)gamma[c] * rstd);
-  scale_out[c] = sc;
-  shift_out[c] = (float)((double)beta[c] - mean * (double)gamma[c] * rstd);
-  if (running_mean) {
-    double unb = count > 1.0 ? var * (count / (count - 1.0)) : var;
-    running_mean[c] = (float)((1.0 - (double)momentum) * (double)running_mean[c] + (double)momentum * mean);
-    running_var[c] = (float)((1.0 - (double)momentum) * (double)running_var[c] + (double)momentum * unb);
+  if constexpr (FIN::on) {
+    static_assert(FIN::NA == (SQ ? 2 : 1), "one partial array per total");
+    const float* const arr[2] = {psum, psq};
+    last_block_finalize<V, FIN>(counters, lds, arr, C, fin);
   }
 }
 
@@ -232,14 +388,15 @@
   return true;
 }
 
-template <typename T, bool CONV, bool SEQ_IN>
-__global__ void __launch_bounds__(NORM_RY* NORM_CX)
+template <typename T, bool CONV, bool SEQ_IN, typename FIN = FinNone>
+__global__ void __launch_bounds__(NORM_RY* NORM_CX) __attribute__((amdgpu_waves_per_eu(FIN::on ? FUSED_WAVES : 1, FIN::on ? FUSED_WAVES : 8)))
     k_bn_bwd_reduce(const T* __restrict__ G, const T* __restrict__ X, long R, int C, long ldg, long ldx,
                     const float* __restrict__ scale, const float* __restrict__ shift, const float* __restrict__ mean,
                     const float* __restrict__ rstd, RowMap rm, const int* __restrict__ lens, int N,
-                    float* __restrict__ psum_g, float* __restrict__ psum_gx) {
+                    float* __restrict__ psum_g, float* __restrict__ psum_gx, unsigned* __restrict__ counters, FIN fin) {
   constexpr int V = Vec16<T>::N;
-  __shared__ float red[NORM_RY][NORM_CX * V + 1];
+  __shared__ double lds[RedLds<V, FIN::on>::DOUBLES];
+  float(*red)[NORM_CX * V + 1] = reinterpret_cast<float(*)[NORM_CX * V + 1]>(lds);
   const RedMap m(C / V);
   float s[V], q[V];
 #pragma unroll
@@ -267,21 +424,19 @@
 #pragma unroll
     for (int i = 0; i < V; ++i) psum_gx[(long)blockIdx.y * C + (long)m.chunk * V + i] = o[i];
   }
-}
-
-__global__ void k_bn_bwd_finalize(const float* __restrict__ psum_g, const float* __restrict__ psum_gx, int P, int C,
-                                  double count, float* __restrict__ dgamma, float* __restrict__ dbeta,
-                                  float* __restrict__ c1, float* __restrict__ c2) {
+  if constexpr (FIN::on) {
+    const float* const arr[2] = {psum_g, psum_gx};
+    last_block_finalize<V, FIN>(counters, lds, arr, C, fin);
+  }
+}
+
+__global__ void k_bn_bwd_finalize(const float* __restrict__ psum_g, const float* __restrict__ psum_gx, int P, int C, FinBnBwd fin) {
   const int c = blockIdx.x * FIN_COLS + (threadIdx.x & (FIN_COLS - 1)), py = threadIdx.x / FIN_COLS;
   const float* const arr[2] = {psum_g, psum_gx};
   double tot[2];
   finalize_sums<2>(arr, P, C, c, py, tot);
   if (py != 0 || c >= C) return;
-  const double s = tot[0], q = tot[1];
-  dbeta[c] = (float)s;
-  dgamma[c] = (float)q;
-  c1[c] = (float)(s / count);
-  c2[c] = (float)(q / count);
+  fin.col(c, tot);
 }
 
 template <typename T, bool CONV, bool SEQ_IN>
@@ -393,19 +548,35 @@
   return (int)gy;
 }
 
-template <typename T>
-int colstats_impl(const void* X, long R, int C, long ld, float* psum, float* psq, int* P_out, hipStream_t st) {
+template <typename T, bool SQ, typename FIN>
+int colstats_launch(const void* X, long R, int C, long ld, float* psum, float* psq, const void* B, void* O, long ldo,
+                    unsigned* counters, const FIN& fin, int* P_out, hipStream_t st) {
   constexpr int V = Vec16<T>::N;
-  DS2_REQUIRE(C % V == 0 && ld % V == 0, DS2_ERR_ALIGN);
+  DS2_REQUIRE(C % V == 0 && ld % V == 0 && ldo % V == 0, DS2_ERR_ALIGN);
   dim3 blk(NORM_CX, NORM_RY);
   dim3 grd(ds2_cdiv(C / V, NORM_CX), norm_grid_y(R, ds2_cdiv(C / V, NORM_CX)));
-  if (psq)
-    hipLaunchKernelGGL((k_colstats<T, true>), grd, blk, 0, st, (const T*)X, R, C, ld, psum, psq);
-  else
-    hipLaunchKernelGGL((k_colstats<T, false>), grd, blk, 0, st, (const T*)X, R, C, ld, psum, psq);
+  DS2_REQUIRE(!FIN::on || (counters != nullptr && grd.x <= (unsigned)NORM_CTR_WORDS), DS2_ERR_ARG);
+  if constexpr (FIN::with_add2) {
+    if (B) {
+      hipLaunchKernelGGL((k_colstats<T, SQ, FIN, true>), grd, blk, 0, st, (const T*)X, R, C, ld, psum, psq, (const T*)B, (T*)O, ldo,
+                         counters, fin);
+      *P_out = grd.y;
+      DS2_CHECK_LAUNCH();
+      return 0;
+    }
+  }
+  DS2_REQUIRE(B == nullptr, DS2_ERR_ARG);
+  hipLaunchKernelGGL((k_colstats<T, SQ, FIN, false>), grd, blk, 0, st, (const T*)X, R, C, ld, psum, psq, (const T*)nullptr,
+                       (T*)nullptr, 0L, counters, fin);
   *P_out = grd.y;
   DS2_CHECK_LAUNCH();
   return 0;
+}
+template <bool SQ, typename FIN>
+int colstats_any(int dtype, const void* X, long R, int C, long ld, float* psum, float* psq, const void* B, void* O, long ldo,
+                 unsigned* counters, const FIN& fin, int* P_out, hipStream_t st) {
+  return dtype == DS2_F32 ? colstats_launch<float, SQ, FIN>(X, R, C, ld, psum, psq, B, O, ldo, counters, fin, P_out, st)
+                          : colstats_launch<bf16_t, SQ, FIN>(X, R, C, ld, psum, psq, B, O, ldo, counters, fin, P_out, st);
 }
 
 inline int apply_grid(long total) {
@@ -421,48 +592,34 @@
 
 int ds2_norm_partials(long R) { return norm_grid_y(R); }
 
-int ds2_colsum(int dtype, const void* X, long R, int C, long ld, float* out, float scale, float* ws, ds2_stream_t st_) {
-  hipStream_t st = (hipStream_t)st_;
+static int colsum_impl(bool fused, int dtype, const void* X, long R, int C, long ld, float* out, float scale, float* ws, hipStream_t st) {
   int P = 0, rc;
-  if (dtype == DS2_F32)
-    rc = colstats_impl<float>(X, R, C, ld, ws, nullptr, &P, st);
-  else
-    rc = colstats_impl<bf16_t>(X, R, C, ld, ws, nullptr, &P, st);
+  const FinColsum fin{out, scale};
+  if (fused)
+    return colstats_any<false, FinColsum>(dtype, X, R, C, ld, ws + NORM_CTR_WORDS, nullptr, nullptr, nullptr, 0, (unsigned*)ws, fin, &P, st);
+  rc = colstats_any<false, FinNone>(dtype, X, R, C, ld, ws, nullptr, nullptr, nullptr, 0, nullptr, FinNone{}, &P, st);
   if (rc) return rc;
-  hipLaunchKernelGGL(k_colsum_finalize, dim3(ds2_cdiv(C, FIN_COLS)), dim3(256), 0, st, ws, P, C, out, scale);
+  hipLaunchKernelGGL(k_colsum_finalize, dim3(ds2_cdiv(C, FIN_COLS)), dim3(256), 0, st, ws, P, C, fin);
   DS2_CHECK_LAUNCH();
   return 0;
 }
-
-int ds2_bn_fwd(int dtype, int mode, int training, const void* X, void* Y, long R, int C, long ldx, long ldy, int F, int Tp,
-               int N, const int* lens, const float* gamma, const float* beta, float* running_mean, float* running_var,
-               long long* num_batches_tracked, float eps, float momentum, float* save_mean, float* save_rstd,
-               float* save_scale, float* save_shift, float* ws, ds2_stream_t st_) {
-  hipStream_t st = (hipStream_t)st_;
-  DS2_REQUIRE(dtype == DS2_F32 || dtype == DS2_BF16, DS2_ERR_DTYPE);
-  DS2_REQUIRE(mode >= 0 && mode <= 2, DS2_ERR_ARG);
-  DS2_REQUIRE(mode == 0 || R < (1L << 31), DS2_ERR_ARG);
-  int rc, P = 0;
-  if (training) {
-    float* psum = ws;
-    float* psq = ws + (long)norm_grid_y(R) * C;
-    rc = dtype == DS2_F32 ? colstats_impl<float>(X, R, C, ldx, psum, psq, &P, st)
-                          : colstats_impl<bf16_t>(X, R, C, ldx, psum, psq, &P, st);
-    if (rc) return rc;
-    hipLaunchKernelGGL(k_bn_finalize, dim3(ds2_cdiv(C, FIN_COLS)), dim3(256), 0, st, psum, psq, P, C, (double)R, gamma, beta,
-                       eps, momentum, running_mean, running_var, num_batches_tracked, save_mean, save_rstd, save_scale,
-                       save_shift);
-  } else {
-    hipLaunchKernelGGL(k_bn_eval_coeffs, dim3(ds2_cdiv(C, 128)), dim3(128), 0, st, C, gamma, beta, running_mean,
-                       running_var, eps, save_scale, save_shift);
-  }
-  DS2_CHECK_LAUNCH();
+int ds2_colsum(int dtype, const void* X, long R, int C, long ld, float* out, float scale, float* ws, ds2_stream_t st_) {
+  return colsum_impl(false, dtype, X, R, C, ld, out, scale, ws, (hipStream_t)st_);
+}
+int ds2_colsum_fused(int dtype, const void* X, long R, int C, long ld, float* out, float scale, float* ws, ds2_stream_t st_) {
+  return colsum_impl(true, dtype, X, R, C, ld, out, scale, ws, (hipStream_t)st_);
+}
+int ds2_norm_fused_ws_header(void) { return NORM_CTR_WORDS; }
+
+static int bn_apply_launch(int dtype, int mode, bool centred, const void* X, void* Y, long R, int C, long ldx, long ldy, int F, int Tp,
+                           int N, const int* lens, const float* beta, const float* save_mean, const float* save_scale,
+                           const float* save_shift, hipStream_t st) {
   RowMap rm{F, Tp};
   const int V = dtype == DS2_F32 ? 4 : 8;
   DS2_REQUIRE(C % V == 0 && ldx % V == 0 && ldy % V == 0, DS2_ERR_ALIGN);
   dim3 g(apply_grid(R * (C / V))), b(256);
 #define LAUNCH_APPLY(TT)                                                                                              \
-  if (mode == 0 && training && R == 1)                                                                                \
+  if (mode == 0 && centred)                                                                                           \
     hipLaunchKernelGGL((k_bn_apply<TT, false, false, true>), g, b, 0, st, (const TT*)X, (TT*)Y, R, C, ldx, ldy,        \
                        save_scale, save_shift, save_mean, beta, rm, lens, N);                                         \
   else if (mode == 0)                                                                                                 \
@@ -484,10 +641,72 @@
   return 0;
 }
 
-int ds2_bn_bwd(int dtype, int mode, const void* G, const void* X, void* DX, long R, int C, long ldg, long ldx, long lddx,
-               int F, int Tp, int N, const int* lens, const float* save_mean, const float* save_rstd,
-               const float* save_scale, const float* save_shift, float* dgamma, float* dbeta, float* ws, ds2_stream_t st_) {
-  hipStream_t st = (hipStream_t)st_;
+static int bn_fwd_impl(bool fused, int dtype, int mode, int training, const void* X, void* Y, long R, int C, long ldx, long ldy, int F,
+                       int Tp, int N, const int* lens, const float* gamma, const float* beta, float* running_mean,
+                       float* running_var, long long* num_batches_tracked, float eps, float momentum, float* save_mean,
+                       float* save_rstd, float* save_scale, float* save_shift, float* ws, hipStream_t st) {
+  DS2_REQUIRE(dtype == DS2_F32 || dtype == DS2_BF16, DS2_ERR_DTYPE);
+  DS2_REQUIRE(mode >= 0 && mode <= 2, DS2_ERR_ARG);
+  DS2_REQUIRE(mode == 0 || R < (1L << 31), DS2_ERR_ARG);
+  int rc, P = 0;
+  if (training) {
+    const FinBn fin{(double)R, gamma, beta, eps, momentum, running_mean, running_var, num_batches_tracked,
+                    save_mean, save_rstd, save_scale, save_shift};
+    float* psum = ws + (fused ? NORM_CTR_WORDS : 0);
+    float* psq = psum + (long)norm_grid_y(R) * C;
+    if (fused) {
+      rc = colstats_any<true, FinBn>(dtype, X, R, C, ldx, psum, psq, nullptr, nullptr, 0, (unsigned*)ws, fin, &P, st);
+      if (rc) return rc;
+    } else {
+      rc = colstats_any<true, FinNone>(dtype, X, R, C, ldx, psum, psq, nullptr, nullptr, 0, nullptr, FinNone{}, &P, st);
+      if (rc) return rc;
+      hipLaunchKernelGGL(k_bn_finalize, dim3(ds2_cdiv(C, FIN_COLS)), dim3(256), 0, st, psum, psq, P, C, fin);
+    }
+  } else {
+    hipLaunchKernelGGL(k_bn_eval_coeffs, dim3(ds2_cdiv(C, 128)), dim3(128), 0, st, C, gamma, beta, running_mean,
+                       running_var, eps, save_scale, save_shift);
+  }
+  DS2_CHECK_LAUNCH();
+  return bn_apply_launch(dtype, mode, training && R == 1, X, Y, R, C, ldx, ldy, F, Tp, N, lens, beta, save_mean, save_scale, save_shift, st);
+}
+int ds2_bn_fwd(int dtype, int mode, int training, const void* X, void* Y, long R, int C, long ldx, long ldy, int F, int Tp,
+               int N, const int* lens, const float* gamma, const float* beta, float* running_mean, float* running_var,
+               long long* num_batches_tracked, float eps, float momentum, float* save_mean, float* save_rstd,
+               float* save_scale, float* save_shift, float* ws, ds2_stream_t st_) {
+  return bn_fwd_impl(false, dtype, mode, training, X, Y, R, C, ldx, ldy, F, Tp, N, lens, gamma, beta, running_mean, running_var,
+                     num_batches_tracked, eps, momentum, save_mean, save_rstd, save_scale, save_shift, ws, (hipStream_t)st_);
+}
+int ds2_bn_fwd_fused(int dtype, int mode, int training, const void* X, void* Y, long R, int C, long ldx, long ldy, int F, int Tp,
+                     int N, const int* lens, const float* gamma, const float* beta, float* running_mean, float* running_var,
+                     long long* num_batches_tracked, float eps, float momentum, float* save_mean, float* save_rstd,
+                     float* save_scale, float* save_shift, float* ws, ds2_stream_t st_) {
+  return bn_fwd_impl(true, dtype, mode, training, X, Y, R, C, ldx, ldy, F, Tp, N, lens, gamma, beta, running_mean, running_var,
+                     num_batches_tracked, eps, momentum, save_mean, save_rstd, save_scale, save_shift, ws, (hipStream_t)st_);
+}
+
+int ds2_add2_colstats(int dtype, const void* a, const void* b, void* out, long R, int C, long ld, long ldo, const float* gamma,
+                      const float* beta, float* running_mean, float* running_var, long long* num_batches_tracked, float eps,
+                      float momentum, float* save_mean, float* save_rstd, float* save_scale, float* save_shift, float* ws,
+                      ds2_stream_t st_) {
+  DS2_REQUIRE(dtype == DS2_F32 || dtype == DS2_BF16, DS2_ERR_DTYPE);
+  DS2_REQUIRE(a && b && out && ws && R > 0 && C > 0 && ld >= C && ldo >= C, DS2_ERR_ARG);
+  const FinBn fin{(double)R, gamma, beta, eps, momentum, running_mean, running_var, num_batches_tracked,
+                  save_mean, save_rstd, save_scale, save_shift};
+  float* psum = ws + NORM_CTR_WORDS;
+  int P = 0;
+  return colstats_any<true, FinBn>(dtype, a, R, C, ld, psum, psum + (long)norm_grid_y(R) * C, b, out, ldo, (unsigned*)ws, fin, &P,
+                                   (hipStream_t)st_);
+}
+int ds2_bn_apply_seq(int dtype, const void* X, void* Y, long R, int C, long ldx, long ldy, const float* beta, const float* save_mean,
+                     const float* save_scale, const float* save_shift, ds2_stream_t st_) {
+  DS2_REQUIRE(dtype == DS2_F32 || dtype == DS2_BF16, DS2_ERR_DTYPE);
+  return bn_apply_launch(dtype, 0, R == 1, X, Y, R, C, ldx, ldy, 0, 0, 0, nullptr, beta, save_mean, save_scale, save_shift,
+                         (hipStream_t)st_);
+}
+
+static int bn_bwd_impl(bool fused, int dtype, int mode, const void* G, const void* X, void* DX, long R, int C, long ldg, long ldx,
+                       long lddx, int F, int Tp, int N, const int* lens, const float* save_mean, const float* save_rstd,
+                       const float* save_scale, const float* save_shift, float* dgamma, float* dbeta, float* ws, hipStream_t st) {
   DS2_REQUIRE(dtype == DS2_F32 || dtype == DS2_BF16, DS2_ERR_DTYPE);
   DS2_REQUIRE(mode >= 0 && mode <= 2, DS2_ERR_ARG);
   DS2_REQUIRE(mode == 0 || R < (1L << 31), DS2_ERR_ARG);
@@ -495,14 +714,20 @@
   DS2_REQUIRE(C % V == 0 && ldx % V == 0 && ldg % V == 0 && lddx % V == 0, DS2_ERR_ALIGN);
   RowMap rm{F, Tp};
   const int P = norm_grid_y(R, ds2_cdiv(C / V, NORM_CX));
-  float* ps = ws;
-  float* pq = ws + (long)P * C;
+  float* ps = ws + (fused ? NORM_CTR_WORDS : 0);
+  float* pq = ps + (long)P * C;
   float* c1 = pq + (long)P * C;
   float* c2 = c1 + C;
   dim3 blk(NORM_CX, NORM_RY), grd(ds2_cdiv(C / V, NORM_CX), P);
+  DS2_REQUIRE(!fused || grd.x <= (unsigned)NORM_CTR_WORDS, DS2_ERR_ARG);
+  const FinBnBwd fin{(double)R, dgamma, dbeta, c1, c2};
 #define LAUNCH_RED(TT, CV, SI)                                                                                          \
-  hipLaunchKernelGGL((k_bn_bwd_reduce<TT, CV, SI>), grd, blk, 0, st, (const TT*)G, (const TT*)X, R, C, ldg, ldx,          \
-                     save_scale, save_shift, save_mean, save_rstd, rm, lens, N, ps, pq)
+  if (fused)                                                                                                            \
+    hipLaunchKernelGGL((k_bn_bwd_reduce<TT, CV, SI, FinBnBwd>), grd, blk, 0, st, (const TT*)G, (const TT*)X, R, C, ldg,   \
+                       ldx, save_scale, save_shift, save_mean, save_rstd, rm, lens, N, ps, pq, (unsigned*)ws, fin);     \
+  else                                                                                                                  \
+    hipLaunchKernelGGL((k_bn_bwd_reduce<TT, CV, SI, FinNone>), grd, blk, 0, st, (const TT*)G, (const TT*)X, R, C, ldg,    \
+                       ldx, save_scale, save_shift, save_mean, save_rstd, rm, lens, N, ps, pq, (unsigned*)nullptr, FinNone{})
   const int acb = ds2_cdiv(C / V, NORM_CX), arpx = NORM_CX / (C / V < NORM_CX ? C / V : NORM_CX);
   long agy = ds2_cdiv(R, (long)NORM_RY * arpx * 2);
   if (agy > 2048 / acb) agy = 2048 / acb;
@@ -530,9 +755,10 @@
   }
   BOTH(LAUNCH_RED)
   DS2_CHECK_LAUNCH();
-  hipLaunchKernelGGL(k_bn_bwd_finalize, dim3(ds2_cdiv(C, FIN_COLS)), dim3(256), 0, st, ps, pq, P, C, (double)R, dgamma, dbeta,
-                     c1, c2);
-  DS2_CHECK_LAUNCH();
+  if (!fused) {
+    hipLaunchKernelGGL(k_bn_bwd_finalize, dim3(ds2_cdiv(C, FIN_COLS)), dim3(256), 0, st, ps, pq, P, C, fin);
+    DS2_CHECK_LAUNCH();
+  }
   BOTH(LAUNCH_APP)
   DS2_CHECK_LAUNCH();
 #undef BOTH
@@ -540,5 +766,17 @@
 #undef LAUNCH_APP
   return 0;
 }
-
-}
+int ds2_bn_bwd(int dtype, int mode, const void* G, const void* X, void* DX, long R, int C, long ldg, long ldx, long lddx,
+               int F, int Tp, int N, const int* lens, const float* save_mean, const float* save_rstd,
+               const float* save_scale, const float* save_shift, float* dgamma, float* dbeta, float* ws, ds2_stream_t st_) {
+  return bn_bwd_impl(false, dtype, mode, G, X, DX, R, C, ldg, ldx, lddx, F, Tp, N, lens, save_mean, save_rstd, save_scale, save_shift,
+                     dgamma, dbeta, ws, (hipStream_t)st_);
+}
+int ds2_bn_bwd_fused(int dtype, int mode, const void* G, const void* X, void* DX, long R, int C, long ldg, long ldx, long lddx,
+                     int F, int Tp, int N, const int* lens, const float* save_mean, const float* save_rstd,
+                     const float* save_scale, const float* save_shift, float* dgamma, float* dbeta, float* ws, ds2_stream_t st_) {
+  return bn_bwd_impl(true, dtype, mode, G, X, DX, R, C, ldg, ldx, lddx, F, Tp, N, lens, save_mean, save_rstd, save_scale, save_shift,
+                     dgamma, dbeta, ws, (hipStream_t)st_);
+}
+
+}
diff --git a/deepspeech/pytorch_amd/model.py b/deepspeech/pytorch_amd/model.py
--- a/deepspeech/pytorch_amd/model.py
+++ b/deepspeech/pytorch_amd/model.py
@@ -60,6 +60,8 @@
 import os
 
 WGRAD_WITH_DX = os.environ.get("DS2_WGRAD_WITH_DX", "1") not in ("", "0")
+
+FUSED_STATS = True
 
 COMPOSITE_NODE = {"": None, "0": False}.get(os.environ.get("DS2_COMPOSITE_NODE", ""), True)
 PER_LAYER_NODES_FOR_DDP = [False]
@@ -215,15 +217,26 @@
     return g.reshape((G, Hp) + tuple(g.shape[1:]))[:, :H].reshape((G * H,) + tuple(g.shape[1:])).contiguous()
 
 
-def _bn_seq_fwd(bn, w, b, X, Xh, R, Ct, Cp, training):
+def _take_carried_stats(mod, X):
+    cs, mod._carried_stats = getattr(mod, "_carried_stats", None), None
+    if cs is None:
+        return None
+    if cs[0] != X.data_ptr():
+        raise Ds2HipError("BatchNorm statistics were computed with a direction sum that is not this BatchNorm's input")
+    return cs[1]
+
+
+def _bn_seq_fwd(bn, w, b, X, Xh, R, Ct, Cp, training, stats=None):
+    if stats is not None:
+        return ops.bn_apply_seq(X, Xh, stats, b.detach(), R, Ct, X.stride(0), Xh.stride(0))
     if Ct == Cp:
         return ops.bn_fwd(X, 0, training, w.detach(), b.detach(), bn.running_mean, bn.running_var, bn.num_batches_tracked, R, Ct,
-                          X.stride(0), Xh, Xh.stride(0), eps=bn.eps, momentum=bn.momentum)
+                          X.stride(0), Xh, Xh.stride(0), eps=bn.eps, momentum=bn.momentum, fused=FUSED_STATS)
     g, be = w.new_ones(Cp), w.new_zeros(Cp)
     rm, rv = w.new_zeros(Cp), w.new_ones(Cp)
     g[:Ct], be[:Ct], rm[:Ct], rv[:Ct] = w.detach(), b.detach(), bn.running_mean, bn.running_var
     sv = ops.bn_fwd(X, 0, training, g, be, rm, rv, bn.num_batches_tracked, R, Cp, X.stride(0), Xh, Xh.stride(0), eps=bn.eps,
-                    momentum=bn.momentum)
+                    momentum=bn.momentum, fused=FUSED_STATS)
     if training:
         bn.running_mean.copy_(rm[:Ct])
         bn.running_var.copy_(rv[:Ct])
@@ -231,8 +244,12 @@
 
 
 def _bn_seq_bwd(G, X, DX, sv, R, Ct, Cp):
-    dg, db = ops.bn_bwd(G, X, DX, 0, sv, R, Cp, G.stride(0), X.stride(0), DX.stride(0))
+    dg, db = ops.bn_bwd(G, X, DX, 0, sv, R, Cp, G.stride(0), X.stride(0), DX.stride(0), fused=FUSED_STATS)
     return (dg, db) if Ct == Cp else (dg[:Ct].contiguous(), db[:Ct].contiguous())
+
+
+def _colsum(X):
+    return ops.colsum(X, fused=FUSED_STATS)
 
 
 def _perm_cols_to_internal(w):
@@ -266,7 +283,7 @@
         a1 = torch.empty_like(y1)
         sv1 = ops.bn_fwd(y1, 1, training, g1.detach(), be1.detach(), bn1.running_mean, bn1.running_var,
                          bn1.num_batches_tracked, R1, 32, 32, a1, 32, F=F1, Tp=Tp, N=N, lens=lens_dev, eps=bn1.eps,
-                         momentum=bn1.momentum)
+                         momentum=bn1.momentum, fused=FUSED_STATS)
         y2 = ops.conv2_fwd(a1, w2t, b2.detach(), lens_dev, F0)
         R2 = N * F2 * Tp
         x0 = torch.empty((Tp * N, rld), dtype=dtype, device=x.device)
@@ -274,7 +291,7 @@
             x0[:, rin:].zero_()
         sv2 = ops.bn_fwd(y2, 2, training, g2.detach(), be2.detach(), bn2.running_mean, bn2.running_var,
                          bn2.num_batches_tracked, R2, 32, 32, x0, rld, F=F2, Tp=Tp, N=N, lens=lens_dev, eps=bn2.eps,
-                         momentum=bn2.momentum)
+                         momentum=bn2.momentum, fused=FUSED_STATS)
         ctx.mod, ctx.dims, ctx.sv = mod, (N, T, Tp, dtype), (sv1, sv2)
         ctx.save_for_backward(x, y1, a1, y2, lens_dev, w2)
         return x0
@@ -289,16 +306,17 @@
         F0, F1, F2, rld = ctx.mod._F0, ctx.mod._F1, ctx.mod._F2, ctx.mod._rnn_ld
         R1, R2 = N * F1 * Tp, N * F2 * Tp
         dy2 = torch.empty_like(y2)
-        dg2, dbe2 = ops.bn_bwd(dx0, y2, dy2, 2, sv2, R2, 32, rld, 32, 32, F=F2, Tp=Tp, N=N, lens=lens_dev)
+        dg2, dbe2 = ops.bn_bwd(dx0, y2, dy2, 2, sv2, R2, 32, rld, 32, 32, F=F2, Tp=Tp, N=N, lens=lens_dev, fused=FUSED_STATS)
         w2d = c.get(("w2d", dtype), [w2], lambda: [
             w2.detach()[:, :, q::2, :].flip(2, 3).permute(2, 3, 1, 0).contiguous().to(dtype) for q in (0, 1)])
         da1 = ops.conv2_dgrad(dy2, w2d[0], w2d[1], F0)
         dy1 = torch.empty_like(y1)
-        dg1, dbe1 = ops.bn_bwd(da1, y1, dy1, 1, sv1, R1, 32, 32, 32, 32, F=F1, Tp=Tp, N=N, lens=lens_dev)
-        db1 = ops.colsum(dy1.view(R1, 32))
+        dg1, dbe1 = ops.bn_bwd(da1, y1, dy1, 1, sv1, R1, 32, 32, 32, 32, F=F1, Tp=Tp, N=N, lens=lens_dev,
+                              fused=FUSED_STATS)
+        db1 = _colsum(dy1.view(R1, 32))
         dw1k = ops.conv1_wgrad(x, dy1, Tp)
         dw1 = dw1k.t().reshape(32, 1, 41, 11).contiguous()
-        db2 = ops.colsum(dy2.view(R2, 32))
+        db2 = _colsum(dy2.view(R2, 32))
         dw2 = ops.conv2_wgrad(dy2, a1, F0).view(21, 11, 32, 32).permute(2, 3, 0, 1).contiguous()
         return (None, dw1, db1, dg1, dbe1, dw2, db2, dg2, dbe2, None, None, None, None, None)
 
@@ -355,7 +373,7 @@
     if has_bn:
         bn = layer.batch_norm.module
         Xh = ops.empty_padded(R, I, X.dtype, X.device)
-        sv = _bn_seq_fwd(bn, bn_w, bn_b, X, Xh, R, layer.input_size, I, training)
+        sv = _bn_seq_fwd(bn, bn_w, bn_b, X, Xh, R, layer.input_size, I, training, stats=_take_carried_stats(mod, X))
     if ops.split3_ok(dtype, R, D * G * H, I):
         Wih3 = c.get(("wih3", li), wih, lambda: ops.split3(Wih, 1))
         GI = ops.gemm_nt(ops.split3(Xh, 0), Wih3, bias=Bih, out_dtype=torch.float32, rows=rows)
@@ -370,7 +388,15 @@
         cn = cn[..., :Ht].contiguous() if cn is not None else None
     del GI
     if D == 2:
-        out = ops.add2(hext[0, 1:Tp + 1].reshape(R, H), hext[1, 1:Tp + 1].reshape(R, H))
+        nbn = (mod.rnns[li + 1].batch_norm.module if mod.rnns[li + 1].batch_norm is not None else None) if li + 1 < len(mod.rnns) \
+            else mod.fc[0].module[0]
+        a, b = hext[0, 1:Tp + 1].reshape(R, H), hext[1, 1:Tp + 1].reshape(R, H)
+        if FUSED_STATS and training and nbn is not None and nbn.num_features == H:
+            out, nsv = ops.add2_colstats(a, b, nbn.weight.detach(), nbn.bias.detach(), nbn.running_mean, nbn.running_var,
+                                         nbn.num_batches_tracked, eps=nbn.eps, momentum=nbn.momentum)
+            mod._carried_stats = (out.data_ptr(), nsv)
+        else:
+            out = ops.add2(a, b)
     else:
         out = hext[0, 1:Tp + 1].reshape(R, H)
     return out, hn, cn, [X, Xh if has_bn else None, hext, Sv], (kind, H, D, G, I, has_bn, sv, Ht, layer.input_size)
@@ -517,9 +543,9 @@
     if rg.bacc is not None:
         dBih, dBhh_all = ops.rnn_bias_grads(kind, rg.bacc, D, N, H)
         return dBih, dBhh_all, [dBhh_all[d] for d in range(D)]
-    dBih = ops.colsum(rg.dGI)
+    dBih = _colsum(rg.dGI)
     if kind == "gru":
-        return dBih, None, [ops.colsum(rg.dGH[d].reshape(R, GH)) for d in range(D)]
+        return dBih, None, [_colsum(rg.dGH[d].reshape(R, GH)) for d in range(D)]
     return dBih, None, [dBih[d * GH:(d + 1) * GH] for d in range(D)]
 
 
@@ -575,10 +601,10 @@
         dWih = torch.cat([_perm_cols_to_reference(dWih[d * GH:(d + 1) * GH], mod._rnn_in) for d in range(D)], 0)
     bsum = None
     if rg.bacc is not None:
-        bsum = [ops.colsum(rg.bacc[d]) for d in range(D)]
+        bsum = [_colsum(rg.bacc[d]) for d in range(D)]
         dBih = torch.cat([b[:GH] for b in bsum], 0)
     else:
-        dBih = ops.colsum(dGI)
+        dBih = _colsum(dGI)
     per_dir = []
     for d in range(D):
         Hp_T = ops.transpose(_h_prev(hext, d, Tp, R, H))
@@ -593,11 +619,11 @@
                 dWhh = ops.gemm_nt_rows2(dGI_T[d * GH:d * GH + 2 * H], dQ_T, 2 * H, Hp_T, GH, H, ldT, ldT, ldT,
                                          splitk=_wgrad_splitk(GH, H, ldT), coresident=cores)
             dBhh = torch.cat([bsum[d][:2 * H], bsum[d][3 * H:4 * H]], 0) if bsum is not None else \
-                torch.cat([dBih[d * GH:d * GH + 2 * H], ops.colsum(rg.dQ[d].reshape(R, H))], 0)
+                torch.cat([dBih[d * GH:d * GH + 2 * H], _colsum(rg.dQ[d].reshape(R, H))], 0)
         else:
             if kind == "gru":
                 dGH_T = ops.transpose(rg.dGH[d].reshape(R, GH))
-                dBhh = ops.colsum(rg.dGH[d].reshape(R, GH))
+                dBhh = _colsum(rg.dGH[d].reshape(R, GH))
             else:
                 dGH_T = dGI_T[d * GH:(d + 1) * GH]
                 dBhh = dBih[d * GH:(d + 1) * GH]
@@ -806,7 +832,7 @@
         R = Tp * N
         c = mod._cache
         Xh = torch.empty_like(X)
-        sv = _bn_seq_fwd(bn, bn_w, bn_b, X, Xh, R, Ht, H, training)
+        sv = _bn_seq_fwd(bn, bn_w, bn_b, X, Xh, R, Ht, H, training, stats=_take_carried_stats(mod, X))
         Wp = c.get(("wfc", dtype), [wfc], lambda: _pad_cols(torch.cat(
             [wfc.detach(), torch.zeros(Cp - Cc, Ht, device=wfc.device)], 0), H).to(dtype).contiguous())
         logits = ops.gemm_nt(Xh, Wp, out_dtype=torch.float32)
@@ -1070,6 +1096,7 @@
         Tp = (T + 2 * 5 - 10 - 1) // 2 + 1
         dev = x.device
         lens_dev, self._frame_rows = _frame_rows(output_lengths, Tp, N, dev)
+        self._carried_stats = None
         training = self.training
         sm = self.conv.seq_module
         with torch.autocast("cuda", enabled=False):
diff --git a/deepspeech/pytorch_amd/ops.py b/deepspeech/pytorch_amd/ops.py
--- a/deepspeech/pytorch_amd/ops.py
+++ b/deepspeech/pytorch_amd/ops.py
@@ -236,12 +236,37 @@
     return outs
 
 
-def colsum(X, R=None, Cc=None, ld=None, scale=1.0):
+FUSED_FINALIZE = True
+_FUSED_WS = {}
+_FUSED_MAX_CHUNKS = 64 * 32
+
+
+def _use_fused(fused, X, Cc):
+    fused = FUSED_FINALIZE if fused is None else fused
+    return fused and Cc // vecw(X.dtype) <= _FUSED_MAX_CHUNKS
+
+
+def fused_ws(nfloats, device):
+    hdr = query("ds2_norm_fused_ws_header")
+    key = (device.index, torch.cuda.current_stream().cuda_stream)
+    ws = _FUSED_WS.get(key)
+    if ws is None or ws.numel() < hdr + nfloats:
+        ws = torch.empty(hdr + nfloats, dtype=torch.float32, device=device)
+        ws[:hdr].zero_()
+        _FUSED_WS[key] = ws
+    return ws
+
+
+def colsum(X, R=None, Cc=None, ld=None, scale=1.0, fused=None):
     R = X.shape[0] if R is None else R
     Cc = X.shape[1] if Cc is None else Cc
     ld = X.stride(0) if ld is None else ld
     out = torch.empty(Cc, dtype=torch.float32, device=X.device)
-    ws = torch.empty(query("ds2_norm_partials", R) * Cc, dtype=torch.float32, device=X.device)
+    n = query("ds2_norm_partials", R) * Cc
+    if _use_fused(fused, X, Cc):
+        call("ds2_colsum_fused", dt(X), P(X), R, Cc, ld, P(out), float(scale), P(fused_ws(n, X.device)), S())
+        return out
+    ws = torch.empty(n, dtype=torch.float32, device=X.device)
     call("ds2_colsum", dt(X), P(X), R, Cc, ld, P(out), float(scale), P(ws), S())
     return out
 
@@ -316,6 +341,22 @@
     return out
 
 
+def add2_colstats(a, b, gamma, beta, rmean, rvar, nbt, eps=1e-5, momentum=0.1):
+    R, Cc = a.shape
+    assert a.shape == b.shape and a.dtype == b.dtype and a.stride(1) == 1 and b.stride(1) == 1 and a.stride(0) == b.stride(0)
+    out = torch.empty((R, Cc), dtype=a.dtype, device=a.device)
+    sv = BnSaved(Cc, a.device)
+    ws = fused_ws(2 * query("ds2_norm_partials", R) * Cc, a.device)
+    call("ds2_add2_colstats", dt(a), P(a), P(b), P(out), R, Cc, a.stride(0), out.stride(0), PF(gamma), PF(beta), PF(rmean), PF(rvar),
+         P(nbt), float(eps), float(momentum), P(sv.mean), P(sv.rstd), P(sv.scale), P(sv.shift), P(ws), S())
+    return out, sv
+
+
+def bn_apply_seq(X, Y, sv, beta, R, Cc, ldx, ldy):
+    call("ds2_bn_apply_seq", dt(X), P(X), P(Y), R, Cc, ldx, ldy, PF(beta), P(sv.mean), P(sv.scale), P(sv.shift), S())
+    return sv
+
+
 class BnSaved:
     __slots__ = ("mean", "rstd", "scale", "shift")
 
@@ -325,20 +366,24 @@
 
 
 def bn_fwd(X, mode, training, gamma, beta, rmean, rvar, nbt, R, Cc, ldx, Y, ldy, F=0, Tp=0, N=0, lens=None, eps=1e-5,
-           momentum=0.1):
+           momentum=0.1, fused=None):
     sv = BnSaved(Cc, X.device)
-    ws = torch.empty(2 * query("ds2_norm_partials", R) * Cc, dtype=torch.float32, device=X.device)
-    call("ds2_bn_fwd", dt(X), mode, 1 if training else 0, P(X), P(Y), R, Cc, ldx, ldy, F, Tp, N, P(lens), PF(gamma), PF(beta),
+    n = 2 * query("ds2_norm_partials", R) * Cc
+    fused = training and _use_fused(fused, X, Cc)
+    ws = fused_ws(n, X.device) if fused else torch.empty(n, dtype=torch.float32, device=X.device)
+    call("ds2_bn_fwd_fused" if fused else "ds2_bn_fwd", dt(X), mode, 1 if training else 0, P(X), P(Y), R, Cc, ldx, ldy, F, Tp, N, P(lens), PF(gamma), PF(beta),
          PF(rmean), PF(rvar), P(nbt) if training else C.c_void_p(0), float(eps), float(momentum), P(sv.mean), P(sv.rstd),
          P(sv.scale), P(sv.shift), P(ws), S())
     return sv
 
 
-def bn_bwd(G, X, DX, mode, sv, R, Cc, ldg, ldx, lddx, F=0, Tp=0, N=0, lens=None):
+def bn_bwd(G, X, DX, mode, sv, R, Cc, ldg, ldx, lddx, F=0, Tp=0, N=0, lens=None, fused=None):
     dgamma = torch.empty(Cc, dtype=torch.float32, device=X.device)
     dbeta = torch.empty(Cc, dtype=torch.float32, device=X.device)
-    ws = torch.empty((2 * query("ds2_norm_partials", R) + 2) * Cc, dtype=torch.float32, device=X.device)
-    call("ds2_bn_bwd", dt(X), mode, P(G), P(X), P(DX), R, Cc, ldg, ldx, lddx, F, Tp, N, P(lens), P(sv.mean), P(sv.rstd),
+    n = (2 * query("ds2_norm_partials", R) + 2) * Cc
+    fused = _use_fused(fused, X, Cc)
+    ws = fused_ws(n, X.device) if fused else torch.empty(n, dtype=torch.float32, device=X.device)
+    call("ds2_bn_bwd_fused" if fused else "ds2_bn_bwd", dt(X), mode, P(G), P(X), P(DX), R, Cc, ldg, ldx, lddx, F, Tp, N, P(lens), P(sv.mean), P(sv.rstd),
          P(sv.scale), P(sv.shift), P(dgamma), P(dbeta), P(ws), S())
     return dgamma, dbeta
 
diff --git a/include/ds2hip.h b/include/ds2hip.h
--- a/include/ds2hip.h
+++ b/include/ds2hip.h
@@ -62,6 +62,22 @@
                const float* save_scale, const float* save_shift, float* dgamma, float* dbeta, float* ws,
                ds2_stream_t stream);
 int ds2_colsum(int dtype, const void* X, long R, int C, long ld, float* out, float scale, float* ws, ds2_stream_t stream);
+int ds2_norm_fused_ws_header(void);
+int ds2_bn_fwd_fused(int dtype, int mode, int training, const void* X, void* Y, long R, int C, long ldx, long ldy, int F, int Tp,
+                     int N, const int* lens, const float* gamma, const float* beta, float* running_mean, float* running_var,
+                     long long* num_batches_tracked, float eps, float momentum, float* save_mean, float* save_rstd,
+                     float* save_scale, float* save_shift, float* ws, ds2_stream_t stream);
+int ds2_bn_bwd_fused(int dtype, int mode, const void* G, const void* X, void* DX, long R, int C, long ldg, long ldx, long lddx,
+                     int F, int Tp, int N, const int* lens, const float* save_mean, const float* save_rstd,
+                     const float* save_scale, const float* save_shift, float* dgamma, float* dbeta, float* ws,
+                     ds2_stream_t stream);
+int ds2_colsum_fused(int dtype, const void* X, long R, int C, long ld, float* out, float scale, float* ws, ds2_stream_t stream);
+int ds2_add2_colstats(int dtype, const void* a, const void* b, void* out, long R, int C, long ld, long ldo, const float* gamma,
+                      const float* beta, float* running_mean, float* running_var, long long* num_batches_tracked, float eps,
+                      float momentum, float* save_mean, float* save_rstd, float* save_scale, float* save_shift, float* ws,
+                      ds2_stream_t stream);
+int ds2_bn_apply_seq(int dtype, const void* X, void* Y, long R, int C, long ldx, long ldy, const float* beta, const float* save_mean,
+                     const float* save_scale, const float* save_shift, ds2_stream_t stream);
 
 int ds2_conv_rows(int F0, int* F1, int* F2);
 int ds2_conv1_fwd(int dtype, const float* x, const float* w1k, const float* b1, const int* lens, void* y1, int N, int F0, int T,
```

Result: no change. 21090 (-0.8%).
